# timescale/pgvectorscale

Hardware: AMD Instinct MI355X
Metric: QPS at recall@10>=0.99 (higher is better)
Workload: dtype u64 xor+popcount (SBQ) / f32 (rerank)

## Files before the change

include/vsgpu.h:

```cpp
#ifndef VSGPU_H
#define VSGPU_H

#include <stddef.h>
#include <stdint.h>

#ifdef __cplusplus
extern "C" {
#endif

#define VS_INVALID_NODE 0xFFFFFFFFu

enum vs_distance_type { VS_COSINE = 0, VS_L2 = 1, VS_IP = 2 };
enum vs_storage_type { VS_STORAGE_SBQ = 0, VS_STORAGE_PLAIN = 1 };

enum vs_status {
    VS_OK = 0,
    VS_ERR_INVALID = -1,
    VS_ERR_HIP = -2,
    VS_ERR_OOM = -3,
    VS_ERR_CAPACITY = -4,
    VS_ERR_STATE = -5
};

typedef struct vs_ctx vs_ctx;
typedef struct vs_index vs_index;
typedef struct vs_scan vs_scan;

typedef struct vs_index_desc {
    uint32_t n;
    uint32_t dim_full;
    uint32_t dim_index;
    uint32_t bits;
    uint32_t words;
    uint32_t num_neighbors;
    uint32_t distance_type;
    uint32_t has_labels;
    uint32_t default_start;
    uint32_t n_label_starts;
    uint32_t storage_type;
} vs_index_desc;

typedef struct vs_index_host {
    const uint64_t* codes;
    const uint32_t* nbrs;
    uint32_t nbr_stride;
    const uint64_t* heap_tids;
    const float* vecs;
    const float* mean;
    const float* m2;
    uint64_t count;
    const uint32_t* label_off;
    const int16_t* label_val;
    const int16_t* label_start_labels;
    const uint32_t* label_start_nodes;
} vs_index_host;

typedef struct vs_stats {
    uint64_t queries;
    uint64_t visited_nodes;
    uint64_t candidate_nodes;
    uint64_t quantized_distance_comparisons;
    uint64_t full_distance_comparisons;
    uint64_t node_reads;
    uint64_t node_heap_reads;
    uint64_t next_calls;
    uint64_t retries;
    uint64_t fallback_scans;
    uint64_t fallback_visited_nodes;
    uint64_t fallback_quantized_distance_comparisons;
} vs_stats;

const char* vs_last_error(void);

int vs_set_option(const char* name, const char* value);
int vs_get_option(const char* name, char* out, size_t cap);
const char* vs_version(void);

int vs_ctx_create(int device, vs_ctx** out);
int vs_ctx_create_staging(int device, size_t staging_bytes, vs_ctx** out);
void vs_ctx_destroy(vs_ctx* ctx);
int vs_ctx_sync(vs_ctx* ctx);
void* vs_ctx_stream(vs_ctx* ctx);
int vs_ctx_device_name(vs_ctx* ctx, char* buf, size_t len);
int vs_ctx_mem_info(vs_ctx* ctx, uint64_t* free_bytes, uint64_t* total_bytes);

typedef struct vs_profile {
    double ms[8];
    uint64_t launches[8];
} vs_profile;
int vs_profile_enable(vs_ctx* ctx, int on);
int vs_profile_read(vs_ctx* ctx, vs_profile* out, int reset);

int vs_dev_alloc(vs_ctx* ctx, size_t bytes, void** out);
int vs_dev_free(vs_ctx* ctx, void* p);
int vs_dev_upload(vs_ctx* ctx, void* dst_dev, const void* src_host, size_t bytes);
int vs_dev_download(vs_ctx* ctx, void* dst_host, const void* src_dev, size_t bytes);

int vs_index_upload(vs_ctx* ctx, const vs_index_desc* desc, const vs_index_host* host, vs_index** out);
int vs_index_alloc(vs_ctx* ctx, const vs_index_desc* desc, int with_vecs, vs_index** out);
void vs_index_free(vs_index* idx);
int vs_index_view(vs_index* src, vs_ctx* ctx, vs_index** out);
int vs_index_set_slab(vs_index* idx, void* d_mem, size_t bytes);
int vs_ws_probe(vs_ctx* ctx, void* d_mem, size_t bytes, uint32_t iters, float* ms_out);
int vs_ws_probe_mix(vs_index* idx, void* d_mem, size_t bytes, uint32_t iters, float* ms_out);
int vs_index_prepare_workspace(vs_index* idx);
int vs_index_get_desc(const vs_index* idx, vs_index_desc* out);
enum vs_array { VS_ARR_CODES = 0, VS_ARR_NBRS = 1, VS_ARR_TIDS = 2, VS_ARR_VECS = 3, VS_ARR_MEAN = 4, VS_ARR_M2 = 5,
                VS_ARR_VNORM = 6, VS_ARR_LABEL_OFF = 7, VS_ARR_LABEL_VAL = 8 };
int vs_index_array(const vs_index* idx, int which, void** dev_ptr, uint32_t* row_stride);
int vs_index_rerank_order(vs_index* idx, uint32_t* out_perm, uint32_t cap, uint32_t* out_n);
int vs_index_set_quantizer(vs_index* idx, const float* mean, const float* m2, uint64_t count);
int vs_index_set_start_nodes(vs_index* idx, uint32_t default_start, const int16_t* labels, const uint32_t* nodes, uint32_t n);
int vs_index_set_labels(vs_index* idx, const uint32_t* label_off, const int16_t* label_val);
int vs_index_set_visibility(vs_index* idx, const uint8_t* visible);
int vs_index_set_visibility_dev(vs_index* idx, const uint8_t* d_visible);
#define VS_MAX_SNAPSHOTS 16
int vs_index_snapshot_put(vs_index* idx, uint32_t snapshot, const uint8_t* visible);
int vs_index_snapshot_use(vs_index* idx, uint32_t snapshot, const uint8_t** previous );
int vs_index_snapshot_share(vs_index* view, const vs_index* src);
int vs_index_device(const vs_index* idx);
int vs_index_has_neighbor_masks(const vs_index* idx);
int vs_index_get_quantizer(const vs_index* idx, float* mean, float* m2, uint64_t* count);
int vs_index_download(const vs_index* idx, uint64_t* codes, uint32_t* nbrs , uint64_t* heap_tids,
                      float* vecs, uint32_t row_begin, uint32_t row_count);
int vs_index_refresh_norms(vs_index* idx);
int vs_index_mark_deleted(vs_index* idx, const uint32_t* nodes, uint32_t n);
typedef struct vs_bulk_delete_stats {
    uint64_t tuples_removed;
    uint64_t num_index_tuples;
    uint64_t already_deleted;
} vs_bulk_delete_stats;
int vs_index_bulk_delete(vs_index* idx, const uint64_t* dead_tids, uint64_t n_dead, vs_bulk_delete_stats* out );
int vs_index_bulk_delete_dev(vs_index* idx, const uint64_t* d_dead_tids_sorted, uint64_t n_dead, vs_bulk_delete_stats* out);
#define VS_CONSOLIDATE_NO_REPAIR 1u
typedef struct vs_consolidate_stats {
    uint64_t tombstones;
    uint64_t tombstones_kept;
    uint64_t rows_rewritten;
    uint64_t edges_dropped;
    uint64_t edges_added;
    uint64_t rows_pruned;
    uint64_t rows_capped;
    uint64_t rows_emptied;
    uint32_t unreachable_live;
} vs_consolidate_stats;
int vs_index_consolidate_deletes(vs_index* idx, double max_alpha, uint32_t cand_max , uint32_t flags,
                                 vs_consolidate_stats* out );
int vs_index_consolidate_kernel_ms(vs_index* idx, double* ms, int reset);
#define VS_COMPACT_KEEP_EDGES_CHECK 1u
typedef struct vs_compact_stats {
    uint32_t n_before, n_after;
    uint64_t tombstones;
    uint64_t tombstones_kept;
    uint64_t rows_moved;
    uint64_t edges_cut;
    uint64_t rows_emptied;
    uint32_t chunks;
} vs_compact_stats;
int vs_index_compact(vs_index* idx, uint64_t stage_bytes , uint32_t flags,
                     uint32_t* out_new_of , vs_compact_stats* out );
int vs_index_compact_kernel_ms(vs_index* idx, double* ms, int reset);
int vs_index_shrink_to_fit(vs_index* idx);

#define VS_BLCKSZ 8192u
enum vs_page_type {
    VS_PAGE_META_V1 = 0, VS_PAGE_NODE = 1, VS_PAGE_PQ_QUANTIZER_DEF = 2, VS_PAGE_PQ_QUANTIZER_VECTOR = 3,
    VS_PAGE_SBQ_MEANS_V1 = 4, VS_PAGE_SBQ_NODE = 5, VS_PAGE_META_V2 = 6, VS_PAGE_SBQ_MEANS = 7, VS_PAGE_META = 8 };

typedef struct vs_node_layout {
    uint32_t root_size;
    uint32_t off_heap_item_pointer;
    uint32_t off_bq_vector;
    uint32_t off_neighbor_index_pointers;
    uint32_t off_labels;
} vs_node_layout;
int vs_node_layout_default(int has_labels, vs_node_layout* out);

typedef struct vs_pages_info {
    uint32_t n_blocks;
    uint32_t n_nodes;
    uint32_t words;
    uint32_t num_neighbors;
    uint32_t has_labels;
    uint32_t n_deleted;
    uint64_t n_label_vals;
    uint32_t pages_by_type[9];
    uint32_t new_pages;
    uint32_t meta_magic;
    uint32_t meta_version;
} vs_pages_info;

typedef struct vs_pages vs_pages;
int vs_pages_open(uint32_t page_size, int has_labels, const vs_node_layout* layout, uint32_t threads, vs_pages** out);
int vs_plain_layout_default(vs_node_layout* out);
int vs_pages_open_plain(uint32_t page_size, const vs_node_layout* layout, uint32_t threads, vs_pages** out);
int vs_pages_add(vs_pages* p, uint32_t first_block, const void* pages, uint32_t n_blocks);
int vs_pages_finish(vs_pages* p, vs_pages_info* info);
int vs_pages_host(const vs_pages* p, vs_index_host* host);
int vs_pages_node_of(const vs_pages* p, uint32_t block, uint32_t offset, uint32_t* node);
int vs_pages_item_pointer_of(const vs_pages* p, uint32_t node, uint32_t* block, uint32_t* offset);
int vs_pages_read_chain(const vs_pages* p, uint32_t block, uint32_t offset, int page_type, void* buf, size_t cap, size_t* len);
int vs_pages_sbq_means(const vs_pages* p, uint32_t block, uint32_t offset, float* mean, float* m2, uint32_t dim_cap,
                       uint32_t* dim, uint64_t* count);
void vs_pages_close(vs_pages* p);
int vs_pages_headers_only(vs_pages* p);
int vs_pages_block_table(const vs_pages* p, const uint32_t** blk_base, const uint32_t** blk_cnt, uint32_t* n_blocks);

typedef struct vs_meta_layout {
    uint32_t root_size;
    uint32_t off_magic_number, off_version, off_extension_version_when_built, off_distance_type, off_num_dimensions,
        off_num_dimensions_to_index, off_bq_num_bits_per_dimension, off_storage_type, off_num_neighbors, off_search_list_size,
        off_max_alpha, off_start_nodes, off_quantizer_metadata, off_has_labels;
} vs_meta_layout;
int vs_meta_layout_default(vs_meta_layout* out);
typedef struct vs_meta_page {
    uint32_t magic_number, version;
    char extension_version_when_built[64];
    uint32_t distance_type;
    uint32_t num_dimensions, num_dimensions_to_index, bq_num_bits_per_dimension;
    uint32_t storage_type;
    uint32_t num_neighbors, search_list_size;
    double max_alpha;
    uint32_t has_start_nodes;
    uint32_t default_start_block, default_start_offset;
    uint32_t n_labeled_start_nodes;
    uint32_t quantizer_block, quantizer_offset;
    uint32_t has_labels;
} vs_meta_page;
int vs_meta_page_decode(const void* bytes, size_t len, const vs_meta_layout* layout, vs_meta_page* out, int16_t* start_labels,
                        uint32_t* start_blocks, uint32_t* start_offsets, uint32_t cap);
int vs_pages_meta(const vs_pages* p, const vs_meta_layout* layout, vs_meta_page* meta, vs_index_desc* desc, int16_t* start_labels,
                  uint32_t* start_nodes, uint32_t cap);

typedef struct vs_heap_attr {
    int16_t attlen;
    char attalign;
} vs_heap_attr;
typedef struct vs_heap_info {
    uint32_t n_nodes, heap_blocks, toast_blocks;
    uint32_t n_inline;
    uint32_t n_external;
    uint32_t n_deleted;
    uint32_t n_null;
    uint32_t n_dead_line_pointer;
    uint32_t n_not_found;
    uint32_t n_toast_incomplete;
    uint64_t n_chunks;
} vs_heap_info;
typedef struct vs_heap vs_heap;
int vs_heap_open(uint32_t page_size, const vs_heap_attr* attrs, uint32_t natts, uint32_t vector_attno, uint32_t dim,
                 const uint64_t* heap_tids, uint32_t n, float* out_vecs, uint32_t out_stride, vs_heap** out);
int vs_heap_add(vs_heap* h, uint32_t first_block, const void* pages, uint32_t n_blocks);
int vs_heap_toast_add(vs_heap* h, uint32_t first_block, const void* pages, uint32_t n_blocks);
int vs_heap_finish(vs_heap* h, vs_heap_info* info, uint8_t* found);
void vs_heap_close(vs_heap* h);

typedef struct vs_pages_dev vs_pages_dev;
int vs_pages_dev_open(vs_ctx* ctx, uint32_t page_size, const vs_node_layout* layout, uint32_t n_blocks_total, vs_pages_dev** out);
int vs_pages_dev_add(vs_pages_dev* d, uint32_t first_block, const void* pages, uint32_t n_blocks);
int vs_pages_dev_node_of(const vs_pages_dev* d, uint32_t block, uint32_t offset, uint32_t* node);
int vs_pages_dev_sbq_means(const vs_pages_dev* d, uint32_t block, uint32_t offset, float* mean, float* m2, uint32_t dim_cap,
                           uint32_t* dim, uint64_t* count);
int vs_pages_dev_meta(vs_pages_dev* d, const vs_meta_layout* layout, vs_meta_page* meta, vs_index_desc* desc, int16_t* start_labels,
// ... 265 lines not shown
```

pgvectorscale_amd/__init__.py:

```python
from ._lib import VS_COSINE, VS_INVALID_NODE, VS_IP, VS_L2, VsError, load
from .index import Broker, Context, DiskAnnIndex, IndexScan, ScanPool, ShmClient, ShmServer, get_option, set_option
from .multi import Comm, MultiIndex
```

pgvectorscale_amd/_lib.py:

```python
import ctypes as C
import os

_HERE = os.path.dirname(os.path.abspath(__file__))
LIB_PATH = os.environ.get("VS_LIB_PATH") or os.path.join(_HERE, "libvsgpu.so")

VS_INVALID_NODE = 0xFFFFFFFF
VS_COSINE, VS_L2, VS_IP = 0, 1, 2
VS_STORAGE_SBQ, VS_STORAGE_PLAIN = 0, 1
ARR_CODES, ARR_NBRS, ARR_TIDS, ARR_VECS, ARR_MEAN, ARR_M2, ARR_VNORM, ARR_LABEL_OFF, ARR_LABEL_VAL = range(9)


class VsError(RuntimeError):
    def __init__(self, code, msg):
        super().__init__(f"libvsgpu error {code}: {msg}")
        self.code = code


class IndexDesc(C.Structure):
    _fields_ = [(k, C.c_uint32) for k in ("n", "dim_full", "dim_index", "bits", "words", "num_neighbors",
                                          "distance_type", "has_labels", "default_start", "n_label_starts", "storage_type")]


class IndexHost(C.Structure):
    _fields_ = [("codes", C.c_void_p), ("nbrs", C.c_void_p), ("nbr_stride", C.c_uint32), ("heap_tids", C.c_void_p),
# ... 39 lines not shown
class MetaPage(C.Structure):
    _fields_ = [("magic_number", C.c_uint32), ("version", C.c_uint32), ("extension_version_when_built", C.c_char * 64),
                ("distance_type", C.c_uint32), ("num_dimensions", C.c_uint32), ("num_dimensions_to_index", C.c_uint32),
                ("bq_num_bits_per_dimension", C.c_uint32), ("storage_type", C.c_uint32), ("num_neighbors", C.c_uint32),
                ("search_list_size", C.c_uint32), ("max_alpha", C.c_double), ("has_start_nodes", C.c_uint32),
                ("default_start_block", C.c_uint32), ("default_start_offset", C.c_uint32), ("n_labeled_start_nodes", C.c_uint32),
                ("quantizer_block", C.c_uint32), ("quantizer_offset", C.c_uint32), ("has_labels", C.c_uint32)]

    def as_dict(self):
        d = {k: getattr(self, k) for k, _ in self._fields_}
        d["extension_version_when_built"] = d["extension_version_when_built"].decode()
        return d


class HeapAttr(C.Structure):
    _fields_ = [("attlen", C.c_int16), ("attalign", C.c_char)]


class HeapInfo(C.Structure):
    _fields_ = [(k, C.c_uint32) for k in ("n_nodes", "heap_blocks", "toast_blocks", "n_inline", "n_external", "n_deleted", "n_null",
                                          "n_dead_line_pointer", "n_not_found", "n_toast_incomplete")] + [("n_chunks", C.c_uint64)]

    def as_dict(self):
        return {k: int(getattr(self, k)) for k, _ in self._fields_}


class PagesInfo(C.Structure):
    _fields_ = [("n_blocks", C.c_uint32), ("n_nodes", C.c_uint32), ("words", C.c_uint32), ("num_neighbors", C.c_uint32),
                ("has_labels", C.c_uint32), ("n_deleted", C.c_uint32), ("n_label_vals", C.c_uint64),
                ("pages_by_type", C.c_uint32 * 9), ("new_pages", C.c_uint32), ("meta_magic", C.c_uint32),
                ("meta_version", C.c_uint32)]


class PagesOutParams(C.Structure):
    _fields_ = [("page_size", C.c_uint32), ("node_layout", C.POINTER(NodeLayout)), ("meta_layout", C.POINTER(MetaLayout)),
                ("extension_version", C.c_char_p), ("search_list_size", C.c_uint32), ("max_alpha", C.c_double)]


class BrokerConfig(C.Structure):
    _fields_ = [("max_batch", C.c_uint32), ("max_wait_us", C.c_uint32), ("cursor_lanes", C.c_uint32), ("cursor_pool", C.c_uint32)]


class BrokerStats(C.Structure):
    _fields_ = [("batches", C.c_uint64), ("scans", C.c_uint64), ("max_batch", C.c_uint64), ("tasks", C.c_uint64), ("cursors", C.c_uint64)]


class Profile(C.Structure):
    _fields_ = [("ms", C.c_double * 8), ("launches", C.c_uint64 * 8)]


class InsertStats(C.Structure):
    _fields_ = [(k, C.c_uint32) for k in ("first_node", "inserted", "batches", "retries", "mate_edges", "orphans_placed",
                                          "orphans_left", "grew")]

    def as_dict(self):
        return {k: int(getattr(self, k)) for k, _ in self._fields_}


class BulkDeleteStats(C.Structure):
    _fields_ = [(k, C.c_uint64) for k in ("tuples_removed", "num_index_tuples", "already_deleted")]

    def as_dict(self):
        return {k: int(getattr(self, k)) for k, _ in self._fields_}


class ConsolidateStats(C.Structure):
    _fields_ = [(k, C.c_uint64) for k in ("tombstones", "tombstones_kept", "rows_rewritten", "edges_dropped", "edges_added", "rows_pruned",
                                          "rows_capped", "rows_emptied")] + [("unreachable_live", C.c_uint32)]

    def as_dict(self):
        return {k: int(getattr(self, k)) for k, _ in self._fields_}


VS_CONSOLIDATE_NO_REPAIR = 1


class CompactStats(C.Structure):
    _fields_ = [("n_before", C.c_uint32), ("n_after", C.c_uint32)] + [(k, C.c_uint64) for k in (
        "tombstones", "tombstones_kept", "rows_moved", "edges_cut", "rows_emptied")] + [("chunks", C.c_uint32)]

    def as_dict(self):
        return {k: int(getattr(self, k)) for k, _ in self._fields_}


VS_COMPACT_KEEP_EDGES_CHECK = 1


class LabelReachStats(C.Structure):
    _fields_ = [("lost_pairs", C.c_uint64)] + [(k, C.c_uint32) for k in ("lost_nodes", "labels", "labels_without_start", "sweeps")]

    def as_dict(self):
        return {k: int(getattr(self, k)) for k, _ in self._fields_}


class LabelRepairStats(C.Structure):
    _fields_ = [(k, C.c_uint64) for k in ("lost_pairs_before", "lost_pairs_after", "placed_free", "placed_over_dropped", "placed_victim",
                                          "blocked", "contended", "rows_changed", "source_tiles")] + [(k, C.c_uint32) for k in (
        "lost_nodes_before", "lost_nodes_after", "rounds", "sweeps", "labels_without_start", "unreachable_live")]

    def as_dict(self):
        return {k: int(getattr(self, k)) for k, _ in self._fields_}


class PagesFollowInfo(C.Structure):
    _fields_ = [(k, C.c_uint32) for k in ("n_blocks_before", "n_blocks_now", "pages_listed", "node_pages_listed", "n_before", "n_appended",
                                          "rows_relinked", "tids_cleared", "tids_changed", "codes_changed")] + [("label_vals_appended", C.c_uint64)]

    def as_dict(self):
        return {k: int(getattr(self, k)) for k, _ in self._fields_}


class DatagenParams(C.Structure):
    _fields_ = [("seed", C.c_uint64), ("dim", C.c_uint32), ("latent_dim", C.c_uint32), ("n_clusters", C.c_uint32),
                ("intra_pct", C.c_uint32), ("noise_pct", C.c_uint32), ("normalize", C.c_uint32)]


_vp, _u32, _u64, _i, _sz = C.c_void_p, C.c_uint32, C.c_uint64, C.c_int, C.c_size_t
SYMBOLS = {
    "vs_last_error": (C.c_char_p, []),
    "vs_set_option": (_i, [C.c_char_p, C.c_char_p]),
    "vs_get_option": (_i, [C.c_char_p, C.c_char_p, C.c_size_t]),
    "vs_version": (C.c_char_p, []),
    "vs_ctx_create": (_i, [_i, C.POINTER(_vp)]),
    "vs_ctx_create_staging": (_i, [_i, _sz, C.POINTER(_vp)]),
    "vs_ctx_destroy": (None, [_vp]),
    "vs_ctx_sync": (_i, [_vp]),
    "vs_ctx_stream": (_vp, [_vp]),
    "vs_ctx_device_name": (_i, [_vp, C.c_char_p, _sz]),
    "vs_ctx_mem_info": (_i, [_vp, C.POINTER(_u64), C.POINTER(_u64)]),
    "vs_profile_enable": (_i, [_vp, _i]),
    "vs_profile_read": (_i, [_vp, C.POINTER(Profile), _i]),
    "vs_dev_alloc": (_i, [_vp, _sz, C.POINTER(_vp)]),
    "vs_dev_free": (_i, [_vp, _vp]),
    "vs_dev_upload": (_i, [_vp, _vp, _vp, _sz]),
    "vs_dev_download": (_i, [_vp, _vp, _vp, _sz]),
    "vs_index_upload": (_i, [_vp, C.POINTER(IndexDesc), C.POINTER(IndexHost), C.POINTER(_vp)]),
    "vs_index_alloc": (_i, [_vp, C.POINTER(IndexDesc), _i, C.POINTER(_vp)]),
    "vs_index_free": (None, [_vp]),
    "vs_index_view": (_i, [_vp, _vp, _vp]),
    "vs_scanpool_create": (_i, [_vp, _u32, _u32, _u32, _u32, _u32, C.POINTER(_vp)]),
    "vs_scanpool_free": (None, [_vp]),
    "vs_scanpool_rescan": (_i, [_vp, _u32, _vp, _vp, _u32, _i]),
    "vs_scanpool_endscan": (_i, [_vp, _u32]),
    "vs_scanpool_fetch": (_i, [_vp, _vp, _u32, _u32, _vp, _vp, _vp, _vp]),
    "vs_scanpool_get_stats": (_i, [_vp, _u32, _vp]),
    "vs_scanpool_get_work": (_i, [_vp, C.POINTER(_u64), C.POINTER(_u64)]),
    "vs_index_set_slab": (_i, [_vp, _vp, C.c_size_t]),
    "vs_ws_probe": (_i, [_vp, _vp, C.c_size_t, C.c_uint32, C.POINTER(C.c_float)]),
    "vs_ws_probe_mix": (_i, [_vp, _vp, C.c_size_t, C.c_uint32, C.POINTER(C.c_float)]),
    "vs_index_prepare_workspace": (_i, [_vp]),
    "vs_index_get_desc": (_i, [_vp, C.POINTER(IndexDesc)]),
    "vs_index_array": (_i, [_vp, _i, C.POINTER(_vp), C.POINTER(_u32)]),
    "vs_index_rerank_order": (_i, [_vp, _vp, _u32, C.POINTER(_u32)]),
    "vs_index_set_quantizer": (_i, [_vp, _vp, _vp, _u64]),
    "vs_index_set_start_nodes": (_i, [_vp, _u32, _vp, _vp, _u32]),
    "vs_index_set_labels": (_i, [_vp, _vp, _vp]),
    "vs_index_set_visibility": (_i, [_vp, _vp]),
    "vs_index_set_visibility_dev": (_i, [_vp, _vp]),
    "vs_index_get_quantizer": (_i, [_vp, _vp, _vp, C.POINTER(_u64)]),
    "vs_index_download": (_i, [_vp, _vp, _vp, _vp, _vp, _u32, _u32]),
    "vs_index_refresh_norms": (_i, [_vp]),
    "vs_index_mark_deleted": (_i, [_vp, _vp, _u32]),
    "vs_index_bulk_delete": (_i, [_vp, _vp, _u64, C.POINTER(BulkDeleteStats)]),
    "vs_index_bulk_delete_dev": (_i, [_vp, _vp, _u64, C.POINTER(BulkDeleteStats)]),
    "vs_index_consolidate_deletes": (_i, [_vp, C.c_double, _u32, _u32, C.POINTER(ConsolidateStats)]),
    "vs_index_consolidate_kernel_ms": (_i, [_vp, C.POINTER(C.c_double), _i]),
    "vs_index_compact": (_i, [_vp, C.c_uint64, _u32, _vp, C.POINTER(CompactStats)]),
    "vs_index_compact_kernel_ms": (_i, [_vp, C.POINTER(C.c_double), _i]),
    "vs_index_shrink_to_fit": (_i, [_vp]),
    "vs_node_layout_default": (_i, [_i, C.POINTER(NodeLayout)]),
    "vs_pages_open": (_i, [_u32, _i, C.POINTER(NodeLayout), _u32, C.POINTER(_vp)]),
    "vs_pages_open_plain": (_i, [_u32, C.POINTER(NodeLayout), _u32, C.POINTER(_vp)]),
    "vs_plain_layout_default": (_i, [C.POINTER(NodeLayout)]),
    "vs_pages_add": (_i, [_vp, _u32, _vp, _u32]),
    "vs_pages_finish": (_i, [_vp, C.POINTER(PagesInfo)]),
    "vs_pages_host": (_i, [_vp, C.POINTER(IndexHost)]),
    "vs_pages_node_of": (_i, [_vp, _u32, _u32, C.POINTER(_u32)]),
    "vs_pages_item_pointer_of": (_i, [_vp, _u32, C.POINTER(_u32), C.POINTER(_u32)]),
    "vs_pages_read_chain": (_i, [_vp, _u32, _u32, _i, _vp, _sz, C.POINTER(_sz)]),
    "vs_pages_sbq_means": (_i, [_vp, _u32, _u32, _vp, _vp, _u32, C.POINTER(_u32), C.POINTER(_u64)]),
    "vs_pages_close": (None, [_vp]),
    "vs_heap_open": (_i, [_u32, C.POINTER(HeapAttr), _u32, _u32, _u32, _vp, _u32, _vp, _u32, C.POINTER(_vp)]),
    "vs_heap_add": (_i, [_vp, _u32, _vp, _u32]),
    "vs_heap_toast_add": (_i, [_vp, _u32, _vp, _u32]),
    "vs_heap_finish": (_i, [_vp, C.POINTER(HeapInfo), _vp]),
    "vs_heap_close": (None, [_vp]),
    "vs_meta_layout_default": (_i, [C.POINTER(MetaLayout)]),
    "vs_meta_page_decode": (_i, [_vp, _sz, C.POINTER(MetaLayout), C.POINTER(MetaPage), _vp, _vp, _vp, _u32]),
    "vs_pages_meta": (_i, [_vp, C.POINTER(MetaLayout), C.POINTER(MetaPage), C.POINTER(IndexDesc), _vp, _vp, _u32]),
    "vs_pages_dev_meta": (_i, [_vp, C.POINTER(MetaLayout), C.POINTER(MetaPage), C.POINTER(IndexDesc), _vp, _vp, _u32]),
    "vs_pages_headers_only": (_i, [_vp]),
    "vs_pages_block_table": (_i, [_vp, C.POINTER(_vp), C.POINTER(_vp), C.POINTER(_u32)]),
    "vs_pages_dev_open": (_i, [_vp, _u32, C.POINTER(NodeLayout), _u32, C.POINTER(_vp)]),
    "vs_pages_dev_add": (_i, [_vp, _u32, _vp, _u32]),
    "vs_pages_dev_node_of": (_i, [_vp, _u32, _u32, C.POINTER(_u32)]),
    "vs_pages_dev_sbq_means": (_i, [_vp, _u32, _u32, _vp, _vp, _u32, C.POINTER(_u32), C.POINTER(_u64)]),
    "vs_pages_dev_build": (_i, [_vp, C.POINTER(IndexDesc), C.POINTER(IndexHost), C.POINTER(PagesInfo), C.POINTER(_vp)]),
    "vs_pages_dev_close": (None, [_vp]),
    "vs_pages_dev_block_table": (_i, [_vp, C.POINTER(_vp), C.POINTER(_vp), C.POINTER(_u32)]),
    "vs_pages_follow_open": (_i, [_vp, _u32, C.POINTER(NodeLayout), _vp, _u32, C.POINTER(_vp)]),
    "vs_pages_follow_stage": (_i, [_vp, _vp, _vp, _u32, _u32, C.POINTER(PagesFollowInfo)]),
    "vs_pages_follow_new_tids": (_i, [_vp, _vp, _u32]),
    "vs_pages_follow_apply": (_i, [_vp, _vp, _u32, C.POINTER(PagesFollowInfo)]),
    "vs_pages_follow_discard": (_i, [_vp]),
    "vs_pages_follow_close": (None, [_vp]),
    "vs_pages_out_open": (_i, [_vp, C.POINTER(PagesOutParams), C.POINTER(_vp), C.POINTER(PagesInfo)]),
    "vs_pages_out_open_plain": (_i, [_vp, C.POINTER(PagesOutParams), C.POINTER(_vp), C.POINTER(PagesInfo)]),
    "vs_pages_out_read": (_i, [_vp, _u32, _u32, _vp]),
    "vs_pages_out_read_dev": (_i, [_vp, _u32, _u32, _vp]),
    "vs_pages_out_item_pointer_of": (_i, [_vp, _u32, C.POINTER(_u32), C.POINTER(_u32)]),
    "vs_pages_out_close": (None, [_vp]),
    "vs_pages_out_baseline": (_i, [_vp, C.POINTER(_vp)]),
    "vs_pages_base_free": (None, [_vp]),
    "vs_pages_base_blocks": (_u32, [_vp]),
    "vs_pages_out_delta": (_i, [_vp, _vp, C.POINTER(_u32), C.POINTER(_u32), C.POINTER(_vp)]),
    "vs_pages_out_delta_blocks": (_i, [_vp, _vp, _u32]),
    "vs_pages_out_read_blocks": (_i, [_vp, _vp, _u32, _vp]),
    "vs_pages_out_read_blocks_dev": (_i, [_vp, _vp, _u32, _vp]),
    "vs_meta_page_encode": (_i, [C.POINTER(MetaPage), _vp, _vp, _vp, _u32, C.POINTER(MetaLayout), _vp, _sz, C.POINTER(_sz)]),
    "vs_quantize": (_i, [_vp, _vp, _u32, _vp]),
    "vs_hamming_gather": (_i, [_vp, _vp, _vp, _vp, _u32, _vp]),
    "vs_rerank": (_i, [_vp, _vp, _vp, _vp, _u32, _vp]),
    "vs_prepare_queries": (_i, [_vp, _vp, _u32, _vp, _vp, _vp]),
    "vs_scan_topk": (_i, [_vp, _vp, _u32, _u32, _vp, _vp]),
    "vs_scan_topk_filtered": (_i, [_vp, _vp, _vp, _vp, _i, _u32, _u32, _vp, _vp]),
    "vs_search_batch": (_i, [_vp, _vp, _vp, _vp, _u32, _u32, _u32, _u32, _vp, _vp, _vp, C.POINTER(Stats)]),
    "vs_stream_batch": (_i, [_vp, _vp, _vp, _vp, _u32, _u32, _u32, _vp, _vp, C.POINTER(Stats)]),
    "vs_search_batch_dev": (_i, [_vp, _vp, _vp, _vp, _u32, _u32, _u32, _u32, _vp, _vp, _vp]),
    "vs_search_batch_dev_finish": (_i, [_vp, C.POINTER(Stats)]),
    "vs_index_autotune": (_i, [_vp, _vp, _vp, _vp, _u32, _u32, _u32, _u32, _u32, C.c_char_p, C.POINTER(TuneEntry), _u32, C.POINTER(_u32)]),
    "vs_index_set_variant": (_i, [_vp, C.c_char_p]),
    "vs_index_get_variant": (_i, [_vp, C.c_char_p, C.c_size_t]),
    "vs_beginscan": (_i, [_vp, C.POINTER(_vp)]),
    "vs_rescan": (_i, [_vp, _vp, _vp, _u32, _i, _u32, _u32]),
    "vs_gettuple": (_i, [_vp, C.POINTER(_u64), C.POINTER(_u32), C.POINTER(C.c_float)]),
    "vs_scan_xs_recheck": (_i, [_vp]),
    "vs_scan_get_stats": (_i, [_vp, C.POINTER(Stats)]),
    "vs_scan_get_work": (_i, [_vp, C.POINTER(Stats), C.POINTER(_u32)]),
    "vs_endscan": (None, [_vp]),
    "vs_broker_create": (_i, [_vp, C.POINTER(BrokerConfig), C.POINTER(_vp)]),
    "vs_broker_search": (_i, [_vp, _vp, _vp, _u32, _i, _u32, _u32, _u32, _vp, _vp, _vp]),
    "vs_broker_search_snapshot": (_i, [_vp, _vp, _vp, _u32, _i, _u32, _u32, _u32, _u32, _vp, _vp, _vp]),
    "vs_broker_snapshot_put": (_i, [_vp, _u32, _vp]),
    "vs_index_snapshot_put": (_i, [_vp, _u32, _vp]),
    "vs_index_has_neighbor_masks": (_i, [_vp]),
    "vs_index_snapshot_use": (_i, [_vp, _u32, _vp]),
    "vs_index_snapshot_share": (_i, [_vp, _vp]),
    "vs_index_device": (_i, [_vp]),
    "vs_broker_get_stats": (_i, [_vp, C.POINTER(BrokerStats)]),
    "vs_broker_destroy": (None, [_vp]),
    "vs_broker_index": (_vp, [_vp]),
    "vs_beginscan_on_broker": (_i, [_vp, C.POINTER(_vp)]),
    "vs_broker_call": (_i, [_vp, _vp, _vp]),
    "vs_scan_set_snapshot": (_i, [_vp, _u32]),
    "vs_scan_prefetch": (_i, [_vp, _u32]),
    "vs_shm_client_fetch": (_i, [_vp, C.c_uint64, _vp, _vp, _u32, _i, _u32, _u32, _u32, _u32, _u32, _vp, _vp, _vp, C.POINTER(_u32)]),
    "vs_shm_client_end_scan": (_i, [_vp, C.c_uint64]),
    "vs_shm_server_create": (_i, [_vp, C.c_char_p, _u32, _u32, C.POINTER(BrokerConfig), C.POINTER(_vp)]),
    "vs_shm_server_get_stats": (_i, [_vp, C.POINTER(BrokerStats)]),
    "vs_shm_server_pool_stats": (_i, [_vp, C.POINTER(C.c_uint64)]),
    "vs_shm_server_destroy": (None, [_vp]),
    "vs_shm_server_snapshot_put": (_i, [_vp, _u32, _vp]),
    "vs_shm_client_search_snapshot": (_i, [_vp, _vp, _vp, _u32, _i, _u32, _u32, _u32, _u32, _vp, _vp, _vp]),
    "vs_shm_client_open": (_i, [C.c_char_p, C.POINTER(_vp)]),
    "vs_shm_client_dim": (_u32, [_vp]),
    "vs_shm_client_search": (_i, [_vp, _vp, _vp, _u32, _i, _u32, _u32, _u32, _vp, _vp, _vp]),
    "vs_shm_client_close": (None, [_vp]),
    "vs_shard_range": (_i, [_u32, _u32, _u32, C.POINTER(_u32), C.POINTER(_u32)]),
    "vs_index_replicate": (_i, [_vp, _vp, C.POINTER(_vp)]),
    "vs_multi_create": (_i, [_vp, C.POINTER(_i), _u32, _u32, C.POINTER(_vp)]),
    "vs_multi_size": (_u32, [_vp]),
    "vs_multi_index": (_vp, [_vp, _u32]),
    "vs_multi_ctx": (_vp, [_vp, _u32]),
    "vs_multi_search_batch": (_i, [_vp, _vp, _vp, _vp, _u32, _u32, _u32, _u32, _vp, _vp, _vp, C.POINTER(Stats)]),
    "vs_multi_stream_batch": (_i, [_vp, _vp, _vp, _vp, _u32, _u32, _u32, _vp, _vp, C.POINTER(Stats)]),
    "vs_multi_destroy": (None, [_vp]),
    "vs_comm_unique_id": (_i, [_vp]),
    "vs_comm_create": (_i, [_vp, _vp, _u32, _u32, C.POINTER(_vp)]),
    "vs_comm_rank": (_u32, [_vp]),
    "vs_comm_world": (_u32, [_vp]),
    "vs_comm_gather_topk": (_i, [_vp, _vp, _vp, _u32, _u32, _u32, _vp, _vp]),
    "vs_comm_bcast": (_i, [_vp, _vp, _sz, _u32]),
    "vs_comm_replicate_index": (_i, [_vp, _vp, _u32]),
    "vs_comm_destroy": (None, [_vp]),
    "vs_sbq_train": (_i, [_vp]),
    "vs_sbq_quantize_corpus": (_i, [_vp]),
    "vs_build_graph": (_i, [_vp, _u32, C.c_double, _u32, _u64]),
    "vs_index_build_unreachable": (_u32, [_vp]),
    "vs_index_reserve": (_i, [_vp, _u32]),
    "vs_index_capacity": (_u32, [_vp]),
    "vs_index_insert": (_i, [_vp, _vp, _vp, _vp, _vp, _u32, _u32, C.c_double, _u32, C.POINTER(InsertStats)]),
    "vs_index_insert_dev": (_i, [_vp, _vp, _vp, _vp, _vp, _u32, _u32, C.c_double, _u32, C.POINTER(InsertStats)]),
    "vs_index_insert_kernel_ms": (_i, [_vp, C.POINTER(C.c_double), _i]),
    "vs_index_build_kernel_ms": (_i, [_vp, C.POINTER(C.c_double), _i]),
    "vs_batch_mates": (_i, [_vp, _vp, _u32, _u32, _vp, _vp]),
    "vs_batch_mates_filtered": (_i, [_vp, _vp, _vp, _vp, _u32, _u32, _vp, _vp]),
    "vs_batch_mates_plain": (_i, [_vp, _u32, _u32, _u32, _vp, _vp]),
    "vs_prune_plain": (_i, [_vp, _vp, _vp, _vp, _u32, C.c_double, _vp, _vp]),
    "vs_index_repair": (_i, [_vp, C.POINTER(_u32)]),
    "vs_index_label_reach": (_i, [_vp, C.POINTER(LabelReachStats), _vp, _vp, _vp, _u32, _vp]),
    "vs_index_repair_labels": (_i, [_vp, _u32, _u32, C.POINTER(LabelRepairStats)]),
    "vs_index_label_repair_kernel_ms": (_i, [_vp, C.POINTER(C.c_double), _i]),
    "vs_nearest_masked": (_i, [_vp, _vp, _vp, _u32, _vp, _vp, _vp, _vp]),
    "vs_datagen_fill": (_i, [_vp, C.POINTER(DatagenParams), _u64, _u64, _vp]),
    "vs_bruteforce_topk": (_i, [_vp, _vp, _u32, _u32, _vp, _vp]),
}
# ... 32 lines not shown
```

pgvectorscale_amd/csrc/vs_batch.hip:

```cpp
#include <thread>
#include <cstdarg>
#include <cmath>
#include <algorithm>
#include <cstdlib>

#include <atomic>
#include <mutex>
#include <unordered_map>

#include "vs_internal.h"


static uint32_t knob_u32(const char* name, int tuned, uint32_t dflt) {
    const char* v = vs_opt_get(name);
    if (v && *v) return (uint32_t)strtoul(v, nullptr, 10);
    return tuned >= 0 ? (uint32_t)tuned : dflt;
}

static uint32_t gload_pct() { return std::min<uint32_t>(std::max<uint32_t>(env_u32("VS_F_GLOAD_PCT", 75), 25), 90); }

static Caps initial_caps(const vs_index* ix, uint32_t L, uint32_t M) {
    uint64_t visits = 2ull * L + M + 32;
    uint64_t pushes = visits * ix->d.num_neighbors;
    Caps c;
    c.hl = env_u32("VS_HL", 1024);
    c.lh = env_u32("VS_LH", 0);
    c.g0 = env_u32("VS_G0", 4096);
    c.hcap = (uint32_t)std::min<uint64_t>(std::max<uint64_t>(pushes, c.hl), 1u << 22);
    c.vcap = (uint32_t)std::min<uint64_t>(3ull * L + M + 64, 1u << 20);
    c.hashcap = std::max<uint32_t>(next_pow2_u32(std::min<uint64_t>(2ull * pushes, 1u << 23)), c.g0);
    const uint64_t typ_visits = (uint64_t)L + L / 4 + M + 16;
    uint64_t typ_ins = typ_visits * std::min<uint64_t>(ix->d.num_neighbors, 16);
    if (ix->obs.valid && ix->obs.L == L && ix->obs.M == M) typ_ins = (uint64_t)(ix->obs.ins_mean * 1.75) + 96;
    const bool lds_table = typ_ins <= knob_u32("VS_F_LDS_MAX_INS", ix->tune.lds_max_ins, 1024);
    c.f_lh = env_u32("VS_F_LH", lds_table ? (uint32_t)round_up_u32((uint32_t)typ_ins, 64) : 0u);
    c.f_pool_frac = !lds_table ? 1.0
                    : (ix->obs.valid && ix->obs.L == L && ix->obs.M == M) ? std::min(1.0, 2.0 * ix->obs.ov_frac + 0.03) : 1.0;
    if (const char* e = vs_opt_get("VS_F_POOL")) c.f_pool_frac = std::min(1.0, std::max(0.01, atof(e)));
    uint32_t hl_auto = 1023;
    if (lds_table && ix->obs.valid && ix->obs.L == L && ix->obs.M == M) {
        const double want = 0.75 * ix->obs.ins_mean;
        hl_auto = want > 2047 ? 4095 : (want > 1023 ? 2047 : 1023);
    }
    if (!lds_table) hl_auto = 511;
    c.f_hl = env_u32("VS_F_HL", hl_auto);
    const uint32_t want_v = (uint32_t)std::min<uint64_t>((uint64_t)L + L / 2 + 32, 1u << 20);
    c.f_vr = knob_u32("VS_F_VR", ix->tune.vr, (lds_table && want_v <= 512) ? 8 : 0);
    c.f_vcap = c.f_vr ? 512 : round_up_u32(std::max<uint32_t>(env_u32("VS_F_VCAP", 2 * want_v), 64), 64);
    c.f_on = env_u32("VS_FAST", 1) != 0 && ix->d.storage_type != VS_STORAGE_PLAIN;
    if (c.f_on) {
        if (c.f_lh) c.f_lh = round_up_u32(std::max<uint32_t>(c.f_lh, 256), 4);
        c.f_hl = std::max<uint32_t>(next_pow2_u32(c.f_hl + 1), 64) - 1;
        c.f_gcap = next_pow2_u32(std::min<uint64_t>(std::max<uint64_t>(std::min<uint64_t>(pushes, 4 * typ_ins), 1024), 1u << 22));
        if (!lds_table && ix->obs.valid && ix->obs.L == L && ix->obs.M == M && env_u32("VS_F_GCAP_FIT", 1)) {
            const uint64_t need = (uint64_t)((ix->obs.ins_max * 1.04 + 128) * 100.0 / gload_pct()) + 64;
            c.f_gcap = (uint32_t)std::min<uint64_t>(c.f_gcap, std::max<uint64_t>(round_up_u32((uint32_t)std::min<uint64_t>(need, 1u << 22), 256), 1024));
        }
        if (const uint32_t g = env_u32("VS_F_GCAP", lds_table ? 0 : ix->tune.gcap)) c.f_gcap = round_up_u32(std::max<uint32_t>(g, 256), 256);
        c.f_sb = 0;
        while ((1ull << c.f_sb) < (uint64_t)c.f_lh + c.f_gcap) c.f_sb++;
        c.f_hcap = (uint32_t)std::min<uint64_t>(std::max<uint64_t>(pushes, c.f_hl), 1u << 22);
        c.f_gstride = round_up_u32(c.f_hcap - c.f_hl + 2, 2);
        const uint64_t nbits = (uint64_t)ix->d.dim_index * ix->d.bits;
        FastLaunch probe{};
        probe.hl = c.f_hl;
        probe.lh = c.f_lh;
        probe.vr = c.f_vr;
        probe.vcap = c.f_vcap;
        if (nbits >= (1ull << (32 - c.f_sb)) || fast_lds_bytes(ix, probe) > 64 * 1024) c.f_on = false;
    }
    return c;
}

static uint32_t fast_pool_slots(uint32_t nq, double frac) {
    const uint64_t floor_slots = vs_opt_get("VS_F_POOL") ? 1 : 256;
    return (uint32_t)std::min<uint64_t>(nq, std::max<uint64_t>(floor_slots, (uint64_t)(frac * nq) + 1));
}
static uint32_t general_pool_slots(uint32_t nq) { return std::max<uint32_t>(64, nq / 64); }

static bool grow_caps(Caps& c, uint32_t ovf) {
    bool grew = (ovf & (OVF_POOL | OVF_KEY)) != 0;
    if ((ovf & OVF_HEAP) && c.hcap < (1u << 24)) {
        c.hcap *= 2;
        grew = true;
    }
    if (ovf & OVF_VISITED) {
        c.vcap *= 2;
        grew = true;
    }
    if ((ovf & OVF_HASH) && c.hashcap < (1u << 26)) {
        c.hashcap *= 2;
        grew = true;
    }
    return grew;
}

static const double ORDER_MIN_REUSE = 2.0;
static const uint32_t ORDER_MIN_NQ = 16384;
static const uint32_t ORDER_SEEDS = 1024;
static const uint32_t ORDER_LABEL_SEEDS = 2048;
static uint32_t rerank_order_seeds(const vs_index* ix, uint32_t nq, uint32_t M, bool* by_labels) {
    const uint32_t mode = env_u32("VS_RERANK_ORDER", 1);
    *by_labels = mode != 2 && !ix->is_view;
    if (mode == 0 || !scan_order_fits(ix)) return 0;
    if (mode == 1 && (nq < ORDER_MIN_NQ || (double)nq * M < ORDER_MIN_REUSE * (double)ix->d.n)) return 0;
    const uint32_t S = std::min<uint32_t>(std::max<uint32_t>(env_u32("VS_RERANK_SEEDS", *by_labels ? ORDER_LABEL_SEEDS : ORDER_SEEDS), 1), 4096);
    return std::min<uint32_t>(S, ix->d.n);
}

static int ensure_region_labels(vs_index* ix, uint32_t S) {
    vs_ctx* c = ix->ctx;
    SearchWorkspace& w = ix->ws;
    const uint32_t n = ix->d.n, step = n / S;
    const bool kept = w.lab_rows > 0 && w.lab_rows <= n && w.lab_epoch == ix->codes_epoch && w.lab_S == S && w.lab_step == step;
    const uint32_t from = kept ? w.lab_rows : 0;
    if (from == n) return VS_OK;
    const bool debug = env_u32("VS_WS_DEBUG", 0) != 0;
    if (debug) VS_HIP(hipStreamSynchronize(c->stream));
    const auto t0 = std::chrono::steady_clock::now();
    if ((size_t)n * 2 > w.order_labels.bytes) {
        DevBuf grown;
        VS_TRY(devbuf_reserve(c, grown, std::max<size_t>((size_t)n * 2, w.order_labels.bytes + w.order_labels.bytes / 2)));
        if (from) VS_HIP(hipMemcpyAsync(grown.p, w.order_labels.p, (size_t)from * 2, hipMemcpyDeviceToDevice, c->stream));
        VS_HIP(hipStreamSynchronize(c->stream));
        devbuf_free(w.order_labels);
        w.order_labels = grown;
    }
    w.lab_rows = 0;
    VS_TRY(launch_region_labels(ix, S, step, from, n - from, (uint16_t*)w.order_labels.p));
    w.lab_rows = n;
    w.lab_S = S;
    w.lab_step = step;
    w.lab_epoch = ix->codes_epoch;
    if (debug) {
        VS_HIP(hipStreamSynchronize(c->stream));
        fprintf(stderr, "[VS_WS_DEBUG] region labels: rows %u .. %u, %u seeds %u rows apart, %.3f ms\n", from, n, S, step,
                std::chrono::duration<double, std::milli>(std::chrono::steady_clock::now() - t0).count());
    }
    return VS_OK;
}

extern "C" int vs_index_rerank_order(vs_index* ix, uint32_t* out_perm, uint32_t cap, uint32_t* out_n) {
    VS_REQUIRE(ix && out_n && (cap == 0 || out_perm), "vs_index_rerank_order: bad args");
    VS_HIP(hipStreamSynchronize(ix->ctx->stream));
    *out_n = ix->ws.order_nq;
    const uint32_t m = std::min(cap, ix->ws.order_nq);
    if (m) VS_HIP(hipMemcpy(out_perm, ix->ws.order_perm.p, (size_t)m * 4, hipMemcpyDeviceToHost));
    return VS_OK;
}

static int run_post_search(vs_index* ix, const BatchPlan& bp, uint32_t* d_out_ids, uint64_t* d_out_tids, float* d_out_dist) {
    vs_ctx* c = ix->ctx;
    SearchWorkspace& w = ix->ws;
    const uint32_t nq = bp.nq, M = bp.M;
    if (bp.stream_only) return VS_OK;
    if (bp.rescore > 0) {
        VS_REQUIRE(ix->vecs, "diskann.query_rescore > 0 needs the heap vector column on the device");
        const uint32_t* perm = nullptr;
        bool deal = false;
        w.order_nq = 0;
        bool by_labels = false;
        if (const uint32_t S = rerank_order_seeds(ix, nq, M, &by_labels)) {
            VS_TRY(devbuf_reserve(c, w.order_work, scan_order_work_bytes(nq, S + 1)));
            VS_TRY(devbuf_reserve(c, w.order_perm, (size_t)nq * 4));
            if (by_labels) VS_TRY(ensure_region_labels(ix, S));
            hipEvent_t ev = prof_begin(c);
            if (by_labels)
                VS_TRY(launch_label_order(ix, (const uint16_t*)w.order_labels.p, w.lab_rows, S, (const uint32_t*)w.stream_ids.p,
                                          (const uint32_t*)w.stream_cnt.p, M, nq, (uint32_t*)w.order_work.p, (uint32_t*)w.order_perm.p));
            else
                VS_TRY(launch_scan_order(ix, (const uint64_t*)w.qcodes.p, nq, S, (uint32_t*)w.order_work.p, (uint32_t*)w.order_perm.p));
            prof_end(c, PK_ORDER, ev);
            perm = (const uint32_t*)w.order_perm.p;
            w.order_nq = nq;
            deal = env_u32("VS_RERANK_DEAL", 1) != 0;
        }
        const uint32_t fused = env_u32("VS_RERANK_FUSED", 1);
        if (fused && rerank_window_fits(ix, M, bp.rescore, bp.k)) {
            hipEvent_t ev = prof_begin(c);
            VS_TRY(launch_rerank_window(ix, (const float*)w.q_full.p, (const uint32_t*)w.stream_ids.p, (const uint32_t*)w.stream_cnt.p, M,
                                        bp.rescore, bp.k, nq, d_out_ids, d_out_tids, d_out_dist, fused == 2 ? 2u : 1u, perm, deal));
            prof_end(c, PK_RERANK, ev);
            return VS_OK;
        }
        VS_TRY(devbuf_reserve(c, w.rr_dist, (size_t)nq * M * 4));
        VS_TRY(devbuf_reserve(c, w.resort_heap, (size_t)nq * bp.rescore * 8));
        hipEvent_t ev = prof_begin(c);
        VS_TRY(launch_rerank(ix, (const float*)w.q_full.p, (const uint32_t*)w.stream_ids.p, nullptr,
                             (const uint32_t*)w.stream_cnt.p, M, nq, (float*)w.rr_dist.p, 0, perm, deal));
        prof_end(c, PK_RERANK, ev);
    }
    hipEvent_t ev = prof_begin(c);
    VS_TRY(launch_resort(ix, nq, M, bp.rescore, bp.k, (const uint32_t*)w.stream_ids.p, (const uint32_t*)w.stream_cnt.p,
                         bp.rescore ? (const float*)w.rr_dist.p : nullptr, (uint64_t*)w.resort_heap.p, d_out_ids,
                         d_out_tids, d_out_dist));
    prof_end(c, PK_RESORT, ev);
    return VS_OK;
}

static int enqueue_reduce(vs_index* ix, const BatchPlan& bp) {
    vs_ctx* c = ix->ctx;
    SearchWorkspace& w = ix->ws;
    VS_TRY(devbuf_reserve(c, w.red, RED_N * 8));
    if (!w.red_host) VS_HIP(hipHostMalloc((void**)&w.red_host, RED_N * 8, hipHostMallocDefault));
    VS_HIP(hipMemsetAsync(w.red.p, 0, RED_N * 8, c->stream));
    VS_TRY(launch_reduce_stats(ix, (const uint32_t*)w.stats.p, w.fb_valid ? (const uint32_t*)w.fb_flag.p : nullptr,
                               (const uint32_t*)w.stream_cnt.p, (const uint32_t*)w.status.p, bp.nq, bp.M, bp.rescore,
                               !bp.stream_only && bp.rescore > 0, ix->last_ins_limit, (uint64_t*)w.red.p));
    VS_HIP(hipMemcpyAsync(w.red_host, w.red.p, RED_N * 8, hipMemcpyDeviceToHost, c->stream));
    return VS_OK;
}

static SearchLaunch general_launch(const vs_index* ix, const BatchPlan& bp, const Caps& caps, const int16_t* d_qlabels,
                                   const uint32_t* d_qlabel_off) {
    const SearchWorkspace& w = ix->ws;
    SearchLaunch s;
    s.nq = bp.nq;
    s.L = bp.L;
    s.M = bp.M;
    s.hl = caps.hl;
    s.hcap = caps.hcap;
    s.vcap = caps.vcap;
    s.lh = caps.lh;
    s.hashcap = caps.hashcap;
    s.g0 = caps.g0;
    s.qcodes = (const uint64_t*)w.qcodes.p;
    s.qlabels = d_qlabels;
    s.qlabel_off = d_qlabel_off;
    s.heap_g = (uint64_t*)w.heap_g.p;
    s.hash = (uint32_t*)w.hash.p;
    s.out_ids = (uint32_t*)w.stream_ids.p;
    s.out_ham = (uint32_t*)w.stream_ham.p;
    s.out_cnt = (uint32_t*)w.stream_cnt.p;
    s.stats = (uint32_t*)w.stats.p;
    s.status = (uint32_t*)w.status.p;
    s.visible = (!bp.stream_only && bp.rescore > 0) ? ix->visible : nullptr;
    return s;
}

static int reserve_general_regions(vs_index* ix, const Caps& caps, uint32_t gslots) {
    vs_ctx* c = ix->ctx;
    SearchWorkspace& w = ix->ws;
    const size_t hg = caps.hcap > caps.hl ? caps.hcap - caps.hl : 0;
    VS_TRY(devbuf_reserve(c, w.hash, (size_t)gslots * caps.hashcap * 4));
    VS_TRY(devbuf_reserve(c, w.heap_g, std::max<size_t>((size_t)gslots * hg * 8, 16)));
    return devbuf_reserve(c, w.pool_ctr, 64);
}

static int retry_failed_scans(vs_index* ix, const BatchPlan& bp, const int16_t* d_qlabels, const uint32_t* d_qlabel_off,
                              Caps& caps, vs_stats* st) {
    vs_ctx* c = ix->ctx;
    SearchWorkspace& w = ix->ws;
    const uint32_t nq = bp.nq;
    std::vector<uint32_t> status(nq);
    for (int attempt = 0;; ++attempt) {
        VS_HIP(hipMemcpyAsync(status.data(), w.status.p, (size_t)nq * 4, hipMemcpyDeviceToHost, c->stream));
        VS_HIP(hipStreamSynchronize(c->stream));
        uint32_t ovf = 0, nbad = 0;
        for (uint32_t v : status) {
            ovf |= v;
            nbad += v != 0;
        }
        if (!ovf) return VS_OK;
        if (st) st->retries++;
        if (attempt >= 8 || !grow_caps(caps, ovf)) {
            vs_set_error("search structures overflowed in %u of %u scans (flags 0x%x) at hcap=%u vcap=%u hashcap=%u", nbad, nq,
                         ovf, caps.hcap, caps.vcap, caps.hashcap);
            return VS_ERR_CAPACITY;
        }
        const uint32_t gslots = std::min<uint32_t>(nq, std::max<uint32_t>(general_pool_slots(nq), nbad));
        VS_TRY(reserve_general_regions(ix, caps, gslots));
        VS_HIP(hipMemsetAsync((char*)w.pool_ctr.p + 32, 0, 4, c->stream));
        SearchLaunch s = general_launch(ix, bp, caps, d_qlabels, d_qlabel_off);
        s.only_failed = 1;
        s.fb_flag = w.fb_valid ? (uint32_t*)w.fb_flag.p : nullptr;
        s.pool_counter = (uint32_t*)((char*)w.pool_ctr.p + 32);
        s.pool_slots = gslots;
        hipEvent_t ev = prof_begin(c);
        VS_TRY(launch_search(ix, s));
        prof_end(c, PK_SEARCH_FB, ev);
    }
}

struct FastPlan {
    FastLaunch f;
    uint32_t gregion;
    uint32_t fslots;
};
template <class T>
static T* fast_select() {
    return (T*)16;
}

static bool opt_is_set(const char* name) {
    const char* v = vs_opt_get(name);
    return v && *v;
}
static uint32_t visited_want(uint32_t L) { return (uint32_t)std::min<uint64_t>((uint64_t)L + L / 2 + 32, 1u << 20); }

static int candidate_holds(vs_index* ix, const FastLaunch& base, const FastLaunch& cand, uint64_t num, uint64_t den, bool* holds,
                           const char* base_name = nullptr, const char* cand_name = nullptr, const char* tail = "") {
    uint32_t res_base = 0, res_cand = 0;
    VS_TRY(fast_resident_scans(ix, base, &res_base));
    VS_TRY(fast_resident_scans(ix, cand, &res_cand));
    if (base_name && env_u32("VS_WS_DEBUG", 0))
        fprintf(stderr, "[VS_WS_DEBUG] resident scans: %s %u, %s %u%s\n", base_name, res_base, cand_name, res_cand, tail);
    *holds = num * res_cand >= den * res_base;
    return VS_OK;
}

static int choose_table_bitmap(vs_index* ix, FastLaunch& f, uint32_t vmode, bool phase, bool* slot_eligible) {
    *slot_eligible = false;
    if (f.lh != 0 || f.vr || !vmode || phase || f.gcap > (1u << 16)) return VS_OK;
    f.vwords = (f.gcap + 127) / 128;
    if (vmode < 2 || f.rc || f.gcap % 32 != 0) return VS_OK;
    *slot_eligible = true;
    FastLaunch g = f;
    g.vwords = f.gcap / 32;
    g.vslot = 1;
    bool holds = false;
    VS_TRY(candidate_holds(ix, f, g, 1, 1, &holds));
    if (holds || env_u32("VS_F_SLOTMAP_FORCE", 0)) f = g;
    return VS_OK;
}

static int choose_tables16(vs_index* ix, FastLaunch& f, uint32_t vmode, bool slot_eligible, bool keyed, uint32_t* gregion) {
    if (vmode != 3 || !f.vwords || !slot_eligible || f.lh != 0) return VS_OK;
    FastLaunch g = f;
    g.gcap = std::max<uint32_t>(next_pow2_u32(f.gcap), 1024);
    if (!fast_tables16_geometry(ix, g)) return VS_OK;
    g.glimit = (uint32_t)((uint64_t)g.gcap * gload_pct() / 100) - 64u;
    char tail[48];
    snprintf(tail, sizeof tail, "; gcap %u -> %u", f.gcap, g.gcap);
    bool holds = false;
    VS_TRY(candidate_holds(ix, f, g, keyed ? 3 : 5, keyed ? 2 : 4, &holds, "4-byte tables", "16-bit tables", tail));
    if (holds || env_u32("VS_F_SLOTMAP_FORCE", 0)) {
        f = g;
        *gregion = g.gregion;
    }
    return VS_OK;
}

static int choose_heap_top(vs_index* ix, FastLaunch& f, Caps& caps, bool phase) {
    if (f.lh != 0 || f.vr || f.hl != 511 || f.hcap <= 511 || phase || opt_is_set("VS_F_HL")) return VS_OK;
    FastLaunch h = f;
    h.hl = 255;
    h.gstride = round_up_u32(h.hcap - h.hl + 2, 2);
    bool holds = false;
    VS_TRY(candidate_holds(ix, f, h, 10, 11, &holds, "heap top 511", "255"));
    if (holds) {
        f = h;
        caps.f_hl = h.hl;
        caps.f_gstride = h.gstride;
    }
    return VS_OK;
}

static int choose_visited_ring(vs_index* ix, FastLaunch& f, uint32_t L, bool phase) {
    if (f.lh != 0 || f.vr || f.minw == 7 || phase) return VS_OK;
    const uint32_t want_v = visited_want(L);
    const uint32_t lean_v = round_up_u32(std::max<uint32_t>(want_v + 2 * want_v / 5, 64), 64);
    if (opt_is_set("VS_F_VCAP") || lean_v >= f.vcap) return VS_OK;
    FastLaunch v = f;
    v.vcap = lean_v;
    char wide_name[40], lean_name[24];
    snprintf(wide_name, sizeof wide_name, "visited ring %u entries", f.vcap);
    snprintf(lean_name, sizeof lean_name, "%u entries", v.vcap);
    bool holds = false;
    VS_TRY(candidate_holds(ix, f, v, 10, 11, &holds, wide_name, lean_name));
    if (holds) f = v;
    return VS_OK;
}

static void choose_ring_step7(FastLaunch& f, uint32_t L) {
    if (f.minw == 7 && f.vslot == 2 && !f.vr && !env_u32("VS_F_VCAP", 0)) f.vcap = round_up_u32(std::max<uint32_t>(2 * visited_want(L), 64), 16);
}

static int choose_persistent_grid(vs_index* ix, FastLaunch& f, uint32_t* fslots) {
    if (!knob_u32("VS_F_PERSIST", ix->tune.persist, 1)) return VS_OK;
    uint32_t res = 0;
    VS_TRY(fast_resident_scans(ix, f, &res));
    f.persist = std::max<uint32_t>(1, (uint32_t)((uint64_t)res * env_u32("VS_F_PERSIST_PCT", 100) / 100));
    *fslots = std::min(f.persist, f.nq);
    return VS_OK;
}

static int plan_fast_launch(vs_index* ix, const BatchPlan& bp, Caps& caps, bool keyed, bool masked, FastPlan* out) {
    const bool phase = env_u32("VS_PHASE", 0) != 0;
    FastPlan p{};
    FastLaunch& f = p.f;
    f.nq = bp.nq;
    f.L = bp.L;
    f.M = bp.M;
    f.hl = caps.f_hl;
    f.hcap = caps.f_hcap;
    f.gstride = caps.f_gstride;
    f.vr = caps.f_vr;
    f.gcap = caps.f_gcap;
    f.glimit = (uint32_t)((uint64_t)caps.f_gcap * gload_pct() / 100) - 64u;
    f.lh = caps.f_lh;
    f.minw = knob_u32("VS_F_MINW", (caps.f_lh == 0 && !caps.f_vr) ? ix->tune.minw : -1, caps.f_lh == 0 ? (caps.f_vr ? 4 : 6) : 1);
    f.flags = env_u32("VS_F_FLAGS", 0);
    f.sb = caps.f_sb;
    f.vcap = caps.f_vcap;
    f.qlabel_off = keyed ? fast_select<const uint32_t>() : nullptr;
    f.visible = masked ? fast_select<const uint8_t>() : nullptr;
    f.rc = caps.f_lh == 0 ? env_u32("VS_F_RC", 0) : 0;
    if (f.rc) f.rc = next_pow2_u32(f.rc);
    p.gregion = f.gcap;
    p.fslots = fast_pool_slots(bp.nq, caps.f_pool_frac);
    const uint32_t vmode = knob_u32("VS_F_VIRGIN", ix->tune.virgin, 3);
    bool slot_eligible = false;
    VS_TRY(choose_table_bitmap(ix, f, vmode, phase, &slot_eligible));
    VS_TRY(choose_tables16(ix, f, vmode, slot_eligible, keyed, &p.gregion));
    VS_TRY(choose_heap_top(ix, f, caps, phase));
    VS_TRY(choose_visited_ring(ix, f, bp.L, phase));
    choose_ring_step7(f, bp.L);
    if (phase) f.phase = fast_select<uint64_t>();
    VS_TRY(choose_persistent_grid(ix, f, &p.fslots));
    *out = p;
    return VS_OK;
}

static bool second_attempt_of(const vs_index* ix, const FastLaunch& first, uint32_t nq, FastLaunch* out) {
    const SearchWorkspace& w = ix->ws;
    FastLaunch r = first;
    r.vwords = 0;
    r.vslot = 0;
    r.persist = 0;
    r.timeline = nullptr;
    r.only_failed = 1;
    r.fb_flag = (uint32_t*)w.fb_flag.p;
    r.phase = nullptr;
    r.gcap = (uint32_t)std::min<uint64_t>(4ull * first.gcap, 1u << 22);
    r.glimit = 0;
    r.hcap = (uint32_t)std::min<uint64_t>(2ull * first.hcap, 1u << 22);
    r.gstride = round_up_u32(r.hcap - r.hl + 2, 2);
    if (!r.vr) r.vcap = 2 * first.vcap;
    r.sb = 0;
    while ((1ull << r.sb) < (uint64_t)r.lh + r.gcap) r.sb++;
    r.pool_slots = general_pool_slots(nq);
    r.pool_counter = (uint32_t*)((char*)w.pool_ctr.p + 16);
    *out = r;
    const uint64_t nbits = (uint64_t)ix->d.dim_index * ix->d.bits;
    return nbits < (1ull << (32 - r.sb)) && fast_lds_bytes(ix, r) <= 64 * 1024;
}

static int bind_fast_buffers(vs_index* ix, FastPlan& p, const int16_t* d_qlabels, const uint32_t* d_qlabel_off, const uint8_t* visible) {
    vs_ctx* c = ix->ctx;
    SearchWorkspace& w = ix->ws;
    FastLaunch& f = p.f;
    const size_t table_bytes = (size_t)p.fslots * p.gregion * 4;
    if (f.persist) {
        const size_t heap_bytes = std::max<size_t>((size_t)p.fslots * f.gstride * 4, 16);
        const uint32_t what = env_u32("VS_WS_SLAB_WHAT", 3);
        if (what & 1) VS_TRY(devbuf_reserve_hot(ix, w.ghash4, table_bytes, 0));
        else VS_TRY(devbuf_reserve(c, w.ghash4, table_bytes));
        if (what & 2) VS_TRY(devbuf_reserve_hot(ix, w.heap_g4, heap_bytes, 1));
        else VS_TRY(devbuf_reserve(c, w.heap_g4, heap_bytes));
    } else {
        VS_TRY(devbuf_reserve(c, w.heap_g4, std::max<size_t>((size_t)f.nq * f.gstride * 4, 16)));
        VS_TRY(devbuf_reserve(c, w.ghash4, table_bytes));
    }
    if (env_u32("VS_WS_DEBUG", 0))
        fprintf(stderr, "[VS_WS_DEBUG] ghash4 %p (%zu B%s) heap_g4 %p (%zu B%s) region bytes: table %zu heap %zu x %u regions; stream_ids %p qcodes %p\n", w.ghash4.p,
                w.ghash4.bytes, w.ghash4.in_slab ? ", slab" : "", w.heap_g4.p, w.heap_g4.bytes, w.heap_g4.in_slab ? ", slab" : "",
                (size_t)p.gregion * 4, (size_t)f.gstride * 4, p.fslots, w.stream_ids.p, w.qcodes.p);
    VS_TRY(devbuf_reserve(c, w.pool_ctr, 64));
    VS_HIP(hipMemsetAsync(w.pool_ctr.p, 0, 64, c->stream));
    VS_TRY(devbuf_reserve(c, w.fb_flag, (size_t)f.nq * 4));
    VS_HIP(hipMemsetAsync(w.fb_flag.p, 0, (size_t)f.nq * 4, c->stream));
    f.qlabels = d_qlabels;
    f.qlabel_off = d_qlabel_off;
    f.visible = visible;
    f.heap_g = (uint32_t*)w.heap_g4.p;
    f.ghash = (uint32_t*)w.ghash4.p;
    f.pool_counter = (uint32_t*)w.pool_ctr.p;
    f.scan_counter = (uint32_t*)w.pool_ctr.p + 2;
    f.pool_slots = p.fslots;
    f.phase = nullptr;
    f.qcodes = (const uint64_t*)w.qcodes.p;
    f.out_ids = (uint32_t*)w.stream_ids.p;
    f.out_ham = (uint32_t*)w.stream_ham.p;
    f.out_cnt = (uint32_t*)w.stream_cnt.p;
    f.stats = (uint32_t*)w.stats.p;
    f.status = (uint32_t*)w.status.p;
    return VS_OK;
}

static int bind_phase_buffer(vs_index* ix, FastLaunch& f) {
    if (!env_u32("VS_PHASE", 0)) return VS_OK;
    SearchWorkspace& w = ix->ws;
    VS_TRY(devbuf_reserve(ix->ctx, w.phase, (size_t)f.nq * 64));
    VS_HIP(hipMemsetAsync(w.phase.p, 0, (size_t)f.nq * 64, ix->ctx->stream));
    f.phase = (uint64_t*)w.phase.p;
    return VS_OK;
}

static int bind_timeline_buffer(vs_index* ix, FastLaunch& f, std::string* path) {
    const char* const tl_opt = vs_opt_get("VS_TIMELINE");
    *path = tl_opt ? tl_opt : "";
    if (path->empty()) return VS_OK;
    SearchWorkspace& w = ix->ws;
    VS_TRY(devbuf_reserve(ix->ctx, w.timeline, (size_t)f.nq * 16));
    VS_HIP(hipMemsetAsync(w.timeline.p, 0, (size_t)f.nq * 16, ix->ctx->stream));
    f.timeline = (uint64_t*)w.timeline.p;
    return VS_OK;
}
static int dump_timeline(vs_index* ix, uint32_t nq, const std::string& path) {
    std::vector<uint64_t> tl((size_t)nq * 2);
    VS_HIP(hipMemcpyAsync(tl.data(), ix->ws.timeline.p, tl.size() * 8, hipMemcpyDeviceToHost, ix->ctx->stream));
    VS_HIP(hipStreamSynchronize(ix->ctx->stream));
    if (FILE* fp = fopen(path.c_str(), "wb")) {
        fwrite(tl.data(), 8, tl.size(), fp);
        fclose(fp);
    }
    return VS_OK;
}

static int dump_fast_status(vs_index* ix, const FastLaunch& f, double pool_frac) {
    vs_ctx* c = ix->ctx;
    SearchWorkspace& w = ix->ws;
    std::vector<uint32_t> stv(f.nq);
    VS_HIP(hipMemcpyAsync(stv.data(), w.status.p, (size_t)f.nq * 4, hipMemcpyDeviceToHost, c->stream));
    uint32_t ctr[2] = {0, 0};
    VS_HIP(hipMemcpyAsync(ctr, w.pool_ctr.p, 4, hipMemcpyDeviceToHost, c->stream));
    VS_HIP(hipStreamSynchronize(c->stream));
    uint32_t hist[16] = {0};
    for (uint32_t v : stv) hist[v & 15]++;
    fprintf(stderr, "[VS_DEBUG_STATUS] fast kernel: lh=%u gcap=%u vr=%u minw=%u bitmap_words=%u (per %s); pool claims=%u of %u;",
            f.lh, f.gcap, f.vr, f.minw, f.vwords, f.vslot == 2 ? "slot, 16-bit entries" : f.vslot ? "slot" : "bucket", ctr[0], fast_pool_slots(f.nq, pool_frac));
    for (int i = 0; i < 16; ++i)
        if (hist[i]) fprintf(stderr, " status[%d]=%u", i, hist[i]);
    fprintf(stderr, "\n");
    return VS_OK;
}

static int run_fast_attempts(vs_index* ix, const BatchPlan& bp, Caps& caps, const int16_t* d_qlabels, const uint32_t* d_qlabel_off) {
    vs_ctx* c = ix->ctx;
    SearchWorkspace& w = ix->ws;
    const uint8_t* const visible = (!bp.stream_only && bp.rescore > 0) ? ix->visible : nullptr;
    ix->last_ins_limit = caps.f_lh ? caps.f_lh - caps.f_lh / 8 - 64 : 0xFFFFFFFFu;
    FastPlan p;
    VS_TRY(plan_fast_launch(ix, bp, caps, d_qlabel_off != nullptr, visible != nullptr, &p));
    FastLaunch& f = p.f;
    VS_TRY(bind_fast_buffers(ix, p, d_qlabels, d_qlabel_off, visible));
    VS_TRY(bind_phase_buffer(ix, f));
    std::string tl_path;
    VS_TRY(bind_timeline_buffer(ix, f, &tl_path));
    hipEvent_t ev = prof_begin(c);
    VS_TRY(launch_search_fast(ix, f));
    prof_end(c, PK_SEARCH, ev);
    if (f.timeline) VS_TRY(dump_timeline(ix, bp.nq, tl_path));
    ix->last_fast = FastSig{f.vwords, f.minw, f.gcap, f.lh, f.vr, 1u};
    FastLaunch r;
    if (env_u32("VS_F_RETRY", 1) && second_attempt_of(ix, f, bp.nq, &r)) {
        VS_TRY(devbuf_reserve(c, w.heap_g4b, (size_t)r.pool_slots * r.gstride * 4));
        VS_TRY(devbuf_reserve(c, w.ghash4b, (size_t)r.pool_slots * r.gcap * 4));
        r.heap_g = (uint32_t*)w.heap_g4b.p;
        r.ghash = (uint32_t*)w.ghash4b.p;
        hipEvent_t ev2 = prof_begin(c);
        VS_TRY(launch_search_fast(ix, r));
        prof_end(c, PK_SEARCH_FB, ev2);
    }
    if (env_u32("VS_DEBUG_STATUS", 0)) VS_TRY(dump_fast_status(ix, f, caps.f_pool_frac));
    return VS_OK;
}

static int run_search_chunk(vs_index* ix, const BatchPlan& bp, const float* d_raw_q, const int16_t* d_qlabels,
                            const uint32_t* d_qlabel_off, uint32_t* d_out_ids, uint64_t* d_out_tids, float* d_out_dist, Caps& caps) {
    vs_ctx* c = ix->ctx;
    SearchWorkspace& w = ix->ws;
    const uint32_t nq = bp.nq, M = bp.M;
    VS_TRY(devbuf_reserve(c, w.q_full, (size_t)nq * ix->vec_stride * 4));
    VS_TRY(devbuf_reserve(c, w.qcodes, (size_t)nq * ix->code_stride * 8));
    VS_TRY(devbuf_reserve(c, w.stream_ids, (size_t)nq * M * 4));
    VS_TRY(devbuf_reserve(c, w.stream_ham, (size_t)nq * M * 4));
    VS_TRY(devbuf_reserve(c, w.stream_cnt, (size_t)nq * 4));
    VS_TRY(devbuf_reserve(c, w.stats, (size_t)nq * ST_N * 4));
    VS_TRY(devbuf_reserve(c, w.status, (size_t)nq * 4));
    {
        hipEvent_t ev = prof_begin(c);
        VS_TRY(launch_prepare_queries(ix, d_raw_q, nq, (float*)w.q_full.p, (uint64_t*)w.qcodes.p));
        if (ix->d.storage_type == VS_STORAGE_PLAIN && ix->d.dim_index < ix->d.dim_full) {
            VS_TRY(devbuf_reserve(c, w.q_index, (size_t)nq * ix->vec_stride * 4));
            VS_TRY(launch_prepare_index_slice(ix, d_raw_q, nq, (float*)w.q_index.p));
        }
        prof_end(c, PK_PREPARE, ev);
    }
    ix->last_fast = FastSig{};
    const bool fast_done = caps.f_on;
    if (fast_done) VS_TRY(run_fast_attempts(ix, bp, caps, d_qlabels, d_qlabel_off));
    w.fb_valid = fast_done;
    {
        const uint32_t gslots = fast_done ? general_pool_slots(nq) : nq;
        VS_TRY(reserve_general_regions(ix, caps, gslots));
        if (fast_done) VS_HIP(hipMemsetAsync((char*)w.pool_ctr.p + 32, 0, 4, c->stream));
        SearchLaunch s = general_launch(ix, bp, caps, d_qlabels, d_qlabel_off);
        s.only_failed = fast_done ? 1u : 0u;
        s.fb_flag = fast_done ? (uint32_t*)w.fb_flag.p : nullptr;
        s.pool_counter = fast_done ? (uint32_t*)((char*)w.pool_ctr.p + 32) : nullptr;
        s.pool_slots = gslots;
        hipEvent_t ev = prof_begin(c);
        VS_TRY(launch_search(ix, s));
        prof_end(c, fast_done ? PK_SEARCH_FB : PK_SEARCH, ev);
    }
    VS_TRY(run_post_search(ix, bp, d_out_ids, d_out_tids, d_out_dist));
    return enqueue_reduce(ix, bp);
}

static void update_scan_obs(vs_index* ix, double sum, double max, uint32_t n_fast, uint32_t n_over, uint32_t nq, uint32_t L, uint32_t M) {
    ScanObs& o = ix->obs;
    const bool same = o.valid && o.L == L && o.M == M;
    const double a = same ? 0.5 : 1.0;
    o.ins_mean = (1 - a) * o.ins_mean + a * (sum / n_fast);
    o.ins_max = same ? std::max(o.ins_max, max) : max;
    o.ov_frac = (1 - a) * (same ? o.ov_frac : 0.0) + a * ((double)n_over / nq);
    o.L = L;
    o.M = M;
    o.valid = true;
}

static int collect_stats_reduced(vs_index* ix, uint32_t nq, uint32_t M, uint32_t rescore, bool stream_only, vs_stats* st, uint32_t obs_L) {
    if (!st) return VS_OK;
    const SearchWorkspace& w = ix->ws;
    const uint64_t* r = w.red_host;
    if (w.fb_valid && ix->last_ins_limit && r[RED_INS_FAST])
        update_scan_obs(ix, (double)r[RED_INS_SUM], (double)r[RED_INS_MAX], (uint32_t)r[RED_INS_FAST], (uint32_t)r[RED_INS_OV], nq, obs_L, M);
    st->queries += nq;
    st->visited_nodes += r[RED_VISITS];
    st->candidate_nodes += r[RED_CAND];
    if (ix->d.storage_type == VS_STORAGE_PLAIN) st->full_distance_comparisons += r[RED_DQ];
    else st->quantized_distance_comparisons += r[RED_DQ];
    st->node_reads += r[RED_READS];
    st->next_calls += r[RED_NEXT];
    st->fallback_scans += r[RED_FB_SCANS];
    st->fallback_visited_nodes += r[RED_FB_VISITS];
    st->fallback_quantized_distance_comparisons += r[RED_FB_DQ];
    if (!stream_only && rescore > 0) {
        st->full_distance_comparisons += r[RED_HEAP_ROWS];
        st->node_heap_reads += r[RED_HEAP_ROWS];
    }
    return VS_OK;
}

static int dump_phase_clocks(vs_index* ix, uint32_t nq, const std::vector<uint32_t>& hs) {
    std::vector<uint64_t> ph((size_t)nq * 8);
    VS_HIP(hipMemcpy(ph.data(), ix->ws.phase.p, ph.size() * 8, hipMemcpyDeviceToHost));
    double sum[8] = {0};
    uint64_t visits = 0;
    for (uint32_t q = 0; q < nq; ++q) {
        for (int k = 0; k < 8; ++k) sum[k] += (double)ph[(size_t)q * 8 + k];
        visits += hs[(size_t)q * ST_N + ST_VISITS];
    }
    const char* names[8] = {"pop", "row_wait", "visited", "dedup", "gather", "push", "other", "-"};
    fprintf(stderr, "[VS_PHASE] shader clocks per visit:");
    for (int k = 0; k < 7; ++k) fprintf(stderr, " %s=%.0f", names[k], sum[k] / (double)std::max<uint64_t>(visits, 1));
    fprintf(stderr, "\n");
    return VS_OK;
}

static int collect_stats(vs_index* ix, uint32_t nq, uint32_t M, uint32_t rescore, bool stream_only, vs_stats* st,
                         uint32_t obs_L = 0) {
    if (!st) return VS_OK;
    SearchWorkspace& w = ix->ws;
    std::vector<uint32_t> hs((size_t)nq * ST_N), cnt(nq), fb(nq, 0);
    VS_HIP(hipMemcpyAsync(hs.data(), w.stats.p, hs.size() * 4, hipMemcpyDeviceToHost, ix->ctx->stream));
    if (w.fb_valid) VS_HIP(hipMemcpyAsync(fb.data(), w.fb_flag.p, fb.size() * 4, hipMemcpyDeviceToHost, ix->ctx->stream));
    VS_HIP(hipMemcpyAsync(cnt.data(), w.stream_cnt.p, cnt.size() * 4, hipMemcpyDeviceToHost, ix->ctx->stream));
    VS_HIP(hipStreamSynchronize(ix->ctx->stream));
    if (env_u32("VS_PHASE", 0) && w.phase.p && w.fb_valid) VS_TRY(dump_phase_clocks(ix, nq, hs));
    if (w.fb_valid && ix->last_ins_limit) {
        double sum = 0, mx = 0;
        uint32_t cnt_fast = 0, ov = 0;
        for (uint32_t q = 0; q < nq; ++q) {
            const double v = hs[(size_t)q * ST_N + ST_INS];
            if (fb[q]) {
                ov++;
                mx = std::max(mx, v);
                continue;
            }
            sum += v;
            mx = std::max(mx, v);
            cnt_fast++;
            ov += v > ix->last_ins_limit;
        }
        if (cnt_fast) update_scan_obs(ix, sum, mx, cnt_fast, ov, nq, obs_L, M);
    }
    for (uint32_t q = 0; q < nq; ++q) {
        st->queries++;
        st->visited_nodes += hs[(size_t)q * ST_N + ST_VISITS];
        st->candidate_nodes += hs[(size_t)q * ST_N + ST_CAND];
        if (ix->d.storage_type == VS_STORAGE_PLAIN) st->full_distance_comparisons += hs[(size_t)q * ST_N + ST_DQ];
        else st->quantized_distance_comparisons += hs[(size_t)q * ST_N + ST_DQ];
        st->node_reads += hs[(size_t)q * ST_N + ST_READS];
        uint64_t next_calls = hs[(size_t)q * ST_N + ST_NEXT];
        if (!stream_only && rescore > 0 && cnt[q] < M && next_calls > 0) {
            const int64_t C = cnt[q], S = rescore, kk = (int64_t)M - rescore + 1;
            const int64_t J = std::min<int64_t>(kk, C + 1), j0 = std::max<int64_t>(1, C - S + 2);
            next_calls = next_calls - 1 + (uint64_t)std::max<int64_t>(J - j0 + 1, 1);
        }
        st->next_calls += next_calls;
        if (fb[q]) {
            st->fallback_scans++;
            st->fallback_visited_nodes += hs[(size_t)q * ST_N + ST_VISITS];
            st->fallback_quantized_distance_comparisons += hs[(size_t)q * ST_N + ST_DQ];
        }
        if (!stream_only && rescore > 0) {
            const uint32_t nr = std::min(cnt[q], M) + (ix->visible ? hs[(size_t)q * ST_N + ST_INVIS] : 0u);
            st->full_distance_comparisons += nr;
            st->node_heap_reads += nr;
        }
    }
    return VS_OK;
}

static int finish_launch(vs_index* ix, const BatchPlan& bp, const int16_t* d_qlabels, const uint32_t* d_qlabel_off, Caps& caps,
                         uint32_t* d_out_ids, uint64_t* d_out_tids, float* d_out_dist, vs_stats* st) {
    vs_ctx* c = ix->ctx;
    SearchWorkspace& w = ix->ws;
    VS_REQUIRE(w.red_host, "finish: no launch to finish");
    VS_HIP(hipStreamSynchronize(c->stream));
    if (w.red_host[RED_STATUS]) {
        VS_TRY(retry_failed_scans(ix, bp, d_qlabels, d_qlabel_off, caps, st));
        VS_TRY(run_post_search(ix, bp, d_out_ids, d_out_tids, d_out_dist));
        VS_TRY(enqueue_reduce(ix, bp));
        VS_HIP(hipStreamSynchronize(c->stream));
    }
    if (env_u32("VS_PHASE", 0)) return collect_stats(ix, bp.nq, bp.M, bp.rescore, bp.stream_only, st, bp.L);
    return collect_stats_reduced(ix, bp.nq, bp.M, bp.rescore, bp.stream_only, st, bp.L);
}

static uint32_t stream_len(uint32_t rescore, uint32_t k) { return rescore > 0 ? rescore + k - 1 : k; }

static uint32_t chunk_queries(const vs_index* ix, const Caps& c, uint32_t M, uint32_t nq) {
    const size_t general = (size_t)c.hashcap * 4 + (size_t)(c.hcap > c.hl ? c.hcap - c.hl : 0) * 8;
    size_t per_q = (size_t)M * 12 + ix->vec_stride * 4ull + ix->code_stride * 8ull + 256;
    const bool persist = c.f_on && knob_u32("VS_F_PERSIST", ix->tune.persist, 1);
    size_t fixed = 0;
    if (persist) {
        fixed = (size_t)ix->ctx->prop.multiProcessorCount * 32 * ((size_t)c.f_gcap * 4 + (size_t)c.f_gstride * 4);
        per_q += general / 64 + 64;
    } else if (c.f_on) {
        per_q += (size_t)((double)c.f_gcap * 4 * c.f_pool_frac) + (size_t)c.f_gstride * 4 + general / 64 + 64;
    } else {
        per_q += general;
    }
    size_t budget = 24ull << 30;
    size_t free_b = 0, total_b = 0;
    if (hipMemGetInfo(&free_b, &total_b) == hipSuccess) {
        const SearchWorkspace& w = ix->ws;
        const size_t held = w.hash.bytes + w.heap_g.bytes + w.heap_g4.bytes + w.ghash4.bytes + w.stream_ids.bytes +
                            w.stream_ham.bytes + w.rr_dist.bytes + w.q_full.bytes + w.qcodes.bytes;
        budget = std::min<size_t>((free_b + held) / 2, 64ull << 30);
        budget = std::max<size_t>(budget, 1ull << 30);
    }
    budget = budget > fixed + (budget >> 2) ? budget - fixed : budget >> 2;
    uint32_t m = (uint32_t)std::max<size_t>(1, std::min<size_t>(budget / per_q, 1u << 20));
    return std::min(m, nq);
}

static int upload_label_keys(vs_index* ix, const int16_t* qlabels, const uint32_t* qlabel_off, uint32_t nq,
                             const int16_t** d_labels, const uint32_t** d_off) {
    *d_labels = nullptr;
    *d_off = nullptr;
    if (!qlabel_off) return VS_OK;
    VS_REQUIRE(ix->d.has_labels && ix->label_off, "label scan keys on an index without labels");
    std::vector<int16_t> vals;
    std::vector<uint32_t> off(nq + 1, 0);
    for (uint32_t q = 0; q < nq; ++q) {
        VS_REQUIRE(qlabel_off[q] <= qlabel_off[q + 1], "qlabel_off must be non-decreasing");
        std::vector<int16_t> l(qlabels + qlabel_off[q], qlabels + qlabel_off[q + 1]);
        std::sort(l.begin(), l.end());
        l.erase(std::unique(l.begin(), l.end()), l.end());
        vals.insert(vals.end(), l.begin(), l.end());
        off[q + 1] = (uint32_t)vals.size();
    }
    SearchWorkspace& w = ix->ws;
    VS_TRY(devbuf_reserve(ix->ctx, w.qlabels, std::max<size_t>(vals.size(), 1) * 2));
    VS_TRY(devbuf_reserve(ix->ctx, w.qlabel_off, off.size() * 4));
    if (!vals.empty()) VS_TRY(vs_dev_upload(ix->ctx, w.qlabels.p, vals.data(), vals.size() * 2));
    VS_TRY(vs_dev_upload(ix->ctx, w.qlabel_off.p, off.data(), off.size() * 4));
    *d_labels = (const int16_t*)w.qlabels.p;
    *d_off = (const uint32_t*)w.qlabel_off.p;
    return VS_OK;
}

static int search_host(vs_index* ix, const float* queries, const int16_t* qlabels, const uint32_t* qlabel_off,
                       uint32_t nq, uint32_t L, uint32_t rescore, uint32_t k, bool stream_only, uint32_t* out_ids,
                       uint64_t* out_tids, float* out_dist, uint32_t* out_ham, vs_stats* stats) {
    VS_REQUIRE(ix && (nq == 0 || queries), "search: bad args");
    VS_REQUIRE(L >= 1 && L <= 10000, "diskann.query_search_list_size %u outside [1,10000]", L);
    VS_REQUIRE(rescore <= 1000, "diskann.query_rescore %u outside [0,1000]", rescore);
    VS_REQUIRE(k >= 1, "k must be >= 1");
    if (ix->d.storage_type == VS_STORAGE_PLAIN) {
        VS_REQUIRE(!qlabel_off, "Plain storage does not support label filters");
        if (ix->d.dim_index == ix->d.dim_full) rescore = 0;
    }
    if (stats) memset(stats, 0, sizeof(*stats));
    if (nq == 0) return VS_OK;
    vs_ctx* c = ix->ctx;
    VS_HIP(hipSetDevice(c->device));
    SearchWorkspace& w = ix->ws;
    const uint32_t M = stream_only ? k : stream_len(rescore, k);
    Caps caps = initial_caps(ix, L, M);
    const int16_t* d_labels_all = nullptr;
    const uint32_t* d_off_all = nullptr;
    VS_TRY(upload_label_keys(ix, qlabels, qlabel_off, nq, &d_labels_all, &d_off_all));
    uint32_t chunk = chunk_queries(ix, caps, M, nq);
    {
        const uint32_t want = std::max<uint32_t>(env_u32("VS_HOST_CHUNKS", 4), 1);
        const uint32_t floor_q = env_u32("VS_HOST_CHUNK_MIN", 32768);
        const uint32_t piece = std::max<uint32_t>((nq + want - 1) / want, floor_q);
        chunk = std::min(chunk, std::max<uint32_t>(piece, 1));
    }
    const size_t qrow = (size_t)ix->d.dim_full * 4;
    DevBuf* rawq[2] = {&w.raw_q, &w.raw_q2};
    DevBuf* oids[2] = {&w.out_ids, &w.out_ids2};
    DevBuf* otids[2] = {&w.out_tids, &w.out_tids2};
    DevBuf* odist[2] = {&w.out_dist, &w.out_dist2};
    const uint32_t nchunks = (nq + chunk - 1) / chunk;
    auto cq_of = [&](uint32_t ci) { return std::min(chunk, nq - ci * chunk); };
    auto stage_in = [&](uint32_t ci) -> int {
        const uint32_t cq = cq_of(ci);
        VS_TRY(devbuf_reserve(c, *rawq[ci & 1], (size_t)chunk * qrow));
        return vs_dev_upload(c, rawq[ci & 1]->p, queries + (size_t)ci * chunk * ix->d.dim_full, (size_t)cq * qrow);
    };
    auto launch = [&](uint32_t ci, BatchPlan& bp) -> int {
        const uint32_t cq = cq_of(ci), q0 = ci * chunk;
        VS_TRY(devbuf_reserve(c, *oids[ci & 1], (size_t)chunk * k * 4));
        VS_TRY(devbuf_reserve(c, *otids[ci & 1], (size_t)chunk * k * 8));
        VS_TRY(devbuf_reserve(c, *odist[ci & 1], (size_t)chunk * k * 4));
        bp = BatchPlan{cq, L, rescore, k, M, stream_only};
        return run_search_chunk(ix, bp, (const float*)rawq[ci & 1]->p, d_labels_all, d_off_all ? d_off_all + q0 : nullptr,
                                (uint32_t*)oids[ci & 1]->p, (uint64_t*)otids[ci & 1]->p, (float*)odist[ci & 1]->p, caps);
    };
    auto finish = [&](uint32_t ci, const BatchPlan& bp) -> int {
        const uint32_t q0 = ci * chunk;
        return finish_launch(ix, bp, d_labels_all, d_off_all ? d_off_all + q0 : nullptr, caps, (uint32_t*)oids[ci & 1]->p,
                             (uint64_t*)otids[ci & 1]->p, (float*)odist[ci & 1]->p, stats);
    };
    auto stage_out = [&](uint32_t ci) -> int {
        const uint32_t cq = cq_of(ci), q0 = ci * chunk;
        if (stream_only) {
            VS_TRY(vs_dev_download(c, out_ids + (size_t)q0 * k, w.stream_ids.p, (size_t)cq * k * 4));
            if (out_ham) {
                VS_TRY(vs_dev_download(c, out_ham + (size_t)q0 * k, w.stream_ham.p, (size_t)cq * k * 4));
                if (ix->d.storage_type == VS_STORAGE_PLAIN)
                    for (size_t i = (size_t)q0 * k; i < ((size_t)q0 + cq) * k; ++i)
                        if (out_ids[i] != VS_INVALID_NODE) {
                            int32_t b = (int32_t)(out_ham[i] ^ 0x80000000u);
                            b ^= (int32_t)(((uint32_t)(b >> 31)) >> 1);
                            out_ham[i] = (uint32_t)b;
                        }
            }
            return VS_OK;
        }
        VS_TRY(download_async_rows(c, out_ids + (size_t)q0 * k, oids[ci & 1]->p, (size_t)cq * k * 4));
        if (out_tids) VS_TRY(download_async_rows(c, out_tids + (size_t)q0 * k, otids[ci & 1]->p, (size_t)cq * k * 8));
        if (out_dist) VS_TRY(download_async_rows(c, out_dist + (size_t)q0 * k, odist[ci & 1]->p, (size_t)cq * k * 4));
        return VS_OK;
    };
    BatchPlan bp_cur{}, bp_next{};
    VS_TRY(stage_in(0));
    VS_TRY(launch(0, bp_cur));
    for (uint32_t ci = 0; ci < nchunks; ++ci) {
        if (ci + 1 < nchunks) VS_TRY(stage_in(ci + 1));
        VS_TRY(finish(ci, bp_cur));
        if (stream_only) VS_TRY(stage_out(ci));
        if (ci + 1 < nchunks) VS_TRY(launch(ci + 1, bp_next));
        if (!stream_only) VS_TRY(stage_out(ci));
        bp_cur = bp_next;
    }
    if (stats) ix->last_stats = *stats;
    return VS_OK;
}

static int vs_search_batch_impl(vs_index* ix, const float* queries, const int16_t* qlabels, const uint32_t* qlabel_off,
                               uint32_t nq, uint32_t L, uint32_t rescore, uint32_t k, uint32_t* out_ids,
                               uint64_t* out_tids, float* out_dist, vs_stats* stats) {
    VS_REQUIRE(nq == 0 || out_ids, "vs_search_batch: out_ids is NULL");
    return search_host(ix, queries, qlabels, qlabel_off, nq, L, rescore, k, false, out_ids, out_tids, out_dist, nullptr,
                       stats);
}
extern "C" int vs_search_batch(vs_index* ix, const float* queries, const int16_t* qlabels, const uint32_t* qlabel_off,
                               uint32_t nq, uint32_t L, uint32_t rescore, uint32_t k, uint32_t* out_ids,
                               uint64_t* out_tids, float* out_dist, vs_stats* stats) {
    return vs_guard("vs_search_batch", [&] { return vs_search_batch_impl(ix, queries, qlabels, qlabel_off, nq, L, rescore, k, out_ids, out_tids, out_dist, stats); });
}


static int vs_stream_batch_impl(vs_index* ix, const float* queries, const int16_t* qlabels, const uint32_t* qlabel_off,
                               uint32_t nq, uint32_t L, uint32_t m, uint32_t* out_ids, uint32_t* out_ham, vs_stats* stats) {
    VS_REQUIRE(nq == 0 || out_ids, "vs_stream_batch: out_ids is NULL");
    return search_host(ix, queries, qlabels, qlabel_off, nq, L, 0, m, true, out_ids, nullptr, nullptr, out_ham, stats);
}
extern "C" int vs_stream_batch(vs_index* ix, const float* queries, const int16_t* qlabels, const uint32_t* qlabel_off,
                               uint32_t nq, uint32_t L, uint32_t m, uint32_t* out_ids, uint32_t* out_ham, vs_stats* stats) {
    return vs_guard("vs_stream_batch", [&] { return vs_stream_batch_impl(ix, queries, qlabels, qlabel_off, nq, L, m, out_ids, out_ham, stats); });
}


int vs_search_batch_dev_impl(vs_index* ix, const float* d_queries, const int16_t* d_qlabels,
                                   const uint32_t* d_qlabel_off, uint32_t nq, uint32_t L, uint32_t rescore, uint32_t k,
                                   uint32_t* d_out_ids, uint64_t* d_out_tids, float* d_out_dist) {
    VS_REQUIRE(ix && (nq == 0 || (d_queries && d_out_ids)), "vs_search_batch_dev: bad args");
    VS_REQUIRE(L >= 1 && L <= 10000 && rescore <= 1000 && k >= 1, "vs_search_batch_dev: GUC out of range");
    if (ix->d.storage_type == VS_STORAGE_PLAIN) {
        VS_REQUIRE(!d_qlabel_off, "Plain storage does not support label filters");
        if (ix->d.dim_index == ix->d.dim_full) rescore = 0;
    }
    SearchWorkspace& w = ix->ws;
    w.pending = false;
    if (nq == 0) return VS_OK;
    VS_HIP(hipSetDevice(ix->ctx->device));
    const uint32_t M = stream_len(rescore, k);
    Caps caps = initial_caps(ix, L, M);
    VS_REQUIRE(chunk_queries(ix, caps, M, nq) == nq, "vs_search_batch_dev: batch of %u queries exceeds the workspace budget", nq);
    BatchPlan bp{nq, L, rescore, k, M, false};
    VS_TRY(run_search_chunk(ix, bp, d_queries, d_qlabels, d_qlabel_off, d_out_ids, d_out_tids, d_out_dist, caps));
    w.pending = true;
    w.pend = PendingBatch{bp, caps, d_qlabels, d_qlabel_off, d_out_ids, d_out_tids, d_out_dist};
    ix->last_stats = vs_stats{};
    return VS_OK;
}
extern "C" int vs_search_batch_dev(vs_index* ix, const float* d_queries, const int16_t* d_qlabels,
                                   const uint32_t* d_qlabel_off, uint32_t nq, uint32_t L, uint32_t rescore, uint32_t k,
                                   uint32_t* d_out_ids, uint64_t* d_out_tids, float* d_out_dist) {
    return vs_guard("vs_search_batch_dev", [&] { return vs_search_batch_dev_impl(ix, d_queries, d_qlabels, d_qlabel_off, nq, L, rescore, k, d_out_ids, d_out_tids, d_out_dist); });
}


int vs_search_batch_dev_finish_impl(vs_index* ix, vs_stats* stats) {
    VS_REQUIRE(ix, "vs_search_batch_dev_finish: index is NULL");
    SearchWorkspace& w = ix->ws;
    if (!w.pending) {
        vs_set_error("vs_search_batch_dev_finish: no batch in flight");
        return VS_ERR_STATE;
    }
    w.pending = false;
    PendingBatch pb = w.pend;
    vs_stats st{};
    VS_TRY(finish_launch(ix, pb.bp, pb.d_qlabels, pb.d_qlabel_off, pb.caps, pb.d_out_ids, pb.d_out_tids, pb.d_out_dist, &st));
    ix->last_stats = st;
    if (stats) *stats = st;
    return VS_OK;
}
extern "C" int vs_search_batch_dev_finish(vs_index* ix, vs_stats* stats) {
    return vs_guard("vs_search_batch_dev_finish", [&] { return vs_search_batch_dev_finish_impl(ix, stats); });
}
```

pgvectorscale_amd/csrc/vs_internal.h:

```cpp
#pragma once
#include <hip/hip_runtime.h>

#include <cstdint>
#include <cstdio>
#include <cstring>
#include <string>
#include <atomic>
#include <mutex>
#include <vector>

#include "../../include/vsgpu.h"

#define VS_EMPTY 0xFFFFFFFFu

void vs_set_error(const char* fmt, ...);
const char* vs_opt_get(const char* name);

#define VS_HIP(expr)                                                                                   \
    do {                                                                                               \
        hipError_t _e = (expr);                                                                        \
        if (_e != hipSuccess) {                                                                        \
            vs_set_error("%s failed: %s (%s:%d)", #expr, hipGetErrorString(_e), __FILE__, __LINE__);   \
            return (_e == hipErrorOutOfMemory) ? VS_ERR_OOM : VS_ERR_HIP;                              \
        }                                                                                              \
    } while (0)

#define VS_REQUIRE(cond, ...)         \
    do {                              \
        if (!(cond)) {                \
            vs_set_error(__VA_ARGS__);\
            return VS_ERR_INVALID;    \
        }                             \
    } while (0)

#define VS_REQUIRE_OOM(cond, ...)     \
    do {                              \
        if (!(cond)) {                \
            vs_set_error(__VA_ARGS__);\
            return VS_ERR_OOM;        \
        }                             \
    } while (0)

#define VS_TRY(expr)            \
    do {                        \
        int _r = (expr);        \
        if (_r != VS_OK) return _r; \
    } while (0)

#include <exception>
#include <new>
template <class F>
static inline int vs_guard(const char* what, F&& f) {
    try {
        return f();
    } catch (const std::bad_alloc&) {
        vs_set_error("%s: out of host memory", what);
        return VS_ERR_OOM;
    } catch (const std::exception& e) {
        vs_set_error("%s: %s", what, e.what());
        return VS_ERR_INVALID;
    }
}

__host__ __device__ static inline uint32_t round_up_u32(uint32_t x, uint32_t m) { return (x + m - 1) / m * m; }
static inline uint32_t next_pow2_u32(uint64_t x) {
    uint64_t p = 1;
    while (p < x) p <<= 1;
    return (uint32_t)p;
}

struct vs_ctx {
    int device = -1;
    hipStream_t stream = nullptr;
    hipStream_t copy_stream = nullptr;
    void* pinned[2] = {nullptr, nullptr};
    size_t pinned_bytes = 0;
    hipEvent_t pinned_ev[2] = {nullptr, nullptr};
    hipDeviceProp_t prop;
    bool profiling = false;
    struct ProfSpan { int kind; hipEvent_t a, b; };
    std::vector<ProfSpan> spans;
    std::vector<hipEvent_t> event_pool;
    double prof_ms[8] = {0};
    uint64_t prof_launches[8] = {0};
};
enum { PK_PREPARE = 0, PK_SEARCH = 1, PK_RERANK = 2, PK_RESORT = 3, PK_SEARCH_FB = 4, PK_SCAN = 5, PK_ORDER = 6, PK_PAGES = 7 };
hipEvent_t prof_begin(vs_ctx* c);
void prof_end(vs_ctx* c, int kind, hipEvent_t a);

struct DevBuf {
    void* p = nullptr;
    size_t bytes = 0;
    bool in_slab = false;
};

struct WsSlab {
    std::mutex mu;
    void* base[2] = {nullptr, nullptr};
    size_t bytes[2] = {0, 0}, used[2] = {0, 0};
    void* owned[2] = {nullptr, nullptr};
    int refs = 1;
    int device = 0;
    bool tried = false;
    bool external = false;
};

struct Caps {
    uint32_t hl, hcap, vcap, lh, hashcap, g0;
    bool f_on;
    uint32_t f_hl, f_hcap, f_gstride, f_lh, f_gcap, f_sb, f_vr, f_vcap;
    double f_pool_frac;
};
struct BatchPlan {
    uint32_t nq, L, rescore, k, M;
    bool stream_only;
};
struct PendingBatch {
    BatchPlan bp;
    Caps caps;
    const int16_t* d_qlabels;
    const uint32_t* d_qlabel_off;
    uint32_t* d_out_ids;
    uint64_t* d_out_tids;
    float* d_out_dist;
};

struct SearchWorkspace {
    DevBuf q_full, qcodes, qlabels, qlabel_off, hash, heap_g, heap_g4, ghash4, heap_g4b, ghash4b, pool_ctr, fb_flag, phase, timeline, stream_ids, stream_ham, stream_cnt, stats, status,
        rr_dist, out_ids, out_tids, out_dist, resort_heap, raw_q, misc, q_index,
        raw_q2, out_ids2, out_tids2, out_dist2,
        red,
        order_work, order_perm,
        order_labels;
    uint32_t order_nq = 0;
    uint32_t lab_rows = 0, lab_S = 0, lab_step = 0;
    uint64_t lab_epoch = 0;
    uint64_t* red_host = nullptr;
    bool fb_valid = false;
    bool pending = false;
    PendingBatch pend{};
};

struct ScanObs {
    bool valid = false;
    uint32_t L = 0, M = 0;
    double ins_mean = 0, ins_max = 0;
    double ov_frac = 1.0;
};

struct TuneVariant {
    int virgin = -1, minw = -1, persist = -1;
    int lds_max_ins = -1;
    int vr = -1;
    uint32_t gcap = 0;
    char name[40] = "default";
};
struct FastSig {
    uint32_t vwords = 0, minw = 0, gcap = 0, lh = 0, vr = 0, ran = 0;
    bool operator==(const FastSig& o) const {
        return vwords == o.vwords && minw == o.minw && gcap == o.gcap && lh == o.lh && vr == o.vr && ran == o.ran;
    }
};

struct vs_index {
    vs_ctx* ctx = nullptr;
    bool is_view = false;
    bool uploaded = false;
    vs_index* view_of = nullptr;
    uint64_t owner_id = 0;
    WsSlab* slab = nullptr;
    vs_index_desc d{};
    uint32_t capacity = 0;
    uint32_t code_stride = 0;
    uint32_t nbr_stride = 0;
    uint32_t vec_stride = 0;
    uint64_t* codes = nullptr;
    uint64_t codes_epoch = 0;
    uint32_t* nbrs = nullptr;
    uint64_t* tids = nullptr;
    double insert_ms[3] = {0, 0, 0};
    double build_ms[3] = {0, 0, 0};
    double consolidate_ms[2] = {0, 0};
    double compact_ms[2] = {0, 0};
    double label_repair_ms[4] = {0, 0, 0, 0};
    uint32_t build_unreachable = 0;
    const uint8_t* visible = nullptr;
    uint8_t* visible_own = nullptr;
    uint8_t* snap[VS_MAX_SNAPSHOTS] = {nullptr};
    float* vecs = nullptr;
    float* vnorm = nullptr;
    float* vnorm_idx = nullptr;
    float* mean = nullptr;
    float* m2 = nullptr;
    uint64_t count = 0;
    uint32_t* label_off = nullptr;
    int16_t* label_val = nullptr;
    uint64_t* label_mask = nullptr;
    uint8_t* label_bit = nullptr;
    uint64_t* nbr_mask = nullptr;
    bool nbr_mask_valid = false;
    bool nbr_mask_tried = false;
    uint64_t n_label_vals = 0;
    int16_t* ls_labels = nullptr;
    uint32_t* ls_nodes = nullptr;
    SearchWorkspace ws;
    ScanObs obs;
    uint32_t last_ins_limit = 0;
    TuneVariant tune;
    FastSig last_fast;
    vs_stats last_stats{};
};

struct DeviceOnce {
    std::atomic<uint64_t> mask{0};
    bool pending(int device) const { return device < 0 || device >= 64 || !((mask.load(std::memory_order_acquire) >> device) & 1ull); }
    void done(int device) {
        if (device >= 0 && device < 64) mask.fetch_or(1ull << device, std::memory_order_acq_rel);
    }
};
int devbuf_reserve(vs_ctx* ctx, DevBuf& b, size_t bytes);
int devbuf_reserve_hot(vs_index* ix, DevBuf& b, size_t bytes, int which);
uint64_t vs_new_owner_id();
WsSlab* vs_slab_new(int device);
void vs_slab_release(WsSlab* s);
int vs_index_live_views(vs_index* ix);
int vs_index_open_writers(const vs_index* ix);
void vs_index_writer_opened(uint64_t owner_id);
void vs_index_writer_closed(uint64_t owner_id);
#define VS_REQUIRE_OWNER(ix, what)                                                                                                     \
    do {                                                                                                                                \
        if ((ix)->is_view) {                                                                                                            \
            vs_set_error("%s: this handle is a view; the arrays belong to the index it was made from", what);                         \
            return VS_ERR_STATE;                                                                                                        \
        }                                                                                                                               \
    } while (0)
#define VS_REQUIRE_NO_VIEWS(ix, what)                                                                                                  \
    do {                                                                                                                                \
        const int _nv = vs_index_live_views(ix);                                                                                        \
        if (_nv > 0) {                                                                                                                  \
            vs_set_error("%s: %d view(s) of this index are alive (cursor lanes, a second stream, a vs_multi shard) and hold its device " \
                         "pointers; free them first",                                                                                  \
                         what, _nv);                                                                                                    \
            return VS_ERR_STATE;                                                                                                        \
        }                                                                                                                               \
    } while (0)
int vs_index_reserve_impl(vs_index* ix, uint32_t capacity, const char* what);
int vs_upload_rows(vs_ctx* c, void* dst, size_t dev_row_bytes, const void* src, size_t host_row_bytes, size_t copy_bytes, size_t rows);
int vs_validate_graph(vs_index* ix);
bool vs_neighbor_masks_wanted(const vs_index* ix);
int vs_refresh_neighbor_masks(vs_index* ix);
int vs_refresh_label_masks(vs_index* ix);
void devbuf_free(DevBuf& b);
static inline uint32_t env_u32(const char* name, uint32_t dflt) {
    const char* v = vs_opt_get(name);
    return v && *v ? (uint32_t)strtoul(v, nullptr, 10) : dflt;
}
size_t slab_bytes_wanted(const vs_index* ix);
void slab_select(vs_index* ix, WsSlab* s, size_t slab_bytes);
hipEvent_t pool_event(vs_ctx* c);
int download_async_rows(vs_ctx* c, void* dst, const void* src, size_t bytes);
void stage_copy(void* dst, const void* src, size_t n);
int vs_search_batch_dev_impl(vs_index* ix, const float* d_queries, const int16_t* d_qlabels, const uint32_t* d_qlabel_off, uint32_t nq,
                             uint32_t L, uint32_t rescore, uint32_t k, uint32_t* d_out_ids, uint64_t* d_out_tids, float* d_out_dist);
int vs_search_batch_dev_finish_impl(vs_index* ix, vs_stats* stats);

struct SearchLaunch {
    uint32_t nq, L, M;
    uint32_t hl;
    uint32_t hcap;
    uint32_t vcap;
    uint32_t lh;
    uint32_t hashcap;
    uint32_t g0;
    const uint64_t* qcodes;
    const int16_t* qlabels;
    const uint32_t* qlabel_off;
    uint64_t* heap_g;
    uint32_t* hash;
    uint32_t* out_ids;
    uint32_t* out_ham;
    uint32_t* out_cnt;
    uint32_t* stats;
    uint32_t* status;
    uint32_t only_failed = 0;
    uint32_t* pool_counter = nullptr;
    uint32_t pool_slots = 0;
    uint32_t* fb_flag = nullptr;
    const uint8_t* visible = nullptr;
    uint32_t* resume = nullptr;
    uint32_t resume_stride = 0;
    uint32_t* row_stats = nullptr;
};
enum { RS_INIT = 0, RS_HLEN, RS_HMAX, RS_VLEN, RS_GLEV, RS_NINS_L, RS_NINS_G, RS_NINS_TOP, RS_VISITS, RS_CAND, RS_DQ, RS_READS,
       RS_NEXT, RS_INVIS, RS_STATUS, RS_EMITTED, RS_HDR = 16 };
size_t search_resume_words(const SearchLaunch& s);
struct FastLaunch {
    uint32_t nq, L, M;
    uint32_t hl;
    uint32_t hcap;
    uint32_t gstride;
    uint32_t lh;
    uint32_t gcap;
    uint32_t glimit = 0;
    uint32_t sb;
    uint32_t vr;
    uint32_t vcap;
    uint32_t minw;
    uint32_t rc = 0;
    uint32_t persist = 0;
    uint32_t vwords = 0;
    uint32_t vslot = 0;
    uint32_t qd = 0, qk = 0, ocap = 0, gregion = 0;
    uint32_t build = 0;
    uint32_t flags = 0;
    uint32_t only_failed = 0;
    uint32_t* fb_flag = nullptr;
    const uint8_t* visible = nullptr;
    const uint64_t* qcodes;
    const int16_t* qlabels;
    const uint32_t* qlabel_off;
    uint32_t* heap_g;
    uint32_t* ghash;
    uint32_t* pool_counter;
    uint32_t pool_slots;
    uint32_t* out_ids;
    uint32_t* out_ham;
    uint32_t* out_cnt;
    uint32_t* stats;
    uint32_t* status;
    uint64_t* phase = nullptr;
    uint32_t* scan_counter = nullptr;
    uint64_t* timeline = nullptr;
    uint32_t* resume = nullptr;
    uint32_t resume_stride = 0;
    uint32_t* row_stats = nullptr;
};
enum { RSF_INIT = 0, RSF_HLEN, RSF_VHEAD, RSF_VLEN, RSF_NINS_G, RSF_N_OVF, RSF_HMAX, RSF_VISITS, RSF_CAND, RSF_POPS, RSF_INVIS, RSF_STATUS,
       RSF_NEXT, RSF_ENDED, RSF_HDR = 16 };
size_t fast_resume_words(const FastLaunch& s);
enum {
    FAST_FULL_VARIANT = 8,
};
size_t fast_lds_bytes(const vs_index* idx, const FastLaunch& s);
static inline bool fast_tables16_geometry(const vs_index* idx, FastLaunch& f) {
    uint32_t qd = 1, lb = 0;
    while ((1ull << qd) < (uint64_t)(idx->d.n > 2 ? idx->d.n : 2)) qd++;
    while ((1u << lb) < (f.gcap >> 3)) lb++;
    if (qd < lb + 3) qd = lb + 3;
    f.qd = qd;
    f.qk = qd - lb;
    const uint32_t o = round_up_u32(f.gcap / 16, 32);
    f.ocap = o > 256 ? o : 256;
    f.vwords = (f.gcap + f.ocap) / 32;
    f.vslot = 2;
    f.gregion = (f.gcap >> 1) + f.ocap;
    f.sb = 0;
    while ((1ull << f.sb) < (uint64_t)f.gcap + f.ocap) f.sb++;
    const uint64_t nbits = (uint64_t)idx->d.dim_index * idx->d.bits;
    return f.qk <= 16 && f.qd <= 32 && nbits < (1ull << (32 - f.sb));
}
int launch_search_fast(vs_index* idx, const FastLaunch& s);
int fast_resident_scans(vs_index* idx, const FastLaunch& s, uint32_t* out);
enum { ST_VISITS = 0, ST_CAND = 1, ST_DQ = 2, ST_READS = 3, ST_NEXT = 4, ST_GSPILL = 5, ST_INVIS = 6, ST_INS = 7 , ST_N = 8 };
enum { OVF_HEAP = 1, OVF_VISITED = 2, OVF_HASH = 4, OVF_POOL = 8,
       OVF_KEY = 16 };
size_t search_lds_bytes(const vs_index* idx, const SearchLaunch& s);

int launch_prepare_queries(vs_index* idx, const float* d_raw, uint32_t nq, float* d_q_full, uint64_t* d_qcodes);
int launch_quantize_rows(vs_index* idx, const float* d_rows, uint32_t row_stride, uint32_t nrows, uint64_t* d_codes,
                         uint32_t code_stride);
int launch_hamming_gather(vs_index* idx, const uint64_t* d_qcodes, const uint32_t* d_ids, const uint32_t* d_off,
                          uint32_t nq, uint32_t* d_out);
int launch_rerank(vs_index* idx, const float* d_q_full, const uint32_t* d_ids, const uint32_t* d_off,
                  const uint32_t* d_cnt, uint32_t fixed_m, uint32_t nq, float* d_out, uint32_t row_base = 0,
                  const uint32_t* d_perm = nullptr, bool deal = false);
int launch_search(vs_index* idx, const SearchLaunch& s, bool build_mode = false);
int launch_resort(vs_index* idx, uint32_t nq, uint32_t M, uint32_t rescore, uint32_t k, const uint32_t* d_stream_ids,
                  const uint32_t* d_cnt, const float* d_dist, uint64_t* d_heap_ws, uint32_t* d_out_ids,
                  uint64_t* d_out_tids, float* d_out_dist);
bool rerank_window_fits(const vs_index* idx, uint32_t M, uint32_t rescore, uint32_t k);
int launch_rerank_window(vs_index* idx, const float* d_q_full, const uint32_t* d_stream_ids, const uint32_t* d_cnt, uint32_t M,
                         uint32_t rescore, uint32_t k, uint32_t nq, uint32_t* d_out_ids, uint64_t* d_out_tids, float* d_out_dist,
                         uint32_t mode, const uint32_t* d_perm = nullptr, bool deal = false);
bool scan_order_fits(const vs_index* idx);
size_t scan_order_work_bytes(uint32_t nq, uint32_t S);
int launch_scan_order(vs_index* idx, const uint64_t* d_qcodes, uint32_t nq, uint32_t S, uint32_t* d_work, uint32_t* d_perm);
int launch_region_labels(vs_index* idx, uint32_t S, uint32_t seed_step, uint32_t row_begin, uint32_t rows, uint16_t* d_labels);
int launch_label_order(vs_index* idx, const uint16_t* d_labels, uint32_t lab_rows, uint32_t S, const uint32_t* d_stream_ids,
                       const uint32_t* d_cnt, uint32_t M, uint32_t nq, uint32_t* d_work, uint32_t* d_perm);
enum { RED_STATUS = 0, RED_VISITS, RED_CAND, RED_DQ, RED_READS, RED_NEXT, RED_FB_SCANS, RED_FB_VISITS, RED_FB_DQ, RED_HEAP_ROWS,
       RED_INS_SUM, RED_INS_MAX, RED_INS_FAST, RED_INS_OV, RED_N = 16 };
int launch_reduce_stats(vs_index* idx, const uint32_t* d_stats, const uint32_t* d_fb, const uint32_t* d_cnt, const uint32_t* d_status,
                        uint32_t nq, uint32_t M, uint32_t rescore, bool windowed, uint32_t ins_limit, uint64_t* d_red);
int launch_resort_cursor(vs_index* idx, uint32_t n, bool exhausted, uint32_t rescore, uint32_t k, const uint32_t* d_stream,
                         const float* d_dist, const uint32_t* d_keys, uint64_t* d_heap, uint32_t* d_cur, uint32_t* d_out_ids,
                         uint64_t* d_out_tids, float* d_out_dist);
int launch_resort_cursor_batch(vs_index* idx, uint32_t n, const uint32_t* d_list, uint32_t rescore, uint32_t k, const uint32_t* d_stream,
                               const float* d_dist, const uint32_t* d_keys, uint32_t row_stride, uint64_t* d_heap, uint32_t* d_cur,
                               uint32_t* d_out_ids, uint64_t* d_out_tids, float* d_out_dist, uint32_t out_stride);
int launch_pool_append(vs_index* idx, uint32_t nq, const uint32_t* d_cnt, const uint32_t* d_off, const uint32_t* d_stage, uint32_t stage_kind_stride, uint32_t M,
                       uint32_t* d_all, uint32_t all_kind_stride, uint32_t rows_cap);
int launch_row_norms(vs_index* idx);
int launch_row_norms_range(vs_index* idx, uint32_t row_begin, uint32_t rows);
int vs_quantize_row_range(vs_index* ix, uint32_t row_begin, uint32_t rows);
int launch_slice_norms(vs_index* idx, float* d_out);
int launch_prepare_index_slice(vs_index* idx, const float* d_raw, uint32_t nq, float* d_q_index, uint32_t raw_stride = 0);
int launch_slice_norms_range(vs_index* idx, uint32_t row_begin, uint32_t rows);
int launch_validate_nbrs(vs_index* idx, uint32_t* d_flag);
int launch_scan_topk(vs_index* idx, const uint64_t* d_qcodes, uint32_t nq, uint32_t k, uint32_t* d_out_ids,
                     uint32_t* d_out_ham, const int16_t* d_qlabels = nullptr, const uint32_t* d_qlabel_off = nullptr,
                     bool live_only = false);
```

pgvectorscale_amd/csrc/vs_kernels.hip:

```cpp
#include "vs_internal.h"
#include "vs_device.h"

__device__ void lds_preprocess_cosine(float* buf, uint32_t n, int lane, uint32_t stride, float* bcast , bool active = true) {
    __syncthreads();
    if (active && lane == 0) {
        float norm = 0.0f;
        for (uint32_t i = 0; i < n; ++i) {
            float p = buf[i] * buf[i];
            norm = norm + p;
        }
        const float eps = 1.1920929e-07f;
        float adj = eps * (float)n;
        float s = 0.0f;
        if (!(norm < eps) && !(norm >= 1.0f - adj && norm <= 1.0f + adj)) s = sqrtf(norm);
        *bcast = s;
    }
    __syncthreads();
    if (active) {
        float s = *bcast;
        if (s != 0.0f)
            for (uint32_t i = lane; i < n; i += stride) buf[i] = buf[i] / s;
    }
    __syncthreads();
}

__device__ void wave_quantize(const float* v, uint32_t dims, uint32_t bits, const float* __restrict__ mean,
                              const float* __restrict__ m2, float count_f, uint64_t* out, uint32_t words,
                              uint32_t out_stride, int lane) {
    for (uint32_t w = 0; w < out_stride; ++w) {
        uint64_t word = 0;
        if (w < words) {
            uint32_t g = w * 64u + (uint32_t)lane;
            uint32_t dim = g / bits;
            uint32_t j = g - dim * bits;
            bool bit = false;
            if (dim < dims) {
                float x = v[dim];
                float mu = mean[dim];
                if (bits == 1) {
                    bit = x > mu;
                } else {
                    float variance = m2[dim] / count_f;
                    float std_dev = sqrtf(variance);
                    float ranges = (float)(bits + 1);
                    float z = (x - mu) / std_dev;
                    float index = (z + 2.0f) / (4.0f / ranges);
                    uint32_t ones = 0;
                    if (!(index < 1.0f)) {
                        float fl = floorf(index);
                        if (fl != fl) ones = 0;
                        else if (fl >= (float)bits) ones = bits;
                        else if (fl <= 0.0f) ones = 0;
                        else ones = (uint32_t)fl;
                    }
                    bit = j < ones;
                }
            }
            word = __ballot(bit);
        }
        if (lane == 0) out[w] = word;
    }
}

__global__ __launch_bounds__(256) void k_prepare_queries(const float* __restrict__ raw, uint32_t nq,
                                                         uint32_t dim_full, uint32_t dim_index, uint32_t vec_stride,
                                                         uint32_t distance_type, uint32_t bits,
                                                         const float* __restrict__ mean, const float* __restrict__ m2,
                                                         float count_f, uint32_t words, uint32_t code_stride, uint32_t rounds,
                                                         uint32_t vec4, float* __restrict__ q_full, uint64_t* __restrict__ qcodes) {
    extern __shared__ __attribute__((aligned(16))) unsigned char smem[];
    const int lane = threadIdx.x & 63, wave = threadIdx.x >> 6;
    const uint32_t nw = blockDim.x >> 6;
    const bool same = dim_full == dim_index;
    const bool quant = words != 0, multi = quant && bits != 1;
    const uint32_t rf = round_up_u32(dim_full, 4), ri = round_up_u32(dim_index, 4);
    float* mu = reinterpret_cast<float*>(smem);
    float* sdv = mu + (quant ? ri : 0u);
    float* wbase = sdv + (multi ? ri : 0u);
    const uint32_t per_wave = rf + (same ? 0u : ri) + (multi ? ri : 0u) + 4u;
    float* full = wbase + (size_t)wave * per_wave;
    float* idxv = same ? full : full + rf;
    uint32_t* ones = reinterpret_cast<uint32_t*>((same ? full : idxv) + (same ? rf : ri));
    float* bc = reinterpret_cast<float*>(ones + (multi ? ri : 0u));
    if (quant)
        for (uint32_t i = threadIdx.x; i < dim_index; i += blockDim.x) {
            mu[i] = mean[i];
            if (multi) {
                float variance = m2[i] / count_f;
                sdv[i] = sqrtf(variance);
            }
        }
    for (uint32_t r = 0; r < rounds; ++r) {
        const uint32_t q = (blockIdx.x * rounds + r) * nw + (uint32_t)wave;
        const bool active = q < nq;
        __syncthreads();
        if (active) {
            const float* src = raw + (size_t)q * dim_full;
            if (vec4) {
                for (uint32_t i = lane; i < dim_full / 4; i += WAVE)
                    reinterpret_cast<float4*>(full)[i] = reinterpret_cast<const float4*>(src)[i];
            } else {
                for (uint32_t i = lane; i < rf; i += WAVE) full[i] = i < dim_full ? src[i] : 0.0f;
            }
            if (!same)
                for (uint32_t i = lane; i < dim_index; i += WAVE) idxv[i] = src[i];
        }
        if (distance_type == VS_COSINE) {
            lds_preprocess_cosine(full, dim_full, lane, WAVE, bc, active);
            if (!same) lds_preprocess_cosine(idxv, dim_index, lane, WAVE, bc, active);
        } else {
            __syncthreads();
        }
        if (active) {
            float* qf = q_full + (size_t)q * vec_stride;
            for (uint32_t i = lane; i < vec_stride / 4; i += WAVE) reinterpret_cast<float4*>(qf)[i] = reinterpret_cast<const float4*>(full)[i];
            if (multi) {
                const float ranges = (float)(bits + 1);
                for (uint32_t dim = lane; dim < dim_index; dim += WAVE) {
                    float x = idxv[dim];
                    float z = (x - mu[dim]) / sdv[dim];
                    float index = (z + 2.0f) / (4.0f / ranges);
                    uint32_t o = 0;
                    if (!(index < 1.0f)) {
                        float fl = floorf(index);
                        if (fl != fl) o = 0;
                        else if (fl >= (float)bits) o = bits;
                        else if (fl <= 0.0f) o = 0;
                        else o = (uint32_t)fl;
                    }
                    ones[dim] = o;
                }
            }
        }
        __syncthreads();
        if (active) {
            uint64_t* out = qcodes + (size_t)q * code_stride;
            uint64_t mine = 0;
            for (uint32_t w = 0; w < code_stride; ++w) {
                uint64_t word = 0;
                if (w < words) {
                    const uint32_t g = w * 64u + (uint32_t)lane;
                    const uint32_t dim = g / bits;
                    const uint32_t j = g - dim * bits;
                    bool bit = false;
                    if (dim < dim_index) bit = multi ? j < ones[dim] : idxv[dim] > mu[dim];
                    word = __ballot(bit);
                }
                if ((uint32_t)lane == (w & 63u)) mine = word;
                if ((w & 63u) == 63u || w + 1 == code_stride) {
                    const uint32_t w0 = w & ~63u;
                    if (w0 + (uint32_t)lane <= w) out[w0 + lane] = mine;
                }
            }
        }
    }
}

__global__ __launch_bounds__(WAVE) void k_prepare_index_slice(const float* __restrict__ raw, uint32_t nq, uint32_t dim_full,
                                                              uint32_t dim_index, uint32_t vec_stride, uint32_t distance_type,
                                                              float* __restrict__ q_index) {
    extern __shared__ __attribute__((aligned(16))) unsigned char smem[];
    float* idxv = reinterpret_cast<float*>(smem);
    float* bc = idxv + round_up_u32(dim_index, 4);
    const int lane = threadIdx.x;
    const uint32_t q = blockIdx.x;
    if (q >= nq) return;
    for (uint32_t i = lane; i < dim_index; i += WAVE) idxv[i] = raw[(size_t)q * dim_full + i];
    __syncthreads();
    if (distance_type == VS_COSINE) lds_preprocess_cosine(idxv, dim_index, lane, blockDim.x, bc);
    for (uint32_t i = lane; i < vec_stride; i += WAVE) q_index[(size_t)q * vec_stride + i] = i < dim_index ? idxv[i] : 0.0f;
}

__global__ __launch_bounds__(WAVE) void k_quantize_rows(const float* __restrict__ rows, uint32_t row_stride,
                                                        uint32_t nrows, uint32_t dims, uint32_t bits,
                                                        const float* __restrict__ mean, const float* __restrict__ m2,
                                                        float count_f, uint32_t words, uint32_t code_stride,
                                                        uint64_t* __restrict__ codes) {
    const int lane = threadIdx.x;
    for (uint32_t r = blockIdx.x; r < nrows; r += gridDim.x)
        wave_quantize(rows + (size_t)r * row_stride, dims, bits, mean, m2, count_f, codes + (size_t)r * code_stride,
                      words, code_stride, lane);
}

__global__ __launch_bounds__(WAVE) void k_hamming_gather(const uint64_t* __restrict__ codes, uint32_t code_stride,
                                                         const uint64_t* __restrict__ qcodes,
                                                         const uint32_t* __restrict__ ids,
                                                         const uint32_t* __restrict__ off, uint32_t nq,
                                                         uint32_t* __restrict__ out) {
    extern __shared__ __attribute__((aligned(16))) unsigned char smem[];
    uint64_t* qc = reinterpret_cast<uint64_t*>(smem);
    const int lane = threadIdx.x;
    const uint32_t q = blockIdx.x;
    if (q >= nq) return;
    for (uint32_t w = lane; w < code_stride; w += WAVE) qc[w] = qcodes[(size_t)q * code_stride + w];
    __syncthreads();
    const uint32_t b = off[q], e = off[q + 1];
    for (uint32_t base = b; base < e; base += 16) {
        uint32_t j = base + (uint32_t)(lane >> 2);
        bool valid = j < e;
        uint32_t id = valid ? ids[j] : 0;
        uint32_t d = ham_row4(codes + (size_t)id * code_stride, qc, lane & 3, code_stride, valid);
        if (valid && (lane & 3) == 0) out[j] = d;
    }
}

__device__ __forceinline__ float shfl_f(float v, int src) { return __shfl(v, src, WAVE); }

__device__ __forceinline__ float rerank_row_dist(const float* __restrict__ row, const float* qv, float s, uint32_t distance_type,
                                                 uint32_t steps, uint32_t dim_full, int lane, int l8, bool valid) {
    float a0 = 0.f, a1 = 0.f, a2 = 0.f, a3 = 0.f;
    if (valid) {
        if (distance_type == VS_L2) {
            for (uint32_t t = 0; t < steps; ++t) {
                float4 x = *reinterpret_cast<const float4*>(row + 32 * t + 4 * l8);
                float4 y = *reinterpret_cast<const float4*>(qv + 32 * t + 4 * l8);
                float d0 = x.x - y.x, d1 = x.y - y.y, d2 = x.z - y.z, d3 = x.w - y.w;
                float p0 = d0 * d0, p1 = d1 * d1, p2 = d2 * d2, p3 = d3 * d3;
                a0 = a0 + p0;
                a1 = a1 + p1;
                a2 = a2 + p2;
                a3 = a3 + p3;
            }
        } else {
            for (uint32_t t = 0; t < steps; ++t) {
                float4 x = *reinterpret_cast<const float4*>(row + 32 * t + 4 * l8);
                float4 y = *reinterpret_cast<const float4*>(qv + 32 * t + 4 * l8);
                if (s != 0.0f) {
                    x.x = x.x / s;
                    x.y = x.y / s;
                    x.z = x.z / s;
                    x.w = x.w / s;
                }
                a0 = __builtin_fmaf(x.x, y.x, a0);
                a1 = __builtin_fmaf(x.y, y.y, a1);
                a2 = __builtin_fmaf(x.z, y.z, a2);
                a3 = __builtin_fmaf(x.w, y.w, a3);
            }
        }
    }
    float s0 = a0 + shfl_f(a0, lane ^ 1);
    float s1 = a1 + shfl_f(a1, lane ^ 1);
    float s2 = a2 + shfl_f(a2, lane ^ 1);
    float s3 = a3 + shfl_f(a3, lane ^ 1);
    float t0 = s0 + s1;
    float t1 = s2 + s3;
    float h = t0 + t1;
    const int g0 = lane & ~7;
    float h0 = shfl_f(h, g0 + 0), h1 = shfl_f(h, g0 + 2), h2 = shfl_f(h, g0 + 4), h3 = shfl_f(h, g0 + 6);
    float dist = h0 + h1;
    dist = dist + h2;
    dist = dist + h3;
    float r = dist;
    if (valid && l8 == 0) {
        for (uint32_t i = steps * 32; i < dim_full; ++i) {
            float x = row[i];
            if (distance_type == VS_L2) {
                float diff = x - qv[i];
                float p = diff * diff;
                dist = dist + p;
            } else {
                if (s != 0.0f) x = x / s;
                float p = x * qv[i];
                dist = dist + p;
            }
        }
        if (distance_type == VS_L2) r = dist;
        else if (distance_type == VS_IP) r = -dist;
        else r = fmaxf(1.0f - dist, 0.0f);
// ... 911 lines not shown
```

pgvectorscale_amd/csrc/vs_search_fast.hip:

```cpp
#ifndef VS_FAST_TU
#define VS_FAST_TU 0
#endif
#include <cstdlib>

#include "vs_device.h"

#define MAX_QLABELS 64
#define VS_Q16_A 0x9E3779B1u
#define VS_Q16_B 0x85EBCA6Bu
#define VS_Q16_AI 0x0E8B2F51u
#define VS_Q16_BI 0xA5CB9243u
static_assert((uint32_t)(VS_Q16_A * VS_Q16_AI) == 1u && (uint32_t)(VS_Q16_B * VS_Q16_BI) == 1u, "inverse multipliers");
#define ARB_SLOTS 128

struct FastArgs {
    const uint64_t* codes;
    const uint32_t* nbrs;
    const uint64_t* tids;
    const uint32_t* label_off;
    const int16_t* label_val;
    const uint64_t* label_mask;
    const uint8_t* label_bit;
    const uint64_t* nbr_mask;
    const int16_t* ls_labels;
// ... 427 lines not shown
                    const uint32_t gi = (uint32_t)r * 64u + (uint32_t)lane;
                    idx += (uint32_t)__popcll(__ballot(gi < len && h[r] < hd));
                }
            }
#pragma unroll
            for (int r = NR - 1; r >= 0; --r) {
                if ((uint32_t)r * 64u <= len && (uint32_t)r * 64u + 63u >= idx) {
                    const uint32_t ch = r > 0 ? readlane_u32(h[r > 0 ? r - 1 : 0], 63) : 0u;
                    const uint32_t cn = r > 0 ? readlane_u32(n[r > 0 ? r - 1 : 0], 63) : 0u;
                    const uint32_t sh = wave_shr1(h[r], ch), sn = wave_shr1(n[r], cn);
                    const uint32_t gi = (uint32_t)r * 64u + (uint32_t)lane;
                    h[r] = gi > idx ? sh : (gi == idx ? hd : h[r]);
                    n[r] = gi > idx ? sn : (gi == idx ? node : n[r]);
                }
            }
            len++;
            return;
        }
        if (len < WAVE) {
            const uint32_t x = head + (uint32_t)lane;
            const uint32_t sl = x >= vcapv ? x - vcapv : x;
            uint64_t e = ~0ull;
            if ((uint32_t)lane < len) e = ring[sl];
            const bool lt = (uint32_t)lane < len && ((uint32_t)(e >> 32) & VIS_HAM_MASK) < hd;
            const uint32_t idx = (uint32_t)__popcll(__ballot(lt));
            const uint32_t plo = wave_shr1((uint32_t)e, 0), phi = wave_shr1((uint32_t)(e >> 32), 0);
            const uint64_t nw = ((uint64_t)(hd | (flags << 30)) << 32) | node;
            if ((uint32_t)lane >= idx && (uint32_t)lane <= len) ring[sl] = (uint32_t)lane == idx ? nw : (((uint64_t)phi << 32) | plo);
            len++;
            wave_sync();
            return;
        }
        uint32_t idx = 0;
        for (uint32_t base = 0; base < len; base += WAVE) {
            const uint32_t i = base + lane;
            const bool lt = i < len && ((uint32_t)(ring[slot(i)] >> 32) & VIS_HAM_MASK) < hd;
            idx += (uint32_t)__popcll(__ballot(lt));
        }
        if (2 * idx < len) {
            for (uint32_t base = 0; base < idx; base += WAVE) {
                const uint32_t i = base + lane;
                uint64_t e = 0;
                if (i < idx) e = ring[slot(i)];
                wave_sync();
                if (i < idx) ring[slot(i - 1)] = e;
                wave_sync();
            }
            head = head ? head - 1 : vcapv - 1;
        } else {
            uint32_t hi = len;
            while (hi > idx) {
                const uint32_t lo = (hi - idx > WAVE) ? hi - WAVE : idx;
                const uint32_t i = lo + lane;
                uint64_t e = 0;
                if (i < hi) e = ring[slot(i)];
                wave_sync();
                if (i < hi) ring[slot(i + 1)] = e;
                wave_sync();
                hi = lo;
            }
        }
        if (lane == 0) ring[slot(idx)] = ((uint64_t)(hd | (flags << 30)) << 32) | node;
        len++;
        wave_sync();
    }
    __device__ __forceinline__ void pop_front(uint32_t& hd, uint32_t& node, uint32_t& flags) {
        flags = 0;
        if (VR > 0) {
            hd = readlane_u32(h[0], 0);
            node = readlane_u32(n[0], 0);
#pragma unroll
            for (int r = 0; r < NR; ++r) {
                if ((uint32_t)r * 64u < len) {
                    const uint32_t ch = r + 1 < NR ? readlane_u32(h[r + 1 < NR ? r + 1 : 0], 0) : 0u;
                    const uint32_t cn = r + 1 < NR ? readlane_u32(n[r + 1 < NR ? r + 1 : 0], 0) : 0u;
                    h[r] = wave_shl1(h[r], ch);
                    n[r] = wave_shl1(n[r], cn);
                }
            }
            len--;
            return;
        }
        const uint64_t front = ring[head];
        hd = rfl((uint32_t)(front >> 32));
        flags = hd >> 30;
        hd &= VIS_HAM_MASK;
        node = rfl((uint32_t)front);
        head = head + 1 == vcapv ? 0 : head + 1;
        len--;
    }
};

template <int NCH, bool QL = false, bool XW = false>
__device__ __forceinline__ uint32_t ham_row_reg(const uint64_t* __restrict__ row, const ulonglong2 (&qv)[NCH > 0 ? NCH : 1],
                                                const uint64_t* qc_l, int l4, uint32_t code_stride, bool active, bool stream) {
    uint32_t acc = 0;
    if (NCH > 0) {
        if (active) {
            ulonglong2 r[NCH > 0 ? NCH : 1];
#pragma unroll
            for (int t = 0; t < NCH; ++t) {
                const uint32_t w = 2u * (uint32_t)l4 + 8u * (uint32_t)t;
                r[t] = (!XW && w >= code_stride) ? make_ulonglong2(0, 0)
                       : stream ? load_stream16(row + w) : *reinterpret_cast<const ulonglong2*>(row + w);
            }
#pragma unroll
            for (int t = 0; t < NCH; ++t) {
                const ulonglong2 qq = QL ? *reinterpret_cast<const ulonglong2*>(qc_l + 2u * (uint32_t)l4 + 8u * (uint32_t)t) : qv[t];
                acc += (uint32_t)__popcll(r[t].x ^ qq.x) + (uint32_t)__popcll(r[t].y ^ qq.y);
            }
        }
        return quad_sum(acc);
    }
    return ham_row4(row, qc_l, l4, code_stride, active);
}

template <int NCH, bool QL = false>
__device__ __forceinline__ void ham_row_reg2(const uint64_t* __restrict__ row_a, const uint64_t* __restrict__ row_b,
                                             const ulonglong2 (&qv)[NCH > 0 ? NCH : 1], const uint64_t* qc_l, int l4, uint32_t code_stride, bool act_a,
                                             bool act_b, bool stream, uint32_t& da, uint32_t& db) {
    constexpr int N = NCH > 0 ? NCH : 1;
    ulonglong2 ra[N], rb[N];
#pragma unroll
    for (int t = 0; t < N; ++t) {
        const uint32_t w = 2u * (uint32_t)l4 + 8u * (uint32_t)t;
        const bool in = w < code_stride;
        ra[t] = !(act_a && in) ? make_ulonglong2(0, 0) : stream ? load_stream16(row_a + w) : *reinterpret_cast<const ulonglong2*>(row_a + w);
        rb[t] = !(act_b && in) ? make_ulonglong2(0, 0) : stream ? load_stream16(row_b + w) : *reinterpret_cast<const ulonglong2*>(row_b + w);
    }
    uint32_t acc_a = 0, acc_b = 0;
#pragma unroll
    for (int t = 0; t < N; ++t) {
        const ulonglong2 qq = QL ? *reinterpret_cast<const ulonglong2*>(qc_l + 2u * (uint32_t)l4 + 8u * (uint32_t)t) : qv[t];
        acc_a += (uint32_t)__popcll(ra[t].x ^ qq.x) + (uint32_t)__popcll(ra[t].y ^ qq.y);
        acc_b += (uint32_t)__popcll(rb[t].x ^ qq.x) + (uint32_t)__popcll(rb[t].y ^ qq.y);
    }
    da = quad_sum(act_a ? acc_a : 0u);
    db = quad_sum(act_b ? acc_b : 0u);
}

__device__ __forceinline__ uint32_t wave_min_u32(uint32_t v) {
    v = min(v, (uint32_t)__builtin_amdgcn_update_dpp(-1, (int)v, 0x111 , 0xF, 0xF, false));
    v = min(v, (uint32_t)__builtin_amdgcn_update_dpp(-1, (int)v, 0x112 , 0xF, 0xF, false));
    v = min(v, (uint32_t)__builtin_amdgcn_update_dpp(-1, (int)v, 0x114 , 0xF, 0xF, false));
    v = min(v, (uint32_t)__builtin_amdgcn_update_dpp(-1, (int)v, 0x118 , 0xF, 0xF, false));
    return min(min(readlane_u32(v, 15), readlane_u32(v, 31)), min(readlane_u32(v, 47), readlane_u32(v, 63)));
}

#define OPT_XW 1
#define OPT_R1 2
#define OPT_NS64 4
#define OPT_RS 8
#define OPT_G2 16
template <int NCH, int VR, bool TIMING, int MINW, bool BUILD, bool FULL, int VG, int OPT>
__device__ __forceinline__ void fast_scan(const FastArgs& a, const uint32_t q, const uint32_t slot) {
    constexpr bool XW = (OPT & OPT_XW) != 0 && NCH > 0;
    constexpr bool R1 = (OPT & OPT_R1) != 0;
    constexpr bool RS = (OPT & OPT_RS) != 0;
    static_assert(!RS || (VG == 3 && VR == 0 && !BUILD), "resumable scans: 16-bit tables, LDS-ring visited list");
    const uint64_t* const codes_v = FULL ? a.codes : in_vgpr(a.codes);
    const uint32_t* const nbrs_v = FULL ? a.nbrs : in_vgpr(a.nbrs);
    const uint64_t* const tids_v = FULL ? a.tids : in_vgpr(a.tids);
    const uint32_t cstride = XW ? 8u * (uint32_t)NCH : a.code_stride;
    const uint32_t nstride = (OPT & OPT_NS64) ? 64u : a.nbr_stride;
    const uint32_t R_v = in_vgpr(a.R);
    extern __shared__ __attribute__((aligned(16))) unsigned char smem[];
    int lane_v = threadIdx.x;
    asm volatile("" : "+v"(lane_v));
    int lane = lane_v;
    const FastLaunch& s = a.s;
    const uint32_t lhv = VG ? 0u : s.lh;
    const uint32_t onlyfv = VG ? 0u : s.only_failed;
    const uint32_t rcv = VG >= 2 ? 0u : s.rc;
    if (onlyfv && s.status[q] == 0) return;
    if (RS && s.status[q] == 0) return;
    uint32_t* const rs = RS ? s.resume + (size_t)q * s.resume_stride : nullptr;
    const bool resumed = RS && rfl(rs[RSF_INIT]) == 1u;
    if (s.timeline && lane == 0) s.timeline[2 * (size_t)q] = wall_clock64();

    constexpr bool LEAN = MINW == 7 && VG == 3;
    constexpr bool QL = NCH > 0 && MINW >= 6;
    uint32_t* surv_id = reinterpret_cast<uint32_t*>(smem);
    uint32_t* surv_slot = surv_id + 64;
    uint32_t* surv_d = LEAN ? surv_slot : surv_slot + 64;
    uint32_t* arb = surv_d + 64;
    constexpr uint32_t ARB_N = VG >= 2 ? 0u : (uint32_t)ARB_SLOTS;
    uint64_t* qc_fix = reinterpret_cast<uint64_t*>(arb + ARB_N);
    int16_t* ql = reinterpret_cast<int16_t*>(qc_fix + (QL ? 8 * NCH : 0));
    uint32_t* hp = reinterpret_cast<uint32_t*>(ql + (LEAN && !FULL ? 0 : MAX_QLABELS));
    uint32_t* lhash = hp + (s.hl + 1);
    uint64_t* ring = reinterpret_cast<uint64_t*>(lhash + lhv);
    uint32_t* rc = reinterpret_cast<uint32_t*>(ring + (VR > 0 ? 0 : s.vcap));
    const uint32_t rcm = rcv - 1u;
    uint32_t* vmap = rc + rcv;
    uint64_t* qc_l = QL ? qc_fix : reinterpret_cast<uint64_t*>(smem + ((((vmap + s.vwords) - reinterpret_cast<uint32_t*>(smem)) * 4u + 15u) & ~15u));

    int l4 = lane & 3;
    constexpr bool stream_rows = true;
    constexpr bool G2 = NCH == 3 && VR == 0 && (MINW == 5 || (OPT & OPT_G2) != 0) && !BUILD && !TIMING;
    ulonglong2 qv[NCH > 0 ? NCH : 1];
    if (QL) {
        qv[0] = make_ulonglong2(0, 0);
        for (uint32_t w = lane; w < 8u * (uint32_t)NCH; w += WAVE)
            qc_l[w] = w < a.code_stride ? s.qcodes[(size_t)q * cstride + w] : 0ull;
    } else if (NCH > 0) {
#pragma unroll
        for (int t = 0; t < NCH; ++t) {
            const uint32_t w = 2u * (uint32_t)l4 + 8u * (uint32_t)t;
            qv[t] = w < a.code_stride
                        ? *reinterpret_cast<const ulonglong2*>(s.qcodes + (size_t)q * cstride + w)
                        : make_ulonglong2(0, 0);
        }
    } else {
        for (uint32_t w = lane; w < a.code_stride; w += WAVE) qc_l[w] = s.qcodes[(size_t)q * cstride + w];
    }
    for (uint32_t i = 4u * lane; i < lhv; i += 4u * WAVE)
        *reinterpret_cast<uint4*>(lhash + i) = make_uint4(VS_EMPTY, VS_EMPTY, VS_EMPTY, VS_EMPTY);
    if (lane == 0 && !resumed) hp[0] = 0;
    for (uint32_t i = lane; i < ARB_N; i += WAVE) arb[i] = 0;
    for (uint32_t i = lane; i < rcv; i += WAVE) rc[i] = VS_EMPTY;
    if (VG && !resumed)
        for (uint32_t i = lane; i < s.vwords; i += WAVE) vmap[i] = 0;
    const uint32_t image_words = RS ? (uint32_t)((vmap + s.vwords) - hp) : 0u;
    if (resumed)
        for (uint32_t i = 4u * lane; i < image_words; i += 4u * WAVE) *reinterpret_cast<uint4*>(hp + i) = *reinterpret_cast<const uint4*>(rs + RSF_HDR + i);
    const uint8_t* const visible = FULL ? s.visible : nullptr;
    const bool labels_some = FULL && s.qlabel_off != nullptr;
    uint32_t nql = 0;
    bool wide_key = false;
    if (labels_some) {
        const uint32_t lb = s.qlabel_off[q], le = s.qlabel_off[q + 1];
        wide_key = le - lb > (uint32_t)MAX_QLABELS;
        nql = min(le - lb, (uint32_t)MAX_QLABELS);
        for (uint32_t i = lane; i < nql; i += WAVE) ql[i] = s.qlabels[lb + i];
    }
    const bool has_label_filter = labels_some && nql > 0;
    wave_sync();
    uint64_t qmask = 0;
    if (has_label_filter && a.label_mask) {
        uint64_t mine = 0;
        if ((uint32_t)lane < nql) {
            const uint32_t bit = a.label_bit[(uint16_t)ql[lane]];
            if (bit < 64u) mine = 1ull << bit;
        }
        for (int o = 32; o >= 1; o >>= 1) mine |= __shfl_xor(mine, o, WAVE);
        qmask = mine;
    }

    FastHeap<(MINW >= 7)> heap;
    heap.l = hp;
    heap.g = (s.persist || RS) ? s.heap_g + (size_t)slot * s.gstride : (onlyfv ? s.heap_g : s.heap_g + (size_t)q * s.gstride);
    heap.hl = s.hl;
    heap.sb = s.sb;
    heap.init(lane);
    Visited<VR> vis;
    vis.init(lane, ring, VR > 0 ? 64u * VR : s.vcap);

    const uint32_t slot_limit = lhv - lhv / 8;
    const uint32_t smask = (1u << s.sb) - 1u;
    uint32_t emitted = 0, status = wide_key ? (uint32_t)OVF_KEY : 0u, nins = 0, hmax = 0;
    uint32_t st_visits = 0, st_cand = 0, st_pops = 0;
    uint64_t ph[8] = {0, 0, 0, 0, 0, 0, 0, 0};
    uint64_t tmark = TIMING ? __builtin_readcyclecounter() : 0;
    auto lap = [&](int k) {
        if (TIMING) {
            const uint64_t now = __builtin_readcyclecounter();
            ph[k] += now - tmark;
            tmark = now;
        }
    };

    uint32_t* ghash = s.ghash;
    const uint32_t gbuckets = s.gcap >> 2;
    uint32_t nins_g = 0;
    bool g_open = false, region = false;
    auto claim_region = [&]() -> bool {
        if (region) return true;
        if (s.persist || RS) {
            region = true;
            ghash = s.ghash + (size_t)slot * (VG == 3 ? s.gregion : s.gcap);
            return true;
        }
        uint32_t pslot = 0;
        if (lane == 0) pslot = atomicAdd(s.pool_counter, 1u);
        pslot = rfl(pslot);
        if (pslot >= s.pool_slots) {
            status |= OVF_POOL;
            return false;
        }
        region = true;
        ghash = s.ghash + (size_t)pslot * (VG == 3 ? s.gregion : s.gcap);
        if (onlyfv) heap.g = s.heap_g + (size_t)pslot * s.gstride;
        return true;
    };
    auto hash_home = [&](uint32_t nid) -> uint32_t { return (uint32_t)(((uint64_t)hash_u32(nid) * lhv) >> 32); };
    auto g_empty = [&](uint32_t v) -> bool { return v == VS_EMPTY; };
    const uint32_t qdm = in_vgpr(VG == 3 ? (s.qd >= 32 ? 0xFFFFFFFFu : (1u << s.qd) - 1u) : 0u);
    const uint32_t qxs = in_vgpr((s.qd + 1u) >> 1);
    const uint32_t qk_v = in_vgpr(s.qk), rmask_v = in_vgpr((1u << s.qk) - 1u);
    const uint32_t ovf_lim_v = in_vgpr(s.ocap - s.ocap / 4);
    auto q_fwd = [&](uint32_t id) -> uint32_t {
        uint32_t x = (id * VS_Q16_A) & qdm;
        x ^= x >> qxs;
        x = (x * VS_Q16_B) & qdm;
        x ^= x >> qxs;
        return x;
    };
    auto q_inv = [&](uint32_t x) -> uint32_t {
        x ^= x >> qxs;
        x = (x * VS_Q16_BI) & qdm;
        x ^= x >> qxs;
        return (x * VS_Q16_AI) & qdm;
    };
    auto node_load = [&](uint32_t handle) -> uint32_t {
        if (VG == 3) {
            if (handle < s.gcap) return gload16(reinterpret_cast<const uint16_t*>(ghash) + handle);
            return gload32(ghash + (s.gcap >> 1) + (handle - s.gcap));
        }
        if (handle < lhv) return lload32(lhash + handle);
        return gload32(ghash + (handle - lhv));
    };
    auto node_of = [&](uint32_t handle, uint32_t raw) -> uint32_t {
        if (VG == 3 && handle < s.gcap) return rfl(q_inv(((handle >> 3) << qk_v) | raw));
        return raw;
    };
    auto finish_insert = [&](uint32_t nid, bool act, uint32_t slot, uint32_t old, uint32_t& slot_out) -> bool {
        bool fresh = false;
        if (act) {
            for (;;) {
                if (old == VS_EMPTY) { fresh = true; break; }
                if (old == nid) break;
                slot = slot + 1 == lhv ? 0 : slot + 1;
                old = atomicCAS(&lhash[slot], VS_EMPTY, nid);
            }
            slot_out = slot;
        }
        nins += (uint32_t)__popcll(__ballot(fresh));
        return fresh;
    };
    const bool gmode = lhv == 0;
    auto ghash_home = [&](uint32_t nid) -> uint32_t {
        return (uint32_t)(((uint64_t)hash_u32(nid ^ 0x5bd1e995u) * gbuckets) >> 32) << 2;
    };
    auto bucket_load = [&](uint32_t b0) -> uint4 { return *reinterpret_cast<const uint4*>(ghash + b0); };
    auto bucket_fetch = [&](uint32_t b0, bool& virgin) -> uint4 {
        if (VG) {
            const uint32_t b = b0 >> 2;
            virgin = ((vmap[b >> 5] >> (b & 31u)) & 1u) == 0;
            if (virgin) return make_uint4(VS_EMPTY, VS_EMPTY, VS_EMPTY, VS_EMPTY);
        }
        return bucket_load(b0);
// ... 197 lines not shown
        if (!claim_region()) return false;
        g_open = true;
        if (!VG) {
            for (uint32_t i = 4u * lane; i < s.gcap; i += 4u * WAVE)
                *reinterpret_cast<uint4*>(ghash + i) = make_uint4(VS_EMPTY, VS_EMPTY, VS_EMPTY, VS_EMPTY);
            wave_sync();
        }
        return true;
    };
    auto frozen_insert = [&](uint32_t nid, bool act, uint32_t& slot_out) -> bool {
        bool need_g = act;
        if (act && lhv) {
            uint32_t slot = hash_home(nid);
            for (;;) {
                const uint32_t v = lhash[slot];
                if (v == nid) { need_g = false; break; }
                if (v == VS_EMPTY) break;
                slot = slot + 1 == lhv ? 0 : slot + 1;
            }
        }
        if (!__ballot(need_g)) return false;
        if (!open_table()) return false;
        if (nins_g > s.glimit) {
            status |= OVF_HASH;
            return false;
        }
        if (VG == 3) return b16_insert(nid, need_g, q_fwd(nid), make_uint4(0, 0, 0, 0), 0u, false, slot_out);
        if (VG == 2) return slot_insert(nid, need_g, slot_home(nid), make_uint4(0, 0, 0, 0), 0u, slot_out);
        const uint32_t b0 = ghash_home(nid);
        uint4 v = make_uint4(0, 0, 0, 0);
        bool virgin = false;
        if (need_g) v = bucket_fetch(b0, virgin);
        return global_insert(nid, need_g, b0, v, virgin, slot_out);
    };

    if (status) {  }
    else if (gmode) open_table();
    else if (onlyfv) claim_region();
    uint32_t next_base = 0, invis_base = 0;
    bool ended = false;
    if (resumed) {
        heap.len = rfl(rs[RSF_HLEN]);
        vis.head = rfl(rs[RSF_VHEAD]);
        vis.len = rfl(rs[RSF_VLEN]);
        nins_g = rfl(rs[RSF_NINS_G]);
        n_ovf = rfl(rs[RSF_N_OVF]);
        hmax = rfl(rs[RSF_HMAX]);
        st_visits = rfl(rs[RSF_VISITS]);
        st_cand = rfl(rs[RSF_CAND]);
        st_pops = rfl(rs[RSF_POPS]);
        invis_base = rfl(rs[RSF_INVIS]);
        status = rfl(rs[RSF_STATUS]);
        next_base = rfl(rs[RSF_NEXT]);
        ended = rfl(rs[RSF_ENDED]) != 0;
    }

    {
        uint32_t nstarts = labels_some ? nql : 1u;
        if (a.default_start == VS_INVALID_NODE || a.n == 0 || status || resumed) nstarts = 0;
        for (uint32_t si = 0; si < nstarts; ++si) {
            uint32_t sn = VS_INVALID_NODE;
            if (!labels_some) {
                sn = a.default_start;
            } else {
                const int16_t lab = ql[si];
                int lo = 0, hi = (int)a.n_ls;
                while (lo < hi) {
                    const int mid = (lo + hi) >> 1;
                    if (a.ls_labels[mid] < lab) lo = mid + 1;
                    else hi = mid;
                }
                if (lo < (int)a.n_ls && a.ls_labels[lo] == lab) sn = a.ls_nodes[lo];
            }
            sn = rfl(sn);
            if (sn == VS_INVALID_NODE) continue;
            uint32_t slot = hash_home(sn), old = VS_EMPTY;
            bool fr;
            if (nins + WAVE > slot_limit) {
                fr = frozen_insert(sn, lane == 0, slot);
                if (status) break;
            } else {
                if (lane == 0) old = atomicCAS(&lhash[slot], VS_EMPTY, sn);
                fr = finish_insert(sn, lane == 0, slot, old, slot);
            }
            if (!rfl(fr ? 1u : 0u)) continue;
            slot = rfl(slot);
            const uint32_t d =
                rfl(ham_row_reg<NCH, QL, XW>(codes_v + (size_t)sn * cstride, qv, qc_l, l4, cstride, lane < 4, stream_rows));
            st_cand++;
            if (heap.len + 1 > s.hcap) { status |= OVF_HEAP; break; }
            heap.push((d << s.sb) | slot);
        }
    }

    uint32_t pfa_node = VS_INVALID_NODE, pfa_val = VS_INVALID_NODE, pfa_h = 0xFFFFFFFFu;
    uint32_t pfb_node = VS_INVALID_NODE, pfb_val = VS_INVALID_NODE, pfb_h = 0xFFFFFFFFu;
    const uint64_t* const nbr_mask = FULL ? a.nbr_mask : nullptr;
    uint64_t pfa_m = 0, pfb_m = 0;

    uint32_t ft_node = VS_INVALID_NODE;
    uint64_t ft_val = 0;
    uint32_t ft_vis = 1, st_invis = invis_base;
    uint32_t hslot0 = 0;
    uint4 gbk0 = make_uint4(0, 0, 0, 0);
    bool rchit0 = false;
    bool virg0 = false;
    uint32_t pret0 = 0;
    while (status == 0 && !(RS && ended)) {
        asm volatile("" : "+v"(lane));
        heap.lane = lane;
        vis.lane = lane;
        l4 = lane & 3;
        hslot0 = 0;
        gbk0 = make_uint4(0, 0, 0, 0);
        rchit0 = false;
        virg0 = false;
        pret0 = 0;
        if (VR > 0 && vis.len > 0) {
            const uint32_t fn = readlane_u32(vis.n[0], 0);
            if (fn != ft_node) {
                ft_node = fn;
                ft_val = load_stream64(tids_v + fn);
                if (visible) ft_vis = visible[fn];
            }
        }
        uint32_t top = 0;
        bool can_visit = heap.len > 0;
        if (can_visit) {
            top = heap.root();
            if (vis.len > s.L)
                can_visit = (top >> s.sb) < vis.ham_at(s.L - 1);
        }
        if (!can_visit) {
            if (BUILD) break;
            if (vis.len == 0) {
                ended = true;
                break;
            }
            uint32_t fd, fnode, fflags;
            vis.pop_front(fd, fnode, fflags);
            st_pops++;
            if (VR > 0) {
                const uint64_t tid = fnode == ft_node ? ft_val : load_stream64(tids_v + fnode);
                fflags = (tid & 0xFFFFull) == 0 ? VIS_DEAD : 0u;
                if (visible) fflags |= rfl(fnode == ft_node ? ft_vis : (uint32_t)visible[fnode]) == 0 ? VIS_HIDDEN : 0u;
            }
            if (fflags & VIS_DEAD) continue;
            if (visible && (fflags & VIS_HIDDEN)) {
                st_invis++;
                continue;
            }
            if (lane == 0) {
                s.out_ids[(size_t)q * s.M + emitted] = fnode;
                s.out_ham[(size_t)q * s.M + emitted] = fd;
                if (RS && s.row_stats) {
                    uint32_t* r = s.row_stats + ((size_t)q * s.M + emitted) * ST_N;
                    r[ST_VISITS] = st_visits;
                    r[ST_CAND] = st_cand;
                    r[ST_DQ] = st_cand;
                    r[ST_READS] = st_pops + st_visits + nins + nins_g;
                    r[ST_NEXT] = next_base + emitted + 1u + (st_invis - invis_base);
                    r[ST_GSPILL] = hmax;
                    r[ST_INVIS] = st_invis;
                    r[7] = nins + nins_g;
                }
            }
            emitted++;
            lap(6);
            if (emitted == s.M) break;
            continue;
        }
        hmax = max(hmax, heap.len);
        lap(6);
        const uint32_t hd = top >> s.sb;
        const uint32_t th = top & smask;
        const bool hit_a = th == pfa_h, hit_b = th == pfb_h;
        const bool hit = hit_a || hit_b;
        uint32_t node_v = hit_a ? pfa_node : pfb_node;
        if (!hit) node_v = node_load(th);
        uint32_t row0 = hit_a ? pfa_val : pfb_val;
        uint64_t rowm = hit_a ? pfa_m : pfb_m;
        uint64_t vtid = 1;
        uint32_t vvis = 1;
        bool early = false;
        if (hit) {
            if (VR == 0 && !BUILD) {
                vtid = load_stream64(tids_v + node_v);
                if (visible) vvis = visible[node_v];
            }
            if (gmode && nins_g <= s.glimit) {
                early = true;
                const uint64_t inval0 = __ballot(row0 == VS_INVALID_NODE);
                const bool act0 = (uint32_t)lane < (inval0 ? (uint32_t)__builtin_ctzll(inval0) : WAVE);
                virg0 = false;
                gbk0 = make_uint4(0, 0, 0, 0);
                if (VG == 3) {
                    hslot0 = q_fwd(row0);
                    pret0 = act0 ? b16_run(hslot0) : 0u;
                    if (pret0) gbk0 = b16_load(hslot0);
                } else if (VG == 2) {
                    hslot0 = slot_home(row0);
                    pret0 = act0 ? slot_run(hslot0) : 0u;
                    if (pret0) gbk0 = *reinterpret_cast<const uint4*>(ghash + (hslot0 & ~3u));
                } else {
                    hslot0 = ghash_home(row0);
                    rchit0 = rcv ? rc[hash_u32(row0 ^ 0x9e3779b9u) & rcm] == row0 : false;
                    if (act0 && !rchit0) gbk0 = bucket_fetch(hslot0, virg0);
                }
            }
        }
        heap.pop();
        const uint32_t node = hit ? rfl(node_v) : node_of(th, rfl(node_v));
        if (!hit && VR == 0 && !BUILD) {
            vtid = load_stream64(tids_v + node);
            if (visible) vvis = visible[node];
        }
        const uint32_t* nrow = nbrs_v + (size_t)node * nstride;
        if (!hit) {
            row0 = ((uint32_t)lane < R_v) ? load_stream32(nrow + lane) : VS_INVALID_NODE;
            if (nbr_mask) rowm = ((uint32_t)lane < R_v) ? load_stream64(nbr_mask + (size_t)node * nstride + lane) : 0ull;
        }
        lap(0);
        if (vis.len + 1 > vis.capacity()) {
            if (BUILD) vis.len = vis.capacity() - 1;
            else { status |= OVF_VISITED; break; }
        }
        st_visits++;
        uint32_t root_after = 0xFFFFFFFFu;
        uint32_t root_node_v = VS_INVALID_NODE;
        auto after_pop = [&]() {
            root_after = heap.len > 0 ? heap.root() : 0xFFFFFFFFu;
            if (root_after != 0xFFFFFFFFu) root_node_v = node_load(root_after & smask);
        };
        after_pop();
        uint32_t best = 0xFFFFFFFFu;
        uint32_t best_node = VS_INVALID_NODE;
        bool pfa_issued = false, pfb_issued = false, vis_done = false;
        bool list_ended = false;
        for (uint32_t c0 = 0; c0 < (R1 ? 1u : a.R) && !list_ended; c0 += WAVE) {
            const uint32_t slotidx = c0 + lane;
            const uint32_t nid = c0 == 0 ? row0 : ((slotidx < R_v) ? load_stream32(nrow + slotidx) : VS_INVALID_NODE);
            const uint64_t inval = __ballot(nid == VS_INVALID_NODE);
            const uint32_t nvalid = inval ? (uint32_t)__builtin_ctzll(inval) : WAVE;
            if (nvalid < WAVE) list_ended = true;
            const bool act = (uint32_t)lane < nvalid;
            lap(1);
            const bool frozen = !gmode && nins + WAVE > slot_limit;
            uint32_t hslot = gmode ? (VG == 3 ? q_fwd(nid) : VG == 2 ? slot_home(nid) : ghash_home(nid)) : hash_home(nid), old = VS_EMPTY;
            uint4 gbk = make_uint4(0, 0, 0, 0);
            bool rchit = false, virg = false;
            uint32_t pret = 0;
            if (gmode && early && c0 == 0) {
                hslot = hslot0;
                gbk = gbk0;
                rchit = rchit0;
                virg = virg0;
                pret = pret0;
            } else if (gmode && VG == 3) {
                if (nins_g > s.glimit) { status |= OVF_HASH; break; }
                pret = act ? b16_run(hslot) : 0u;
                if (pret) gbk = b16_load(hslot);
            } else if (gmode && VG == 2) {
                if (nins_g > s.glimit) { status |= OVF_HASH; break; }
                pret = act ? slot_run(hslot) : 0u;
                if (pret) gbk = *reinterpret_cast<const uint4*>(ghash + (hslot & ~3u));
            } else if (gmode) {
                if (nins_g > s.glimit) { status |= OVF_HASH; break; }
                if (rcv && act) rchit = rc[hash_u32(nid ^ 0x9e3779b9u) & rcm] == nid;
                if (act && !rchit) gbk = bucket_fetch(hslot, virg);
            } else if (!frozen && act) {
                old = atomicCAS(&lhash[hslot], VS_EMPTY, nid);
            }
            if (!vis_done) {
                vis_done = true;
                vis.insert(hd, node, ((vtid & 0xFFFFull) == 0 ? VIS_DEAD : 0u) | (vvis == 0 ? VIS_HIDDEN : 0u));
                lap(2);
            }
            bool fresh;
            if (gmode && VG == 3) {
                fresh = b16_insert(nid, act, hslot, gbk, pret, true, hslot);
                if (__ballot(n_ovf + WAVE > ovf_lim_v)) status |= OVF_HASH;
            } else if (gmode && VG == 2) {
                fresh = slot_insert(nid, act, hslot, gbk, pret, hslot);
            } else if (gmode) {
                fresh = global_insert(nid, act && !rchit, hslot, gbk, virg, hslot);
                if (rcv && act && !rchit) rc[hash_u32(nid ^ 0x9e3779b9u) & rcm] = nid;
            } else if (frozen) {
                fresh = frozen_insert(nid, act, hslot);
                if (status) break;
            } else {
                fresh = finish_insert(nid, act, hslot, old, hslot);
            }
            bool pass = fresh;
            if (has_label_filter && nbr_mask) {
                const uint64_t nm = c0 == 0 ? rowm : ((slotidx < R_v) ? load_stream64(nbr_mask + (size_t)node * nstride + slotidx) : 0ull);
                pass = fresh && (nm & qmask) != 0;
            } else if (has_label_filter && a.label_mask) {
                if (fresh) pass = (a.label_mask[nid] & qmask) != 0;
            } else if (has_label_filter && fresh) {
                const uint32_t lb = a.label_off[nid], le = a.label_off[nid + 1];
                uint32_t i = 0, j = lb;
                bool ov = false;
                while (i < nql && j < le) {
                    const int16_t x = ql[i], y = a.label_val[j];
                    if (x == y) { ov = true; break; }
                    if (x < y) ++i;
                    else ++j;
                }
                pass = ov;
            }
            const uint64_t pm = __ballot(pass);
            const uint32_t c = (uint32_t)__popcll(pm);
            lap(3);
            if (c) {
                if (heap.len + c > s.hcap) { status |= OVF_HEAP; break; }
                if (pass) {
                    const uint32_t rank = (uint32_t)__popcll(pm & ((1ull << lane) - 1ull));
                    surv_id[rank] = nid;
                    surv_slot[rank] = hslot;
                }
                wave_sync();
            }
            if (c == 0) continue;
            const uint32_t pre_n = heap.first_run(c);
            const uint32_t pre_anc = pre_n ? heap.wide_load(pre_n) : 0u;
            const uint32_t npass = (c + 15u) >> 4;
            for (uint32_t pass_i = 0; pass_i < npass; pass_i += G2 ? 2u : 1u) {
                const uint32_t j = pass_i * 16u + (uint32_t)(lane >> 2);
                const bool valid = j < c;
                const uint32_t id = valid ? surv_id[j] : 0;
                const uint64_t* crow = codes_v + (size_t)id * cstride;
                if (pass_i == 0 && !pfa_issued) {
                    pfa_issued = true;
                    pfa_node = VS_INVALID_NODE;
                    pfa_h = 0xFFFFFFFFu;
                    if (root_after != 0xFFFFFFFFu) {
                        pfa_node = node_of(root_after & smask, rfl(root_node_v));
                        pfa_h = root_after & smask;
                        pfa_val = ((uint32_t)lane < R_v) ? load_stream32(nbrs_v + (size_t)pfa_node * nstride + lane) : VS_INVALID_NODE;
                        if (nbr_mask) pfa_m = ((uint32_t)lane < R_v) ? load_stream64(nbr_mask + (size_t)pfa_node * nstride + lane) : 0ull;
                    }
                }
                if (G2) {
                    const uint32_t j2 = j + 16u;
                    const bool valid2 = j2 < c;
                    const uint64_t* crow2 = codes_v + (size_t)(valid2 ? surv_id[j2] : 0u) * cstride;
                    uint32_t d, d2;
                    ham_row_reg2<NCH, QL>(crow, crow2, qv, qc_l, l4, cstride, valid, valid2, stream_rows, d, d2);
                    if (valid && l4 == 0) surv_d[j] = LEAN ? ((d << s.sb) | surv_slot[j]) : d;
                    if (valid2 && l4 == 0) surv_d[j2] = LEAN ? ((d2 << s.sb) | surv_slot[j2]) : d2;
                    continue;
                }
                const uint32_t d = ham_row_reg<NCH, QL, XW>(crow, qv, qc_l, l4, cstride, valid, stream_rows);
                if (valid && l4 == 0) surv_d[j] = LEAN ? ((d << s.sb) | surv_slot[j]) : d;
            }
            st_cand += c;
            wave_sync();
            uint32_t entry = 0xFFFFFFFFu;
            if ((uint32_t)lane < c) entry = LEAN ? surv_slot[lane] : ((surv_d[lane] << s.sb) | surv_slot[lane]);
            if (TIMING) {
                if (__ballot(entry == 0xFFFFFFFEu) == ~0ull) status |= 0x100;
                lap(4);
            }
            {
                const uint32_t m = wave_min_u32(entry);
                if (m < best) {
                    best = m;
                    best_node = rfl(surv_id[__builtin_ctzll(__ballot(entry == m))]);
                }
            }
            if ((R1 || list_ended || c0 + WAVE >= a.R) && !pfb_issued) {
                pfb_issued = true;
                pfb_node = VS_INVALID_NODE;
                pfb_h = 0xFFFFFFFFu;
                if (best != 0xFFFFFFFFu && (best >> s.sb) < (root_after >> s.sb)) {
                    pfb_node = best_node;
                    pfb_h = best & smask;
                    pfb_val = ((uint32_t)lane < R_v) ? load_stream32(nbrs_v + (size_t)pfb_node * nstride + lane) : VS_INVALID_NODE;
                    if (nbr_mask) pfb_m = ((uint32_t)lane < R_v) ? load_stream64(nbr_mask + (size_t)pfb_node * nstride + lane) : 0ull;
                }
            }
            heap.push_run(entry, c, pre_n, pre_anc);
            lap(5);
        }
        if (status) break;
        if (!vis_done) vis.insert(hd, node, ((vtid & 0xFFFFull) == 0 ? VIS_DEAD : 0u) | (vvis == 0 ? VIS_HIDDEN : 0u));
        if (!pfa_issued) {
            pfa_node = VS_INVALID_NODE;
            pfa_h = 0xFFFFFFFFu;
            if (root_after != 0xFFFFFFFFu) {
                pfa_node = node_of(root_after & smask, rfl(root_node_v));
                pfa_h = root_after & smask;
                pfa_val = ((uint32_t)lane < R_v) ? load_stream32(nbrs_v + (size_t)pfa_node * nstride + lane) : VS_INVALID_NODE;
                if (nbr_mask) pfa_m = ((uint32_t)lane < R_v) ? load_stream64(nbr_mask + (size_t)pfa_node * nstride + lane) : 0ull;
            }
        }
        if (!pfb_issued) {
            pfb_node = VS_INVALID_NODE;
            pfb_h = 0xFFFFFFFFu;
        }
    }
    if (BUILD && VR == 0 && status == 0) {
        emitted = min(vis.len, s.M);
        for (uint32_t i = lane; i < emitted; i += WAVE) {
            const uint64_t e = vis.ring[vis.slot(i)];
            s.out_ids[(size_t)q * s.M + i] = (uint32_t)e;
            s.out_ham[(size_t)q * s.M + i] = (uint32_t)(e >> 32) & VIS_HAM_MASK;
        }
    }
    const uint32_t st_next = next_base + emitted + (st_invis - invis_base) + ((emitted < s.M && status == 0) ? 1u : 0u);
    if (RS) {
        wave_sync();
        for (uint32_t i = 4u * lane; i < image_words; i += 4u * WAVE) *reinterpret_cast<uint4*>(rs + RSF_HDR + i) = *reinterpret_cast<const uint4*>(hp + i);
        if (lane == 0) {
            rs[RSF_INIT] = 1u;
            rs[RSF_HLEN] = heap.len;
            rs[RSF_VHEAD] = vis.head;
            rs[RSF_VLEN] = vis.len;
            rs[RSF_NINS_G] = nins_g;
            rs[RSF_N_OVF] = n_ovf;
            rs[RSF_HMAX] = hmax;
            rs[RSF_VISITS] = st_visits;
            rs[RSF_CAND] = st_cand;
            rs[RSF_POPS] = st_pops;
            rs[RSF_INVIS] = st_invis;
            rs[RSF_STATUS] = status;
            rs[RSF_NEXT] = st_next;
            rs[RSF_ENDED] = ended ? 1u : 0u;
        }
    }
    if (status == 0) {
        for (uint32_t i = emitted + lane; i < s.M; i += WAVE) {
            s.out_ids[(size_t)q * s.M + i] = VS_INVALID_NODE;
            s.out_ham[(size_t)q * s.M + i] = 0xFFFFFFFFu;
        }
    }
    if (lane == 0) {
        if (onlyfv && s.fb_flag) s.fb_flag[q] = 1;
        s.status[q] = status;
        s.out_cnt[q] = status ? 0 : emitted;
        if (status == 0) {
            uint32_t* st = s.stats + (size_t)q * ST_N;
            st[ST_VISITS] = st_visits;
            st[ST_CAND] = st_cand;
            st[ST_DQ] = st_cand;
            st[ST_READS] = st_pops + st_visits + nins + nins_g;
            st[ST_NEXT] = st_next;
            st[ST_GSPILL] = hmax;
            st[ST_INVIS] = st_invis;
            st[7] = nins + nins_g;
        }
        if (TIMING && s.phase) {
            lap(6);
            for (int k = 0; k < 8; ++k) s.phase[(size_t)q * 8 + k] = ph[k];
        }
        if (s.timeline) s.timeline[2 * (size_t)q + 1] = wall_clock64();
    }
}

template <int NCH, int VR, bool TIMING, int MINW, bool BUILD, bool FULL = true, int VG = 0, int OPT = 0>
__global__ __launch_bounds__(WAVE, MINW) void k_search_fast(FastArgs a) {
    for (uint32_t it = 0;; ++it) {
        uint32_t q = blockIdx.x;
        if (a.s.persist) {
            if (threadIdx.x == 0) q = atomicAdd(a.s.scan_counter, 1u);
            q = rfl(q);
        } else if (it) {
            return;
        }
        if (q >= a.s.nq) return;
        fast_scan<NCH, VR, TIMING, MINW, BUILD, FULL, VG, OPT>(a, q, blockIdx.x);
        wave_sync();
    }
}

#if VS_FAST_TU == 0
size_t fast_resume_words(const FastLaunch& s) { return RSF_HDR + ((size_t)(s.hl + 1) + 2 * (size_t)s.vcap + s.vwords + 3) / 4 * 4; }

size_t fast_lds_bytes(const vs_index* idx, const FastLaunch& s) {
    const size_t nch = (idx->code_stride + 7) / 8;
    const size_t qcopy = nch > 6 ? (size_t)idx->code_stride * 8 : (s.minw >= 6 && !s.build && !s.phase ? nch * 64 : 0);
    const bool lean = s.minw == 7 && s.vslot == 2 && nch == 3 && !s.build && !s.phase;
    const bool plain = !s.qlabel_off && !s.visible && !(s.flags & FAST_FULL_VARIANT);
    size_t b = (size_t)(s.hl + 1) * 4 + (size_t)s.lh * 4 + (lean ? 2 : 3) * 64 * 4 + (s.vslot ? 0 : ARB_SLOTS * 4) + (s.vr ? 0 : (size_t)s.vcap * 8) +
               (lean && plain ? 0 : MAX_QLABELS * 2) + qcopy + (size_t)s.rc * 4 + (size_t)s.vwords * 4 + (lean ? 16 : 32);
    return (b + 15) / 16 * 16;
}

#endif

template <int NCH, int VR, bool TIMING, int MINW, bool BUILD, bool FULL = true, int VG = 0, int OPT = 0>
static int launch_fast_tt(vs_index* idx, const FastArgs& a, size_t lds, uint32_t* resident) {
    static DeviceOnce attr_set;
    const int attr_dev = idx->ctx->device;
    if (attr_set.pending(attr_dev)) {
        VS_HIP(hipFuncSetAttribute(reinterpret_cast<const void*>(k_search_fast<NCH, VR, TIMING, MINW, BUILD, FULL, VG, OPT>),
                                   hipFuncAttributeMaxDynamicSharedMemorySize, 160 * 1024));
        attr_set.done(attr_dev);
    }
    if (resident) {
        int per_cu = 0;
        VS_HIP(hipOccupancyMaxActiveBlocksPerMultiprocessor(&per_cu, k_search_fast<NCH, VR, TIMING, MINW, BUILD, FULL, VG, OPT>, WAVE, lds));
        *resident = (uint32_t)std::max(per_cu, 1) * (uint32_t)idx->ctx->prop.multiProcessorCount;
        return VS_OK;
    }
    const uint32_t grid = a.s.persist ? std::min<uint32_t>(a.s.persist, a.s.nq) : a.s.nq;
    hipLaunchKernelGGL((k_search_fast<NCH, VR, TIMING, MINW, BUILD, FULL, VG, OPT>), dim3(grid), dim3(WAVE), lds, idx->ctx->stream, a);
    VS_HIP(hipGetLastError());
    return VS_OK;
}

int launch_fast_plain6(vs_index* idx, const FastArgs& a, size_t lds, uint32_t* res, bool std_geom);
int launch_fast_keys6(vs_index* idx, const FastArgs& a, size_t lds, uint32_t* res, bool std_geom);
#if VS_FAST_TU == 1
int launch_fast_plain6(vs_index* idx, const FastArgs& a, size_t lds, uint32_t* res, bool std_geom) {
    if (std_geom) return launch_fast_tt<3, 0, false, 6, false, false, 3, OPT_XW | OPT_R1 | OPT_NS64>(idx, a, lds, res);
    return launch_fast_tt<3, 0, false, 6, false, false, 3>(idx, a, lds, res);
}
#elif VS_FAST_TU == 2
int launch_fast_keys6(vs_index* idx, const FastArgs& a, size_t lds, uint32_t* res, bool std_geom) {
    if (std_geom) return launch_fast_tt<3, 0, false, 6, false, true, 3, OPT_XW | OPT_R1 | OPT_NS64>(idx, a, lds, res);
    return launch_fast_tt<3, 0, false, 6, false, true, 3>(idx, a, lds, res);
}
#else
template <int NCH>
static int launch_fast_t(vs_index* idx, const FastArgs& a, size_t lds, uint32_t* res) {
    if (a.s.build) {
        VS_REQUIRE(a.s.vr == 0 && !a.s.phase, "build-mode search uses the LDS-ring visited list");
        return launch_fast_tt<NCH, 0, false, 1, true>(idx, a, lds, res);
    }
    if (a.s.phase) {
        VS_REQUIRE(NCH == 3, "VS_PHASE diagnostics are built for 17..24-word codes only");
        if (a.s.vr == 8) return launch_fast_tt<3, 8, true, 1, false>(idx, a, lds, res);
        return launch_fast_tt<3, 0, true, 1, false>(idx, a, lds, res);
    }
    if (a.s.resume) {
        VS_REQUIRE(a.s.vwords && a.s.vslot == 2 && !a.s.persist && a.s.vr == 0 && a.s.lh == 0 && a.s.rc == 0 && !a.s.only_failed && a.s.pool_slots >= a.s.nq,
                   "fast search: resumable scans run the 16-bit tables with one region per slot");
        return launch_fast_tt<NCH, 0, false, 1, false, true, 3, OPT_RS>(idx, a, lds, res);
    }
    if (a.s.vwords && a.s.vslot == 2) {
        VS_REQUIRE(a.s.vr == 0 && a.s.lh == 0 && a.s.rc == 0 && a.s.gcap >= 256 && (a.s.gcap & (a.s.gcap - 1)) == 0 && a.s.ocap % 32 == 0 && a.s.ocap >= 64 &&
                       (uint64_t)a.s.vwords * 32 >= (uint64_t)a.s.gcap + a.s.ocap && a.s.qk >= 3 && a.s.qk <= 16 && a.s.qd <= 32 &&
                       (1ull << a.s.qd) == ((uint64_t)(a.s.gcap >> 3) << a.s.qk) && (a.s.qd >= 32 || a.n <= (1ull << a.s.qd)) &&
                       a.s.gregion >= (a.s.gcap >> 1) + a.s.ocap,
                   "fast search: bad geometry of the 16-bit dedup table");
        const bool plain = !a.s.qlabel_off && !a.s.visible && !(a.s.flags & FAST_FULL_VARIANT);
        const bool std_geom = a.code_stride == 24 && a.R <= WAVE && a.nbr_stride == 64;
        if (NCH == 3 && a.s.minw == 6 && plain) return launch_fast_plain6(idx, a, lds, res, std_geom);
        if (NCH == 3 && a.s.minw == 6) return launch_fast_keys6(idx, a, lds, res, std_geom);
        if (NCH == 3 && a.s.minw == 7 && plain && std_geom) return launch_fast_tt<3, 0, false, 7, false, false, 3, OPT_XW | OPT_R1 | OPT_NS64>(idx, a, lds, res);
        if (NCH == 3 && a.s.minw == 7 && plain) return launch_fast_tt<3, 0, false, 7, false, false, 3>(idx, a, lds, res);
        if (NCH == 3 && a.s.minw == 7) return launch_fast_tt<3, 0, false, 7, false, true, 3>(idx, a, lds, res);
        return launch_fast_tt<NCH, 0, false, 1, false, true, 3>(idx, a, lds, res);
    }
    if (a.s.vwords && a.s.vslot) {
        VS_REQUIRE(a.s.vr == 0 && a.s.lh == 0 && (uint64_t)a.s.vwords * 32 >= a.s.gcap && a.s.rc == 0,
                   "fast search: the slot bitmap needs the table-less regime and one bit per slot");
        const bool plain = !a.s.qlabel_off && !a.s.visible && !(a.s.flags & FAST_FULL_VARIANT);
        if (NCH == 3 && a.s.minw == 6 && plain) return launch_fast_tt<3, 0, false, 6, false, false, 2>(idx, a, lds, res);
        if (NCH == 3 && a.s.minw == 6) return launch_fast_tt<3, 0, false, 6, false, true, 2>(idx, a, lds, res);
        return launch_fast_tt<NCH, 0, false, 1, false, true, 2>(idx, a, lds, res);
    }
    if (a.s.vwords) {
        VS_REQUIRE(a.s.vr == 0 && a.s.lh == 0 && (uint64_t)a.s.vwords * 128 >= a.s.gcap,
                   "fast search: the written-bucket bitmap needs the table-less regime and one bit per bucket");
        const bool plain = !a.s.qlabel_off && !a.s.visible && !(a.s.flags & FAST_FULL_VARIANT);
        if (NCH == 3 && a.s.minw == 6 && plain) return launch_fast_tt<3, 0, false, 6, false, false, 1>(idx, a, lds, res);
        if (NCH == 3 && a.s.minw == 6) return launch_fast_tt<3, 0, false, 6, false, true, 1>(idx, a, lds, res);
        if (NCH == 3 && a.s.minw == 5 && plain) return launch_fast_tt<3, 0, false, 5, false, false, 1>(idx, a, lds, res);
        if (NCH == 3 && a.s.minw == 5) return launch_fast_tt<3, 0, false, 5, false, true, 1>(idx, a, lds, res);
        return launch_fast_tt<NCH, 0, false, 1, false, true, 1>(idx, a, lds, res);
    }
    if (a.s.vr == 8) {
        if (NCH == 3) {
            if (a.s.minw == 4) return launch_fast_tt<3, 8, false, 4, false>(idx, a, lds, res);
            if (a.s.minw == 5) return launch_fast_tt<3, 8, false, 5, false>(idx, a, lds, res);
            if (a.s.minw == 6) return launch_fast_tt<3, 8, false, 6, false>(idx, a, lds, res);
        }
        return launch_fast_tt<NCH, 8, false, 1, false>(idx, a, lds, res);
    }
    if (NCH == 3) {
        const bool plain = !a.s.qlabel_off && !a.s.visible && !(a.s.flags & FAST_FULL_VARIANT);
        if (a.s.minw == 5 && plain) return launch_fast_tt<3, 0, false, 5, false, false>(idx, a, lds, res);
        if (a.s.minw == 5) return launch_fast_tt<3, 0, false, 5, false>(idx, a, lds, res);
        if (a.s.minw == 6 && plain) return launch_fast_tt<3, 0, false, 6, false, false>(idx, a, lds, res);
        if (a.s.minw == 6) return launch_fast_tt<3, 0, false, 6, false>(idx, a, lds, res);
        if (a.s.minw == 7) return launch_fast_tt<3, 0, false, 7, false>(idx, a, lds, res);
        if (a.s.minw == 8) return launch_fast_tt<3, 0, false, 8, false>(idx, a, lds, res);
    }
    return launch_fast_tt<NCH, 0, false, 1, false>(idx, a, lds, res);
}

static int fast_dispatch(vs_index* idx, const FastLaunch& s, uint32_t* res) {
    FastArgs a;
    a.codes = idx->codes;
    a.nbrs = idx->nbrs;
    a.tids = idx->tids;
    a.label_off = idx->label_off;
    a.label_val = idx->label_val;
    a.label_mask = idx->label_mask;
    a.label_bit = idx->label_bit;
    a.nbr_mask = nullptr;
    if (s.qlabel_off && idx->label_mask && !s.build) {
        VS_TRY(vs_refresh_neighbor_masks(idx));
        if (idx->nbr_mask_valid && vs_neighbor_masks_wanted(idx)) a.nbr_mask = idx->nbr_mask;
    }
    a.ls_labels = idx->ls_labels;
    a.ls_nodes = idx->ls_nodes;
    a.code_stride = idx->code_stride;
    a.nbr_stride = idx->nbr_stride;
    a.R = idx->d.num_neighbors;
    a.n = idx->d.n;
    a.n_ls = idx->d.n_label_starts;
    a.default_start = idx->d.default_start;
    a.s = s;
    if (!a.s.glimit) a.s.glimit = s.gcap / 4 * 3 - WAVE;
    const size_t lds = fast_lds_bytes(idx, s);
    VS_REQUIRE(lds <= 160 * 1024, "fast search state does not fit LDS (%zu B)", lds);
    VS_REQUIRE(((s.hl + 1) & s.hl) == 0 && s.hl >= 63, "fast search: hl must be 2^k - 1 >= 63");
    VS_REQUIRE(s.vr == 8 || (s.vr == 0 && s.vcap >= 64),
               "fast search: visited list must be 8 register pairs or a ring of >= 64 entries");
    VS_REQUIRE(s.lh % 4 == 0 && (s.lh == 0 || s.lh >= 256) && s.gcap % 4 == 0 && s.gcap >= 256 &&
                   (uint64_t)s.lh + s.gcap + (s.vslot == 2 ? s.ocap : 0u) <= (1ull << s.sb) && s.hcap >= s.hl && s.gstride % 2 == 0 &&
                   s.gstride >= s.hcap - s.hl + 2,
               "fast search: bad dedup table / spill geometry");
    const uint32_t nch = (idx->code_stride + 7) / 8;
    switch (nch) {
        case 1: return launch_fast_t<1>(idx, a, lds, res);
        case 2: return launch_fast_t<2>(idx, a, lds, res);
        case 3: return launch_fast_t<3>(idx, a, lds, res);
        case 4: return launch_fast_t<4>(idx, a, lds, res);
        case 5:
        case 6: return launch_fast_t<6>(idx, a, lds, res);
        default: return launch_fast_t<0>(idx, a, lds, res);
    }
}

int launch_search_fast(vs_index* idx, const FastLaunch& s) {
    if (s.nq == 0) return VS_OK;
    VS_REQUIRE(!s.persist || (s.scan_counter && s.pool_slots >= std::min(s.persist, s.nq)),
               "fast search: a persistent grid needs a scan counter and one region per workgroup");
    return fast_dispatch(idx, s, nullptr);
}

int fast_resident_scans(vs_index* idx, const FastLaunch& s, uint32_t* out) { return fast_dispatch(idx, s, out); }
#endif
```

pgvectorscale_amd/index.py:

```python
import ctypes as C

import numpy as np

from . import _lib
from ._lib import VS_COSINE, VS_INVALID_NODE, VS_IP, VS_L2, IndexDesc, IndexHost, Stats, check

DEFAULT_QUERY_SEARCH_LIST_SIZE = 100
DEFAULT_QUERY_RESCORE = 50
DEFAULT_NUM_NEIGHBORS = 50


def default_bits(dims_to_index):
    return 2 if dims_to_index < 900 else 1


def quantized_size(dims, bits):
    return (dims * bits + 63) // 64


def _p(a):
    return None if a is None else a.ctypes.data_as(C.c_void_p)


def set_option(name, value):
    check(_lib.load().vs_set_option(name.encode(), None if value is None else str(value).encode()))


def get_option(name):
    buf = C.create_string_buffer(256)
    r = check(_lib.load().vs_get_option(name.encode(), buf, 256))
    return buf.value.decode() if r == 1 else None


class Context:

    def __init__(self, device=0):
        self._L = _lib.load()
        h = C.c_void_p()
        check(self._L.vs_ctx_create(device, C.byref(h)))
        self.h = h
        self.device = device

    def device_name(self):
        buf = C.create_string_buffer(256)
        check(self._L.vs_ctx_device_name(self.h, buf, 256))
        return buf.value.decode()

    def mem_info(self):
        f, t = C.c_uint64(), C.c_uint64()
        check(self._L.vs_ctx_mem_info(self.h, C.byref(f), C.byref(t)))
        return int(f.value), int(t.value)

    def sync(self):
        check(self._L.vs_ctx_sync(self.h))

    def profile_enable(self, on=True):
        check(self._L.vs_profile_enable(self.h, int(on)))

    def profile_read(self, reset=True):
        p = _lib.Profile()
        check(self._L.vs_profile_read(self.h, C.byref(p), int(reset)))
        names = ["prepare_queries", "search", "rerank", "resort", "search_fallback", "scan", "rerank_order", "pages_encode"]
        return {n: (float(p.ms[k]), int(p.launches[k])) for k, n in enumerate(names)}

    def ws_probe(self, d_mem, nbytes, iters=600):
        ms = C.c_float(0)
        check(self._L.vs_ws_probe(self.h, d_mem, nbytes, iters, C.byref(ms)))
        return float(ms.value)

    def alloc(self, nbytes):
        p = C.c_void_p()
        check(self._L.vs_dev_alloc(self.h, nbytes, C.byref(p)))
        return p

    def free(self, p):
        check(self._L.vs_dev_free(self.h, p))

    def upload(self, dev_ptr, arr):
        arr = np.ascontiguousarray(arr)
        check(self._L.vs_dev_upload(self.h, dev_ptr, _p(arr), arr.nbytes))

    def download(self, dev_ptr, arr):
        assert arr.flags["C_CONTIGUOUS"]
        check(self._L.vs_dev_download(self.h, _p(arr), dev_ptr, arr.nbytes))
        return arr

    def close(self):
        if self.h:
            self._L.vs_ctx_destroy(self.h)
            self.h = None


class DiskAnnIndex:

    def __init__(self, ctx, handle):
        self.ctx = ctx
        self._L = ctx._L
        self.h = handle
        d = IndexDesc()
        check(self._L.vs_index_get_desc(self.h, C.byref(d)))
        self.desc = d

    def view(self, ctx):
        h = C.c_void_p()
        check(self._L.vs_index_view(self.h, ctx.h, C.byref(h)))
        return DiskAnnIndex(ctx, h)

    def ws_probe_mix(self, d_mem, nbytes, iters=400):
        ms = C.c_float(0)
        check(self._L.vs_ws_probe_mix(self.h, d_mem, nbytes, iters, C.byref(ms)))
        return float(ms.value)

    def set_slab(self, d_mem, nbytes):
        check(self._L.vs_index_set_slab(self.h, d_mem, nbytes))

    def prepare_workspace(self):
        check(self._L.vs_index_prepare_workspace(self.h))

    @classmethod
    def upload(cls, ctx, *, codes, nbrs, heap_tids, vecs, mean, m2, count, bits, dim_index, num_neighbors,
               distance_type, default_start, label_off=None, label_val=None, label_starts=None, storage_type=_lib.VS_STORAGE_SBQ):
        if storage_type == _lib.VS_STORAGE_PLAIN:
            return cls._upload_plain(ctx, nbrs=nbrs, heap_tids=heap_tids, vecs=vecs, num_neighbors=num_neighbors,
                                     distance_type=distance_type, default_start=default_start, dim_index=dim_index)
        codes = np.ascontiguousarray(codes, np.uint64)
        nbrs = np.ascontiguousarray(nbrs, np.uint32)
        heap_tids = np.ascontiguousarray(heap_tids, np.uint64)
        vecs = None if vecs is None else np.ascontiguousarray(vecs, np.float32)
        mean = np.ascontiguousarray(mean, np.float32)
        m2 = None if m2 is None else np.ascontiguousarray(m2, np.float32)
        n, w = codes.shape
        if nbrs.ndim != 2 or nbrs.shape[0] != n or nbrs.shape[1] < num_neighbors:
            raise ValueError(f"nbrs must be [{n}][>= {num_neighbors}], got {nbrs.shape}")
        if heap_tids.shape != (n,):
            raise ValueError(f"heap_tids must have shape ({n},), got {heap_tids.shape}")
        if vecs is not None and (vecs.ndim != 2 or vecs.shape[0] != n or vecs.shape[1] < dim_index):
            raise ValueError(f"vecs must be [{n}][>= {dim_index}], got {vecs.shape}")
        if mean.shape != (dim_index,) or (m2 is not None and m2.shape != (dim_index,)):
            raise ValueError(f"mean / m2 must have shape ({dim_index},)")
        if label_off is not None and np.asarray(label_off).shape != (n + 1,):
            raise ValueError(f"label_off must have shape ({n + 1},)")
        d = IndexDesc()
        d.n, d.dim_index, d.bits, d.words = n, dim_index, bits, w
        d.dim_full = dim_index if vecs is None else vecs.shape[1]
        d.num_neighbors, d.distance_type = num_neighbors, distance_type
        d.has_labels = int(label_off is not None)
        d.default_start = default_start
        ls = sorted((label_starts or {}).items())
        d.n_label_starts = len(ls)
        lsl = np.array([k for k, _ in ls], np.int16)
        lsn = np.array([v for _, v in ls], np.uint32)
        lo = None if label_off is None else np.ascontiguousarray(label_off, np.uint32)
        lv = None if label_val is None else np.ascontiguousarray(label_val, np.int16)
        h = IndexHost()
        h.codes, h.nbrs, h.nbr_stride = _p(codes).value, _p(nbrs).value, nbrs.shape[1]
        h.heap_tids = _p(heap_tids).value
        h.vecs = None if vecs is None else _p(vecs).value
        h.mean = _p(mean).value
        h.m2 = None if m2 is None else _p(m2).value
        h.count = count
        h.label_off = None if lo is None else _p(lo).value
        h.label_val = None if lv is None else _p(lv).value
        h.label_start_labels = _p(lsl).value if len(ls) else None
        h.label_start_nodes = _p(lsn).value if len(ls) else None
        out = C.c_void_p()
        check(ctx._L.vs_index_upload(ctx.h, C.byref(d), C.byref(h), C.byref(out)))
        return cls(ctx, out)

    @classmethod
    def _upload_plain(cls, ctx, *, nbrs, heap_tids, vecs, num_neighbors, distance_type, default_start, dim_index=None):
        nbrs = np.ascontiguousarray(nbrs, np.uint32)
        heap_tids = np.ascontiguousarray(heap_tids, np.uint64)
        vecs = np.ascontiguousarray(vecs, np.float32)
        d = IndexDesc()
        d.n, d.dim_full, d.dim_index = vecs.shape[0], vecs.shape[1], dim_index or vecs.shape[1]
        d.bits, d.words = 1, quantized_size(d.dim_index, 1)
        d.num_neighbors, d.distance_type, d.has_labels = num_neighbors, distance_type, 0
        d.default_start, d.n_label_starts, d.storage_type = default_start, 0, _lib.VS_STORAGE_PLAIN
        h = IndexHost()
        h.nbrs, h.nbr_stride, h.heap_tids, h.vecs = _p(nbrs).value, nbrs.shape[1], _p(heap_tids).value, _p(vecs).value
        out = C.c_void_p()
        check(ctx._L.vs_index_upload(ctx.h, C.byref(d), C.byref(h), C.byref(out)))
        return cls(ctx, out)

# ... 669 lines not shown
```

Baseline: 4.425 million.

## Order persistent graph scans by query locality and cache code rows

Adds a scan-ordering step that clusters the queries (via the existing scan-order kernel) before the fast search. Persistent workgroups then take queries from eight per-group permutation queues, stealing from other queues when theirs run dry. When the expected reuse is high and the working tables fit a nominal last-level cache budget, code rows use plain cached loads instead of non-temporal loads. The search permutation is reused for rerank ordering, the f32 query copy is skipped when the raw device queries can be used directly, and Hamming output writes are dropped when unneeded. The cost is an extra ordering kernel plus atomic queue contention, and cached loads risk thrashing if the cache-size heuristic is wrong.

```diff
diff --git a/include/vsgpu.h b/include/vsgpu.h
--- a/include/vsgpu.h
+++ b/include/vsgpu.h
@@ -109,6 +109,8 @@
                 VS_ARR_VNORM = 6, VS_ARR_LABEL_OFF = 7, VS_ARR_LABEL_VAL = 8 };
 int vs_index_array(const vs_index* idx, int which, void** dev_ptr, uint32_t* row_stride);
 int vs_index_rerank_order(vs_index* idx, uint32_t* out_perm, uint32_t cap, uint32_t* out_n);
+int vs_search_order_rule(uint64_t n, uint32_t nq, uint32_t stream_len, int filtered, int persist16, uint32_t resident_scans,
+                         uint32_t region_words);
 int vs_index_set_quantizer(vs_index* idx, const float* mean, const float* m2, uint64_t count);
 int vs_index_set_start_nodes(vs_index* idx, uint32_t default_start, const int16_t* labels, const uint32_t* nodes, uint32_t n);
 int vs_index_set_labels(vs_index* idx, const uint32_t* label_off, const int16_t* label_val);
diff --git a/pgvectorscale_amd/__init__.py b/pgvectorscale_amd/__init__.py
--- a/pgvectorscale_amd/__init__.py
+++ b/pgvectorscale_amd/__init__.py
@@ -1,3 +1,3 @@
 from ._lib import VS_COSINE, VS_INVALID_NODE, VS_IP, VS_L2, VsError, load
-from .index import Broker, Context, DiskAnnIndex, IndexScan, ScanPool, ShmClient, ShmServer, get_option, set_option
+from .index import Broker, Context, DiskAnnIndex, IndexScan, ScanPool, ShmClient, ShmServer, get_option, search_order_rule, set_option
 from .multi import Comm, MultiIndex
diff --git a/pgvectorscale_amd/_lib.py b/pgvectorscale_amd/_lib.py
--- a/pgvectorscale_amd/_lib.py
+++ b/pgvectorscale_amd/_lib.py
@@ -215,6 +215,7 @@
     "vs_index_get_desc": (_i, [_vp, C.POINTER(IndexDesc)]),
     "vs_index_array": (_i, [_vp, _i, C.POINTER(_vp), C.POINTER(_u32)]),
     "vs_index_rerank_order": (_i, [_vp, _vp, _u32, C.POINTER(_u32)]),
+    "vs_search_order_rule": (_i, [_u64, _u32, _u32, _i, _i, _u32, _u32]),
     "vs_index_set_quantizer": (_i, [_vp, _vp, _vp, _u64]),
     "vs_index_set_start_nodes": (_i, [_vp, _u32, _vp, _vp, _u32]),
     "vs_index_set_labels": (_i, [_vp, _vp, _vp]),
diff --git a/pgvectorscale_amd/csrc/vs_batch.hip b/pgvectorscale_amd/csrc/vs_batch.hip
--- a/pgvectorscale_amd/csrc/vs_batch.hip
+++ b/pgvectorscale_amd/csrc/vs_batch.hip
@@ -108,6 +108,27 @@
     return std::min<uint32_t>(S, ix->d.n);
 }
 
+static const uint32_t ORDER_SEARCH_SEEDS = 2048;
+static const size_t LAST_LEVEL_CACHE_BYTES = 256ull << 20;
+static const size_t ORDER_HOT_ROWS_BYTES = 64ull << 20;
+static bool search_order_rule(uint32_t mode, uint64_t n, uint32_t nq, uint32_t M, bool filtered, bool persist16, uint32_t resident,
+                              uint32_t region_words) {
+    const size_t tables = (size_t)resident * region_words * 4;
+    const double reuse = n ? (double)nq * M / (double)n : 0.0;
+    const bool fits = tables + ORDER_HOT_ROWS_BYTES < LAST_LEVEL_CACHE_BYTES;
+    const bool yes = mode == 2 || (mode == 1 && nq >= ORDER_MIN_NQ && reuse >= ORDER_MIN_REUSE && !filtered && persist16 && fits);
+    if (env_u32("VS_WS_DEBUG", 0))
+        fprintf(stderr, "[VS_WS_DEBUG] scan order: %s, code rows %s (mode %u, nq %u, reuse %.2f, %s, %s, tables %zu MB + %zu MB rows against %zu MB)\n",
+                yes ? "ordered" : "not ordered", yes ? "plain loads" : "non-temporal loads", mode, nq, reuse, filtered ? "filtered" : "unfiltered",
+                persist16 ? "persistent grid + 16-bit tables" : "other launch form", tables >> 20, ORDER_HOT_ROWS_BYTES >> 20,
+                LAST_LEVEL_CACHE_BYTES >> 20);
+    return yes;
+}
+extern "C" int vs_search_order_rule(uint64_t n, uint32_t nq, uint32_t stream_len, int filtered, int persist16, uint32_t resident_scans,
+                                    uint32_t region_words) {
+    return search_order_rule(env_u32("VS_SEARCH_ORDER", 1), n, nq, stream_len, filtered != 0, persist16 != 0, resident_scans, region_words) ? 1 : 0;
+}
+
 static int ensure_region_labels(vs_index* ix, uint32_t S) {
     vs_ctx* c = ix->ctx;
     SearchWorkspace& w = ix->ws;
@@ -160,7 +181,11 @@
         bool deal = false;
         w.order_nq = 0;
         bool by_labels = false;
-        if (const uint32_t S = rerank_order_seeds(ix, nq, M, &by_labels)) {
+        if (w.search_ordered && env_u32("VS_RERANK_ORDER", 1) != 0) {
+            perm = (const uint32_t*)w.order_perm.p;
+            w.order_nq = nq;
+            deal = env_u32("VS_RERANK_DEAL", 1) != 0;
+        } else if (const uint32_t S = rerank_order_seeds(ix, nq, M, &by_labels)) {
             VS_TRY(devbuf_reserve(c, w.order_work, scan_order_work_bytes(nq, S + 1)));
             VS_TRY(devbuf_reserve(c, w.order_perm, (size_t)nq * 4));
             if (by_labels) VS_TRY(ensure_region_labels(ix, S));
@@ -178,7 +203,7 @@
         const uint32_t fused = env_u32("VS_RERANK_FUSED", 1);
         if (fused && rerank_window_fits(ix, M, bp.rescore, bp.k)) {
             hipEvent_t ev = prof_begin(c);
-            VS_TRY(launch_rerank_window(ix, (const float*)w.q_full.p, (const uint32_t*)w.stream_ids.p, (const uint32_t*)w.stream_cnt.p, M,
+            VS_TRY(launch_rerank_window(ix, w.rerank_q, (const uint32_t*)w.stream_ids.p, (const uint32_t*)w.stream_cnt.p, M,
                                         bp.rescore, bp.k, nq, d_out_ids, d_out_tids, d_out_dist, fused == 2 ? 2u : 1u, perm, deal));
             prof_end(c, PK_RERANK, ev);
             return VS_OK;
@@ -186,7 +211,7 @@
         VS_TRY(devbuf_reserve(c, w.rr_dist, (size_t)nq * M * 4));
         VS_TRY(devbuf_reserve(c, w.resort_heap, (size_t)nq * bp.rescore * 8));
         hipEvent_t ev = prof_begin(c);
-        VS_TRY(launch_rerank(ix, (const float*)w.q_full.p, (const uint32_t*)w.stream_ids.p, nullptr,
+        VS_TRY(launch_rerank(ix, w.rerank_q, (const uint32_t*)w.stream_ids.p, nullptr,
                              (const uint32_t*)w.stream_cnt.p, M, nq, (float*)w.rr_dist.p, 0, perm, deal));
         prof_end(c, PK_RERANK, ev);
     }
@@ -238,13 +263,15 @@
     return s;
 }
 
+static const size_t POOL_CTR_BYTES = 128;
+
 static int reserve_general_regions(vs_index* ix, const Caps& caps, uint32_t gslots) {
     vs_ctx* c = ix->ctx;
     SearchWorkspace& w = ix->ws;
     const size_t hg = caps.hcap > caps.hl ? caps.hcap - caps.hl : 0;
     VS_TRY(devbuf_reserve(c, w.hash, (size_t)gslots * caps.hashcap * 4));
     VS_TRY(devbuf_reserve(c, w.heap_g, std::max<size_t>((size_t)gslots * hg * 8, 16)));
-    return devbuf_reserve(c, w.pool_ctr, 64);
+    return devbuf_reserve(c, w.pool_ctr, POOL_CTR_BYTES);
 }
 
 static int retry_failed_scans(vs_index* ix, const BatchPlan& bp, const int16_t* d_qlabels, const uint32_t* d_qlabel_off,
@@ -286,6 +313,7 @@
     FastLaunch f;
     uint32_t gregion;
     uint32_t fslots;
+    bool ordered;
 };
 template <class T>
 static T* fast_select() {
@@ -383,6 +411,15 @@
     f.persist = std::max<uint32_t>(1, (uint32_t)((uint64_t)res * env_u32("VS_F_PERSIST_PCT", 100) / 100));
     *fslots = std::min(f.persist, f.nq);
     return VS_OK;
+}
+
+static void choose_scan_order(const vs_index* ix, const BatchPlan& bp, FastPlan& p, bool keyed, bool masked, bool phase) {
+    FastLaunch& f = p.f;
+    p.ordered = false;
+    const uint32_t mode = env_u32("VS_SEARCH_ORDER", 1);
+    if (mode == 0 || !f.persist || phase || ix->is_view || bp.stream_only || !scan_order_fits(ix)) return;
+    p.ordered = search_order_rule(mode, ix->d.n, bp.nq, bp.M, keyed || masked, f.vslot == 2, p.fslots, p.gregion);
+    f.rows_cached = p.ordered ? 1u : 0u;
 }
 
 static int plan_fast_launch(vs_index* ix, const BatchPlan& bp, Caps& caps, bool keyed, bool masked, FastPlan* out) {
@@ -418,6 +455,7 @@
     choose_ring_step7(f, bp.L);
     if (phase) f.phase = fast_select<uint64_t>();
     VS_TRY(choose_persistent_grid(ix, f, &p.fslots));
+    choose_scan_order(ix, bp, p, keyed, masked, phase);
     *out = p;
     return VS_OK;
 }
@@ -425,6 +463,9 @@
 static bool second_attempt_of(const vs_index* ix, const FastLaunch& first, uint32_t nq, FastLaunch* out) {
     const SearchWorkspace& w = ix->ws;
     FastLaunch r = first;
+    r.perm = nullptr;
+    r.order_counter = nullptr;
+    r.rows_cached = 0;
     r.vwords = 0;
     r.vslot = 0;
     r.persist = 0;
@@ -446,7 +487,8 @@
     return nbits < (1ull << (32 - r.sb)) && fast_lds_bytes(ix, r) <= 64 * 1024;
 }
 
-static int bind_fast_buffers(vs_index* ix, FastPlan& p, const int16_t* d_qlabels, const uint32_t* d_qlabel_off, const uint8_t* visible) {
+static int bind_fast_buffers(vs_index* ix, FastPlan& p, const int16_t* d_qlabels, const uint32_t* d_qlabel_off, const uint8_t* visible,
+                             bool want_ham) {
     vs_ctx* c = ix->ctx;
     SearchWorkspace& w = ix->ws;
     FastLaunch& f = p.f;
@@ -466,8 +508,8 @@
         fprintf(stderr, "[VS_WS_DEBUG] ghash4 %p (%zu B%s) heap_g4 %p (%zu B%s) region bytes: table %zu heap %zu x %u regions; stream_ids %p qcodes %p\n", w.ghash4.p,
                 w.ghash4.bytes, w.ghash4.in_slab ? ", slab" : "", w.heap_g4.p, w.heap_g4.bytes, w.heap_g4.in_slab ? ", slab" : "",
                 (size_t)p.gregion * 4, (size_t)f.gstride * 4, p.fslots, w.stream_ids.p, w.qcodes.p);
-    VS_TRY(devbuf_reserve(c, w.pool_ctr, 64));
-    VS_HIP(hipMemsetAsync(w.pool_ctr.p, 0, 64, c->stream));
+    VS_TRY(devbuf_reserve(c, w.pool_ctr, POOL_CTR_BYTES));
+    VS_HIP(hipMemsetAsync(w.pool_ctr.p, 0, POOL_CTR_BYTES, c->stream));
     VS_TRY(devbuf_reserve(c, w.fb_flag, (size_t)f.nq * 4));
     VS_HIP(hipMemsetAsync(w.fb_flag.p, 0, (size_t)f.nq * 4, c->stream));
     f.qlabels = d_qlabels;
@@ -477,11 +519,13 @@
     f.ghash = (uint32_t*)w.ghash4.p;
     f.pool_counter = (uint32_t*)w.pool_ctr.p;
     f.scan_counter = (uint32_t*)w.pool_ctr.p + 2;
+    f.perm = p.ordered ? (const uint32_t*)w.order_perm.p : nullptr;
+    f.order_counter = p.ordered ? (uint32_t*)w.pool_ctr.p + 16 : nullptr;
     f.pool_slots = p.fslots;
     f.phase = nullptr;
     f.qcodes = (const uint64_t*)w.qcodes.p;
     f.out_ids = (uint32_t*)w.stream_ids.p;
-    f.out_ham = (uint32_t*)w.stream_ham.p;
+    f.out_ham = want_ham ? (uint32_t*)w.stream_ham.p : nullptr;
     f.out_cnt = (uint32_t*)w.stream_cnt.p;
     f.stats = (uint32_t*)w.stats.p;
     f.status = (uint32_t*)w.status.p;
@@ -544,7 +588,17 @@
     FastPlan p;
     VS_TRY(plan_fast_launch(ix, bp, caps, d_qlabel_off != nullptr, visible != nullptr, &p));
     FastLaunch& f = p.f;
-    VS_TRY(bind_fast_buffers(ix, p, d_qlabels, d_qlabel_off, visible));
+    if (p.ordered) {
+        const uint32_t S = std::min<uint32_t>(std::min<uint32_t>(std::max<uint32_t>(env_u32("VS_RERANK_SEEDS", ORDER_SEARCH_SEEDS), 1), 4096), ix->d.n);
+        VS_TRY(devbuf_reserve(c, w.order_work, scan_order_work_bytes(bp.nq, S + 1)));
+        VS_TRY(devbuf_reserve(c, w.order_perm, (size_t)bp.nq * 4));
+        hipEvent_t evo = prof_begin(c);
+        VS_TRY(launch_scan_order(ix, (const uint64_t*)w.qcodes.p, bp.nq, S, (uint32_t*)w.order_work.p, (uint32_t*)w.order_perm.p));
+        prof_end(c, PK_ORDER, evo);
+        w.search_ordered = true;
+    }
+    const bool want_ham = bp.stream_only || ix->d.storage_type == VS_STORAGE_PLAIN;
+    VS_TRY(bind_fast_buffers(ix, p, d_qlabels, d_qlabel_off, visible, want_ham));
     VS_TRY(bind_phase_buffer(ix, f));
     std::string tl_path;
     VS_TRY(bind_timeline_buffer(ix, f, &tl_path));
@@ -567,12 +621,15 @@
     return VS_OK;
 }
 
-static int run_search_chunk(vs_index* ix, const BatchPlan& bp, const float* d_raw_q, const int16_t* d_qlabels,
+static int run_search_chunk(vs_index* ix, const BatchPlan& bp, const float* d_raw_q, bool q_kept, const int16_t* d_qlabels,
                             const uint32_t* d_qlabel_off, uint32_t* d_out_ids, uint64_t* d_out_tids, float* d_out_dist, Caps& caps) {
     vs_ctx* c = ix->ctx;
     SearchWorkspace& w = ix->ws;
     const uint32_t nq = bp.nq, M = bp.M;
-    VS_TRY(devbuf_reserve(c, w.q_full, (size_t)nq * ix->vec_stride * 4));
+    const bool q_bypass = q_kept && ix->d.storage_type != VS_STORAGE_PLAIN && ix->d.distance_type != VS_COSINE &&
+                          ix->d.dim_index == ix->d.dim_full && ix->vec_stride == ix->d.dim_full;
+    if (!q_bypass) VS_TRY(devbuf_reserve(c, w.q_full, (size_t)nq * ix->vec_stride * 4));
+    w.rerank_q = q_bypass ? d_raw_q : (const float*)w.q_full.p;
     VS_TRY(devbuf_reserve(c, w.qcodes, (size_t)nq * ix->code_stride * 8));
     VS_TRY(devbuf_reserve(c, w.stream_ids, (size_t)nq * M * 4));
     VS_TRY(devbuf_reserve(c, w.stream_ham, (size_t)nq * M * 4));
@@ -581,7 +638,7 @@
     VS_TRY(devbuf_reserve(c, w.status, (size_t)nq * 4));
     {
         hipEvent_t ev = prof_begin(c);
-        VS_TRY(launch_prepare_queries(ix, d_raw_q, nq, (float*)w.q_full.p, (uint64_t*)w.qcodes.p));
+        VS_TRY(launch_prepare_queries(ix, d_raw_q, nq, q_bypass ? nullptr : (float*)w.q_full.p, (uint64_t*)w.qcodes.p));
         if (ix->d.storage_type == VS_STORAGE_PLAIN && ix->d.dim_index < ix->d.dim_full) {
             VS_TRY(devbuf_reserve(c, w.q_index, (size_t)nq * ix->vec_stride * 4));
             VS_TRY(launch_prepare_index_slice(ix, d_raw_q, nq, (float*)w.q_index.p));
@@ -589,6 +646,7 @@
         prof_end(c, PK_PREPARE, ev);
     }
     ix->last_fast = FastSig{};
+    w.search_ordered = false;
     const bool fast_done = caps.f_on;
     if (fast_done) VS_TRY(run_fast_attempts(ix, bp, caps, d_qlabels, d_qlabel_off));
     w.fb_valid = fast_done;
@@ -832,7 +890,7 @@
         VS_TRY(devbuf_reserve(c, *otids[ci & 1], (size_t)chunk * k * 8));
         VS_TRY(devbuf_reserve(c, *odist[ci & 1], (size_t)chunk * k * 4));
         bp = BatchPlan{cq, L, rescore, k, M, stream_only};
-        return run_search_chunk(ix, bp, (const float*)rawq[ci & 1]->p, d_labels_all, d_off_all ? d_off_all + q0 : nullptr,
+        return run_search_chunk(ix, bp, (const float*)rawq[ci & 1]->p, false, d_labels_all, d_off_all ? d_off_all + q0 : nullptr,
                                 (uint32_t*)oids[ci & 1]->p, (uint64_t*)otids[ci & 1]->p, (float*)odist[ci & 1]->p, caps);
     };
     auto finish = [&](uint32_t ci, const BatchPlan& bp) -> int {
@@ -918,7 +976,7 @@
     Caps caps = initial_caps(ix, L, M);
     VS_REQUIRE(chunk_queries(ix, caps, M, nq) == nq, "vs_search_batch_dev: batch of %u queries exceeds the workspace budget", nq);
     BatchPlan bp{nq, L, rescore, k, M, false};
-    VS_TRY(run_search_chunk(ix, bp, d_queries, d_qlabels, d_qlabel_off, d_out_ids, d_out_tids, d_out_dist, caps));
+    VS_TRY(run_search_chunk(ix, bp, d_queries, true, d_qlabels, d_qlabel_off, d_out_ids, d_out_tids, d_out_dist, caps));
     w.pending = true;
     w.pend = PendingBatch{bp, caps, d_qlabels, d_qlabel_off, d_out_ids, d_out_tids, d_out_dist};
     ix->last_stats = vs_stats{};
diff --git a/pgvectorscale_amd/csrc/vs_internal.h b/pgvectorscale_amd/csrc/vs_internal.h
--- a/pgvectorscale_amd/csrc/vs_internal.h
+++ b/pgvectorscale_amd/csrc/vs_internal.h
@@ -133,6 +133,8 @@
         order_work, order_perm,
         order_labels;
     uint32_t order_nq = 0;
+    const float* rerank_q = nullptr;
+    bool search_ordered = false;
     uint32_t lab_rows = 0, lab_S = 0, lab_step = 0;
     uint64_t lab_epoch = 0;
     uint64_t* red_host = nullptr;
@@ -330,6 +332,9 @@
     uint32_t* status;
     uint64_t* phase = nullptr;
     uint32_t* scan_counter = nullptr;
+    const uint32_t* perm = nullptr;
+    uint32_t* order_counter = nullptr;
+    uint32_t rows_cached = 0;
     uint64_t* timeline = nullptr;
     uint32_t* resume = nullptr;
     uint32_t resume_stride = 0;
@@ -366,7 +371,7 @@
        OVF_KEY = 16 };
 size_t search_lds_bytes(const vs_index* idx, const SearchLaunch& s);
 
-int launch_prepare_queries(vs_index* idx, const float* d_raw, uint32_t nq, float* d_q_full, uint64_t* d_qcodes);
+int launch_prepare_queries(vs_index* idx, const float* d_raw, uint32_t nq, float* d_q_full , uint64_t* d_qcodes);
 int launch_quantize_rows(vs_index* idx, const float* d_rows, uint32_t row_stride, uint32_t nrows, uint64_t* d_codes,
                          uint32_t code_stride);
 int launch_hamming_gather(vs_index* idx, const uint64_t* d_qcodes, const uint32_t* d_ids, const uint32_t* d_off,
diff --git a/pgvectorscale_amd/csrc/vs_kernels.hip b/pgvectorscale_amd/csrc/vs_kernels.hip
--- a/pgvectorscale_amd/csrc/vs_kernels.hip
+++ b/pgvectorscale_amd/csrc/vs_kernels.hip
@@ -112,8 +112,10 @@
             __syncthreads();
         }
         if (active) {
-            float* qf = q_full + (size_t)q * vec_stride;
-            for (uint32_t i = lane; i < vec_stride / 4; i += WAVE) reinterpret_cast<float4*>(qf)[i] = reinterpret_cast<const float4*>(full)[i];
+            if (q_full) {
+                float* qf = q_full + (size_t)q * vec_stride;
+                for (uint32_t i = lane; i < vec_stride / 4; i += WAVE) reinterpret_cast<float4*>(qf)[i] = reinterpret_cast<const float4*>(full)[i];
+            }
             if (multi) {
                 const float ranges = (float)(bits + 1);
                 for (uint32_t dim = lane; dim < dim_index; dim += WAVE) {
diff --git a/pgvectorscale_amd/csrc/vs_search_fast.hip b/pgvectorscale_amd/csrc/vs_search_fast.hip
--- a/pgvectorscale_amd/csrc/vs_search_fast.hip
+++ b/pgvectorscale_amd/csrc/vs_search_fast.hip
@@ -603,6 +603,7 @@
 #define OPT_NS64 4
 #define OPT_RS 8
 #define OPT_G2 16
+#define OPT_ROWS_CACHED 32
 template <int NCH, int VR, bool TIMING, int MINW, bool BUILD, bool FULL, int VG, int OPT>
 __device__ __forceinline__ void fast_scan(const FastArgs& a, const uint32_t q, const uint32_t slot) {
     constexpr bool XW = (OPT & OPT_XW) != 0 && NCH > 0;
@@ -647,7 +648,7 @@
     uint64_t* qc_l = QL ? qc_fix : reinterpret_cast<uint64_t*>(smem + ((((vmap + s.vwords) - reinterpret_cast<uint32_t*>(smem)) * 4u + 15u) & ~15u));
 
     int l4 = lane & 3;
-    constexpr bool stream_rows = true;
+    constexpr bool stream_rows = (OPT & OPT_ROWS_CACHED) == 0;
     constexpr bool G2 = NCH == 3 && VR == 0 && (MINW == 5 || (OPT & OPT_G2) != 0) && !BUILD && !TIMING;
     ulonglong2 qv[NCH > 0 ? NCH : 1];
     if (QL) {
@@ -1151,7 +1152,7 @@
             }
             if (lane == 0) {
                 s.out_ids[(size_t)q * s.M + emitted] = fnode;
-                s.out_ham[(size_t)q * s.M + emitted] = fd;
+                if (s.out_ham) s.out_ham[(size_t)q * s.M + emitted] = fd;
                 if (RS && s.row_stats) {
                     uint32_t* r = s.row_stats + ((size_t)q * s.M + emitted) * ST_N;
                     r[ST_VISITS] = st_visits;
@@ -1404,7 +1405,7 @@
         for (uint32_t i = lane; i < emitted; i += WAVE) {
             const uint64_t e = vis.ring[vis.slot(i)];
             s.out_ids[(size_t)q * s.M + i] = (uint32_t)e;
-            s.out_ham[(size_t)q * s.M + i] = (uint32_t)(e >> 32) & VIS_HAM_MASK;
+            if (s.out_ham) s.out_ham[(size_t)q * s.M + i] = (uint32_t)(e >> 32) & VIS_HAM_MASK;
         }
     }
     const uint32_t st_next = next_base + emitted + (st_invis - invis_base) + ((emitted < s.M && status == 0) ? 1u : 0u);
@@ -1431,7 +1432,7 @@
     if (status == 0) {
         for (uint32_t i = emitted + lane; i < s.M; i += WAVE) {
             s.out_ids[(size_t)q * s.M + i] = VS_INVALID_NODE;
-            s.out_ham[(size_t)q * s.M + i] = 0xFFFFFFFFu;
+            if (s.out_ham) s.out_ham[(size_t)q * s.M + i] = 0xFFFFFFFFu;
         }
     }
     if (lane == 0) {
@@ -1457,13 +1458,43 @@
     }
 }
 
+__device__ static inline uint32_t take_ordered_scan(const FastLaunch& s, uint32_t x) {
+    const uint32_t per = (s.nq + 7u) / 8u;
+#pragma nounroll
+    for (;;) {
+        const uint32_t first = x * per, have = first < s.nq ? min(per, s.nq - first) : 0u;
+        uint32_t p = 0;
+        if (threadIdx.x == 0) p = atomicAdd(s.order_counter + x, 1u);
+        p = rfl(p);
+        if (p < have) return s.perm[first + p];
+        uint32_t most = 0, from = 8;
+#pragma nounroll
+        for (uint32_t y = 0; y < 8; ++y) {
+            const uint32_t fy = y * per, hy = fy < s.nq ? min(per, s.nq - fy) : 0u;
+            uint32_t cy = 0;
+            if (threadIdx.x == 0) cy = atomicAdd(s.order_counter + y, 0u);
+            cy = rfl(cy);
+            if (cy < hy && hy - cy > most) {
+                most = hy - cy;
+                from = y;
+            }
+        }
+        if (from == 8) return 0xFFFFFFFFu;
+        x = from;
+    }
+}
+
 template <int NCH, int VR, bool TIMING, int MINW, bool BUILD, bool FULL = true, int VG = 0, int OPT = 0>
 __global__ __launch_bounds__(WAVE, MINW) void k_search_fast(FastArgs a) {
     for (uint32_t it = 0;; ++it) {
         uint32_t q = blockIdx.x;
         if (a.s.persist) {
-            if (threadIdx.x == 0) q = atomicAdd(a.s.scan_counter, 1u);
-            q = rfl(q);
+            if (a.s.perm) {
+                q = take_ordered_scan(a.s, blockIdx.x & 7u);
+            } else {
+                if (threadIdx.x == 0) q = atomicAdd(a.s.scan_counter, 1u);
+                q = rfl(q);
+            }
         } else if (it) {
             return;
         }
@@ -1513,6 +1544,7 @@
 int launch_fast_keys6(vs_index* idx, const FastArgs& a, size_t lds, uint32_t* res, bool std_geom);
 #if VS_FAST_TU == 1
 int launch_fast_plain6(vs_index* idx, const FastArgs& a, size_t lds, uint32_t* res, bool std_geom) {
+    if (std_geom && a.s.rows_cached) return launch_fast_tt<3, 0, false, 6, false, false, 3, OPT_XW | OPT_R1 | OPT_NS64 | OPT_ROWS_CACHED>(idx, a, lds, res);
     if (std_geom) return launch_fast_tt<3, 0, false, 6, false, false, 3, OPT_XW | OPT_R1 | OPT_NS64>(idx, a, lds, res);
     return launch_fast_tt<3, 0, false, 6, false, false, 3>(idx, a, lds, res);
 }
@@ -1640,6 +1672,8 @@
     if (s.nq == 0) return VS_OK;
     VS_REQUIRE(!s.persist || (s.scan_counter && s.pool_slots >= std::min(s.persist, s.nq)),
                "fast search: a persistent grid needs a scan counter and one region per workgroup");
+    VS_REQUIRE(!s.perm || (s.persist && s.order_counter && !s.only_failed && !s.resume && !s.build),
+               "fast search: an ordered batch runs on the persistent grid, first attempt only");
     return fast_dispatch(idx, s, nullptr);
 }
 
diff --git a/pgvectorscale_amd/index.py b/pgvectorscale_amd/index.py
--- a/pgvectorscale_amd/index.py
+++ b/pgvectorscale_amd/index.py
@@ -30,6 +30,10 @@
     buf = C.create_string_buffer(256)
     r = check(_lib.load().vs_get_option(name.encode(), buf, 256))
     return buf.value.decode() if r == 1 else None
+
+
+def search_order_rule(n, nq, stream_len, filtered, persist16, resident_scans, region_words):
+    return bool(check(_lib.load().vs_search_order_rule(n, nq, stream_len, int(filtered), int(persist16), resident_scans, region_words)))
 
 
 class Context:
```

New measurement: 4.503 million (median of 6 runs). Within noise of the previous version (+1.7%).
